# siyuanwu99/pred-occ-planner

Measured on AMD Instinct MI355X. Metric: replans/sec (SOGM update + QP: full replan = SOGM update + A* + corridors + QP + deconfliction), 128-agent batch per GPU, 200x200x200x20 voxel grid; aggregate over all agents, higher is better.
Workload: dtype f32 occupancy / f64 planning; 1 GPU; 128 agents/GPU x 1 GPU, 200x200x200x20 SOGM, sim_fkpcp-style moving cylinders, batched ADMM QP (BASELINE configs[2] per GPU); agents_total=128, cloud_points=622040, cylinders=555, map_input_staleness_ticks=0, parallelism=agents sharded x1, 1 all-gather/tick, exchange=local, sogm_grids_per_agent=3, sogm_reset=sparse (logged 32-byte sectors), sogm_cell_order=2x2x2 tiles, map_update=at the start of the tick

## Files before the change

### include/sogm_abi_debug.h

```cpp
#ifndef SOGM_ABI_DEBUG_H
#define SOGM_ABI_DEBUG_H
#include "sogm_abi.h"
#ifdef __cplusplus
extern "C" {
#endif

int sogm_sparse_reset_state(sogm_ctx *ctx, int32_t *out_host);

int         sogm_set_tuning(sogm_ctx *ctx, const char *key, double value);
int         sogm_get_tuning(const sogm_ctx *ctx, const char *key, double *out_value_host);
const char *sogm_tuning_key(int index);

int sogm_map_traffic(sogm_ctx *ctx, int64_t *out_host, int reset);

int sogm_grid_history(sogm_ctx *ctx, int32_t *out_host);

enum {
  SOGM_PROF_CLEAR = 0,
  SOGM_PROF_STAMP = 1,
  SOGM_PROF_SPLAT = 2,
  SOGM_PROF_ASTAR = 3,
  SOGM_PROF_CORRIDOR = 4,
  SOGM_PROF_QP = 5,
  SOGM_PROF_CLEAR_HEAD = 6,
  SOGM_PROF_EXCHANGE = 7,
  SOGM_PROF_N = 8
};
int sogm_set_profiling(sogm_ctx *ctx, int enable);
int sogm_set_profiling_slots(sogm_ctx *ctx, int slot_mask);
int sogm_profile_read(sogm_ctx *ctx, double *out_ms_host);
int sogm_profile_read_all(sogm_ctx *ctx, int slot, double *out_ms_host, int cap, int *out_n);

int sogm_device_clock(sogm_ctx *ctx, int64_t *out_ticks_host, void *stream);
int sogm_tick_clock(sogm_ctx *ctx, int64_t *out2_host);

int sogm_download_reference_layout(sogm_ctx *ctx, int agent, float *out_vt_host);

int sogm_dsp_download_state(sogm_dsp *d, int agent, float *store_host, float *objnum_host,
                            int32_t *counters_host);
int sogm_dsp_upload_state(sogm_dsp *d, int agent, const float *store_host, const float *last_pos3_host, double last_stamp,
                          const int32_t *cursors3_host);
int sogm_dsp_download_born(sogm_dsp *d, int agent, float *born_host, int cap, int32_t *n_born, int32_t *counters4);
int sogm_dsp_download_observations(sogm_dsp *d, int agent, int32_t *nobs_host, float *pc_host,
                                   float *maxlen_host);

int sogm_gridmap_download(sogm_gridmap *g, int agent, double *occupancy_host, int8_t *inflate_host,
                          int32_t *bounds_host, int32_t *counters_host);
int sogm_gridmap_force_frame(sogm_gridmap *g, int raycast_num);

int sogm_corridor_rules_batched(sogm_planner *counters_of, const SogmPlannerParams *pp_host, const double *start_pva,
                                const double *route, const int32_t *route_len, int route_cap, const double *polys,
                                const int32_t *nfaces, const int32_t *seg_state, int n, int max_faces, double *out_box,
                                double *out_shrunk, int32_t *out_seg_nfaces, int32_t *out_seg_state, double *out_polys,
                                int32_t *out_nfaces, int32_t *out_npoly, double *out_goal, void *stream);
#define SOGM_RULES_PARALLEL 1
int sogm_corridor_rules_batched_flags(sogm_planner *counters_of, const SogmPlannerParams *pp_host, const double *start_pva,
                                      const double *route, const int32_t *route_len, int route_cap, const double *polys,
                                      const int32_t *nfaces, const int32_t *seg_state, int n, int max_faces,
                                      double *out_box, double *out_shrunk, int32_t *out_seg_nfaces, int32_t *out_seg_state,
                                      double *out_polys, int32_t *out_nfaces, int32_t *out_npoly, double *out_goal,
                                      int flags, void *stream);

#define SOGM_FINISH_WAVE 1
int sogm_finish_batched(sogm_planner *counters_of, double corridor_tau, const int32_t *ret, const int32_t *npoly,
                        const int32_t *status, const double *cpts, const SogmTrajRecord *swarm, int n_swarm,
                        const int32_t *swarm_ego, const double *swarm_now, const double *t_start, const int32_t *drone_ids,
                        const int32_t *due, int n, SogmTrajRecord *out, int32_t *out_ok, int32_t *out_safe,
                        SogmTrajRecord *pub_own, SogmTrajRecord *pub_table, int flags, void *stream);

int sogm_debug_corridor_pairs(sogm_planner *p, unsigned long long *out4);

enum {
  SOGM_QP_STAT_TOTAL = 0,
  SOGM_QP_STAT_SETUP = 1,
  SOGM_QP_STAT_REFAC = 2,
  SOGM_QP_STAT_N_REFAC = 3,
  SOGM_QP_STAT_CHECK = 4,
  SOGM_QP_STAT_N_CHECK = 5,
  SOGM_QP_STAT_ITERS = 6,
  SOGM_QP_STAT_PATH = 7,
  SOGM_QP_STAT_FACTOR_ASM = 8,
  SOGM_QP_STAT_FACTOR_FWD = 9,
  SOGM_QP_STAT_FACTOR_BWD = 10,
  SOGM_QP_STAT_SHADER_CLOCKS = 11,
  SOGM_QP_STAT_CHECK_STAGE = 12,
  SOGM_QP_STAT_CHECK_RESID = 13,
  SOGM_QP_STAT_SETUP_SPLIT = 14,
  SOGM_QP_STAT_N = 16
};
int sogm_debug_qp_stats(sogm_planner *p, long long *out_host);
int sogm_debug_qp_layout(sogm_planner *p, int n_pieces, const int32_t *nfaces_host, long long *out8);

#ifdef __cplusplus
}
#endif
#endif
```

### pred-occ-planner_amd/_abi.py

```python
import ctypes as C
import os

_HERE = os.path.dirname(os.path.abspath(__file__))
LIB_PATH = os.environ.get("SOGM_LIB_PATH") or os.path.join(_HERE, "libsogm_hip.so")

SOGM_ABI_VERSION = 6
SOGM_MAX_PIECES = 16
SOGM_MAP_FAKE = 0
SOGM_MAP_RISKBASE = 1
SOGM_MAP_RISKVOXEL = 2
SOGM_STORE_F32, SOGM_STORE_F16 = 0, 1
SOGM_LAYOUT_TILED = 16
SOGM_DSP_MAX_T = 16

SOGM_OK = 0
SOGM_ERR_INVALID_ARG = -1
SOGM_ERR_NO_DEVICE = -2
SOGM_ERR_HIP = -3
SOGM_ERR_CAPACITY = -4
SOGM_ERR_STATE = -5
SOGM_ERR_COMM = -6
SOGM_COMM_ID_BYTES = 128
PROF_CLEAR, PROF_STAMP, PROF_SPLAT, PROF_ASTAR, PROF_CORRIDOR, PROF_QP, PROF_CLEAR_HEAD, PROF_EXCHANGE, PROF_N = range(9)

# ... 148 lines not shown
MAPAUDIT_ROW_FIELDS = ("n_region", "n_test", "n_truth", "n_both", "n_test_near", "n_truth_near", "truth_slice", "status")
MAPAUDIT_PARAMS_BYTES = C.sizeof(SogmMapAuditParams)

SOGM_VIEW_OUTSIDE, SOGM_VIEW_OFFIMAGE, SOGM_VIEW_FREE, SOGM_VIEW_SURFACE, SOGM_VIEW_HIDDEN = 0, 1, 2, 3, 4
SOGM_VIEWBIT_OUTSIDE, SOGM_VIEWBIT_OFFIMAGE, SOGM_VIEWBIT_FREE, SOGM_VIEWBIT_SURFACE, SOGM_VIEWBIT_HIDDEN = 1, 2, 4, 8, 16
SOGM_VIEWBIT_ALL = 31
VIEW_CLASS_NAMES = ("outside", "offimage", "free", "surface", "hidden")


class SogmViewParams(C.Structure):
    _fields_ = [("fx", C.c_double), ("fy", C.c_double), ("cx", C.c_double), ("cy", C.c_double), ("depth_scale", C.c_double),
                ("max_depth", C.c_double), ("near_z", C.c_double), ("far_z", C.c_double), ("tan_h", C.c_double),
                ("tan_v", C.c_double), ("band", C.c_double), ("rows", C.c_int32), ("cols", C.c_int32), ("classes", C.c_int32),
                ("reserved_", C.c_int32)]


VIEW_PARAMS_BYTES = C.sizeof(SogmViewParams)


class SogmFsmParams(C.Structure):
    _fields_ = [("replan_duration", C.c_double), ("replan_start_time", C.c_double), ("goal_tolerance", C.c_double),
                ("new_plan_interval", C.c_double), ("replan_max_failures", C.c_int32), ("reserved_", C.c_int32)]


class SogmFsmState(C.Structure):
    _fields_ = [("traj_start", C.c_double), ("status", C.c_int32), ("fail", C.c_int32), ("success", C.c_int32),
                ("reserved_", C.c_int32)]


class SogmFlightFsm(C.Structure):
    _fields_ = [("prm", SogmFsmParams), ("check_duration", C.c_double), ("state_inout", C.c_void_p),
                ("log_state", C.c_void_p), ("log_due", C.c_void_p), ("log_safe", C.c_void_p), ("log_reached", C.c_void_p),
                ("log_pub", C.c_void_p), ("log_hover_start", C.c_void_p), ("log_own", C.c_void_p)]


FSM_STATE_BYTES = C.sizeof(SogmFsmState)
FSM_PUB_NONE, FSM_PUB_NEW, FSM_PUB_HOVER = 0, 1, 2

SOGM_TRAJSRV_QUEUE = 256
SOGM_CMD_PUBLISHED, SOGM_CMD_HELD = 1, 2


class SogmTrajServerParams(C.Structure):
    _fields_ = [("replan_threshold", C.c_double), ("sample_dt", C.c_double), ("yaw_pi", C.c_double),
                ("yaw_dot_max", C.c_double), ("yaw_mode", C.c_int32), ("reserved_", C.c_int32)]


class SogmTrajPoint(C.Structure):
    _fields_ = [("t", C.c_double), ("pos", C.c_double * 3), ("vel", C.c_double * 3), ("acc", C.c_double * 3),
                ("yaw", C.c_double), ("yaw_dot", C.c_double)]


class SogmPositionCommand(C.Structure):
    _fields_ = [("t_pub", C.c_double), ("t_sample", C.c_double), ("pos", C.c_double * 3), ("vel", C.c_double * 3),
                ("acc", C.c_double * 3), ("yaw", C.c_double), ("yaw_dot", C.c_double), ("traj_id", C.c_int32),
                ("flags", C.c_int32)]


class SogmTrajServerCore(C.Structure):
    _fields_ = [("ts", C.c_double), ("te", C.c_double), ("duration", C.c_double), ("last_yaw", C.c_double),
                ("last_yawdot", C.c_double), ("init_pos", C.c_double * 3), ("head", C.c_int32), ("size", C.c_int32),
                ("traj_id", C.c_int32), ("received", C.c_int32), ("overflow", C.c_int32), ("reserved_", C.c_int32 * 3)]


FLIGHT_MAX_TICKS = 64
RULES_PARALLEL = 1
FINISH_WAVE = 1
FLIGHT_HDR_ERR, FLIGHT_HDR_FINISHED, FLIGHT_HDR_LATE_WGS = 4, 5, 15
FLIGHT_STAT_NAMES = ("gate_wait", "map", "search", "corridor", "qp", "finish", "chain", "ticks")
TRAJ_RECORD_BYTES = C.sizeof(SogmTrajRecord)
CYLINDER_BYTES = C.sizeof(SogmCylinder)
DEPTH_CAMERA_BYTES = C.sizeof(SogmDepthCamera)
DEPTH_BODIES_BYTES = C.sizeof(SogmDepthBodies)
SOGM_HIT_GROUND, SOGM_HIT_NONE = -1, -2
LABEL_SOURCES_BYTES = C.sizeof(SogmLabelSources)


class SogmTrajServerState(C.Structure):
    _fields_ = [("core", SogmTrajServerCore), ("traj", SogmTrajRecord)]


TRAJ_POINT_BYTES = C.sizeof(SogmTrajPoint)
POSITION_COMMAND_BYTES = C.sizeof(SogmPositionCommand)
TRAJSRV_STATE_BYTES = C.sizeof(SogmTrajServerState)

_vp = C.c_void_p
_i = C.c_int

QP_STAT_TOTAL, QP_STAT_SETUP, QP_STAT_REFAC, QP_STAT_N_REFAC, QP_STAT_CHECK, QP_STAT_N_CHECK, QP_STAT_ITERS, QP_STAT_PATH = range(8)
QP_STAT_FACTOR_ASM, QP_STAT_FACTOR_FWD, QP_STAT_FACTOR_BWD, QP_STAT_SHADER_CLOCKS = 8, 9, 10, 11
QP_STAT_CHECK_STAGE, QP_STAT_CHECK_RESID, QP_STAT_SETUP_SPLIT, QP_STAT_N = 12, 13, 14, 16

PROTOTYPES = {
    "sogm_abi_version": (_i, []),
    "sogm_last_error": (C.c_char_p, []),
    "sogm_device_count": (_i, []),
    "sogm_create": (_i, [C.POINTER(SogmSpec), _i, _i, C.POINTER(_vp)]),
    "sogm_destroy": (None, [_vp]),
    "sogm_grid_bytes": (C.c_int64, [_vp]),
    "sogm_grid_ptr": (_vp, [_vp]),
    "sogm_set_sparse_reset": (_i, [_vp, _i, _i]),
    "sogm_sparse_reset_state": (_i, [_vp, _vp]),
    "sogm_grid_history": (_i, [_vp, _vp]),
    "sogm_map_traffic": (_i, [_vp, _vp, _i]),
    "sogm_set_resample": (_i, [_vp, C.c_float, _i, _vp, _i]),
    "sogm_set_tuning": (_i, [_vp, C.c_char_p, C.c_double]),
    "sogm_get_tuning": (_i, [_vp, C.c_char_p, C.POINTER(C.c_double)]),
    "sogm_tuning_key": (C.c_char_p, [_i]),
    "sogm_set_body_particles": (_i, [_vp, C.POINTER(C.c_double), _i]),
    "sogm_set_overlap_clear": (_i, [_vp, _i]),
    "sogm_set_profiling": (_i, [_vp, _i]),
    "sogm_set_profiling_slots": (_i, [_vp, _i]),
    "sogm_profile_read": (_i, [_vp, C.POINTER(C.c_double)]),
    "sogm_profile_read_all": (_i, [_vp, _i, C.POINTER(C.c_double), _i, C.POINTER(_i)]),
    "sogm_update_gt": (_i, [_vp, _vp, _vp, _vp, _i, _vp, _vp, _vp]),
    "sogm_project_neighbours": (_i, [_vp, _vp, _i, _vp, _vp]),
    "sogm_update_gt_swarm": (_i, [_vp, _vp, _vp, _vp, _i, _vp, _vp, _vp, _i, _vp, _vp]),
    "sogm_device_clock": (_i, [_vp, C.POINTER(C.c_int64), _vp]),
    "sogm_tick_clock": (_i, [_vp, C.POINTER(C.c_int64)]),
    "sogm_cloud_block_bounds": (_i, [_vp, _i, _i, _vp, _vp]),
    "sogm_update_world": (_i, [_vp, C.POINTER(SogmWorld), _vp, _vp, _vp, _i, _vp, _vp]),
    "sogm_world_frames": (_i, [C.POINTER(SogmWorldTimeline), _i, _i, C.POINTER(SogmWorld), _vp]),
    "sogm_set_future_risk": (_i, [_vp, _vp, _vp, _vp, _vp]),
    "sogm_download_reference_layout": (_i, [_vp, _i, _vp]),
    "sogm_tick_inputs": (_i, [_vp, _i, C.c_double, C.c_double, _vp, _vp, _vp, _vp, _vp, _vp]),
    "sogm_merge_latest": (_i, [_vp, _vp, _vp, _vp, _i, _vp]),
    "sogm_fsm_init": (_i, [_vp, _i, C.c_double, _vp]),
    "sogm_fsm_inputs": (_i, [C.POINTER(SogmFsmParams), _vp, _vp, _vp, _i, C.c_double, _vp, _vp, _vp, _vp, _vp, _vp, _vp,
                             _vp, _vp]),
    "sogm_fsm_apply": (_i, [C.POINTER(SogmFsmParams), _vp, _vp, _vp, _vp, _vp, _vp, _vp, _vp, _vp, _vp, _vp, _i,
                            C.c_double, _vp]),
    "sogm_map_state": (_i, [_vp, _i, C.POINTER(C.c_double), C.POINTER(C.c_float), _vp]),
    "sogm_traj_eval": (_i, [_vp, _i, _vp, _vp, _vp, _vp]),
    "sogm_firi_batched": (_i, [_vp, _i, _vp, _vp, _vp, _vp, _vp, _i, C.c_double, _i, _i, _i, _vp, _vp, _vp, _vp]),
    "sogm_planner_select_agents": (_i, [_vp, _i, _i]),
    "sogm_planner_set_search_mode": (_i, [_vp, _i]),
    "sogm_query_clear": (_i, [_vp, _vp, _vp, _vp, _i, _i, _vp, _vp]),
    "sogm_obstacle_points": (_i, [_vp, _vp, _vp, _vp, _vp, _vp, _i, _vp, _vp, _i, _vp]),
    "sogm_planner_create": (_i, [_vp, C.POINTER(SogmAstarParams), C.POINTER(SogmPlannerParams),
                                 C.POINTER(SogmQpSettings), C.POINTER(_vp)]),
    "sogm_planner_destroy": (None, [_vp]),
    "sogm_astar_search": (_i, [_vp, _vp, _vp, _vp, _vp, _vp, _vp, _i, _vp, _vp, _i, _vp]),
    "sogm_corridor_generate": (_i, [_vp, _vp, _vp, _vp, _vp, _i, _vp, _vp, _vp, _vp, _vp]),
    "sogm_bezier_qp_solve": (_i, [_vp, _vp, _vp, _vp, _vp, _vp, _vp, _vp, _vp, _vp]),
    "sogm_bezier_qp_solve_timed": (_i, [_vp, _vp, _vp, _vp, C.c_double, C.c_double, _vp, _vp, _vp, _vp, _vp, _vp, _vp]),
    "sogm_linprog_batched": (_i, [_i, _vp, _vp, _vp, _vp, _i, _vp, _vp, _vp]),
    "sogm_corridor_rules_batched": (_i, [_vp, _vp, _vp, _vp, _vp, _i, _vp, _vp, _vp, _i, _i, _vp, _vp, _vp, _vp, _vp, _vp,
                                         _vp, _vp, _vp]),
    "sogm_corridor_rules_batched_flags": (_i, [_vp, _vp, _vp, _vp, _vp, _i, _vp, _vp, _vp, _i, _i, _vp, _vp, _vp, _vp, _vp,
                                               _vp, _vp, _vp, _i, _vp]),
    "sogm_finish_batched": (_i, [_vp, C.c_double, _vp, _vp, _vp, _vp, _vp, _i, _vp, _vp, _vp, _vp, _vp, _i, _vp, _vp, _vp,
                                 _vp, _vp, _i, _vp]),
    "sogm_debug_corridor_pairs": (_i, [_vp, _vp]),
    "sogm_debug_qp_stats": (_i, [_vp, _vp]),
    "sogm_debug_qp_layout": (_i, [_vp, _i, _vp, _vp]),
    "sogm_replan": (_i, [_vp, _vp, _vp, _vp, _vp, _vp, _vp, _vp]),
    "sogm_gridmap_create": (_i, [C.POINTER(SogmGridMapParams), _i, _i, C.POINTER(_vp)]),
    "sogm_gridmap_destroy": (None, [_vp]),
    "sogm_gridmap_update": (_i, [_vp, _vp, _vp, _vp, _vp, _vp]),
    "sogm_gridmap_query_inflate": (_i, [_vp, _vp, _vp, _i, _vp, _vp]),
    "sogm_render_depth": (_i, [C.POINTER(SogmWorld), C.POINTER(SogmDepthCamera), _i, _vp, _vp, _vp, _vp, _vp, _vp]),
    "sogm_render_depth_swarm": (_i, [C.POINTER(SogmWorld), C.POINTER(SogmDepthCamera), C.POINTER(SogmDepthBodies), _i, _vp,
                                     _vp, _vp, _vp, _vp, _vp, _vp]),
    "sogm_gridmap_download": (_i, [_vp, _i, _vp, _vp, _vp, _vp]),
    "sogm_gridmap_force_frame": (_i, [_vp, _i]),
    "sogm_traj_safe": (_i, [_vp, _vp, _vp, C.c_double, _vp, _vp]),
    "sogm_safe_after_opt": (_i, [_vp, _vp, _vp, _vp, _i, _vp, _vp, _vp, _vp]),
    "sogm_planner_flow_error": (_i, [_vp]),
    "sogm_planner_flow_failures": (_i, [_vp, _vp]),
    "sogm_planner_set_publish": (_i, [_vp, _vp, _vp]),
    "sogm_planner_set_prestamp": (_i, [_vp, _vp]),
    "sogm_prestamp_pending": (_i, [_vp]),
    "sogm_prestamp_join": (_i, [_vp, _vp]),
    "sogm_update_prestamped": (_i, [_vp, _vp, _i, _vp, _vp]),
    "sogm_planner_counters": (_i, [_vp, C.POINTER(C.c_int64), _i]),
    "sogm_flight_run": (_i, [_vp, C.POINTER(SogmFlight), _vp]),
    "sogm_flight_prepare": (_i, [_vp, _i]),
    "sogm_flight_stats": (_i, [_vp, _vp, _vp]),
    "sogm_planner_set_swarm": (_i, [_vp, _vp, _i, _vp, _vp]),
    "sogm_planner_set_due": (_i, [_vp, _vp]),
    "sogm_planner_set_flight_fsm": (_i, [_vp, C.POINTER(SogmFlightFsm)]),
    "sogm_audit_init_agents": (_i, [_vp, _i, _vp]),
    "sogm_swarm_audit": (_i, [C.POINTER(SogmAuditParams), _vp, _i, _i, _vp, C.c_double, _i, C.c_double, _i, _i, _vp, _vp,
                              _vp, _i, _vp, _vp, _vp, _vp]),
    "sogm_map_audit_default_params": (_i, [_i, _i, C.POINTER(SogmMapAuditParams)]),
    "sogm_map_audit": (_i, [_vp, _vp, C.POINTER(SogmMapAuditParams), _vp, _vp, _vp, _vp]),
    "sogm_view_default_params": (_i, [C.POINTER(SogmDepthCamera), C.POINTER(SogmViewParams)]),
    "sogm_view_mask": (_i, [_vp, C.POINTER(SogmViewParams), _vp, _vp, _vp, _vp, _vp, _vp]),
    "sogm_map_audit_masked": (_i, [_vp, _vp, C.POINTER(SogmMapAuditParams), _vp, _vp, _vp, _vp]),
    "sogm_traj_server_init": (_i, [_vp, _vp, _i, C.c_double, _vp, _vp, _vp]),
    "sogm_traj_server_run": (_i, [C.POINTER(SogmTrajServerParams), _vp, _vp, _vp, _vp, _vp, _i, _i, _i, _i, C.c_double, _i,
                                  C.c_double, C.c_double, _vp, _vp]),
    "sogm_camera_poses": (_i, [_vp, _i, _i, C.POINTER(C.c_double), C.POINTER(C.c_double), _vp, _vp, _vp]),
    "sogm_traj_allgather": (_i, [_vp, _vp, _vp, _i, _vp, _vp]),
    "sogm_exchange_wait": (_i, [_vp, _vp]),
    "sogm_comm_unique_id": (_i, [C.c_char_p]),
    "sogm_comm_create": (_i, [C.c_char_p, _i, _i, _i, C.POINTER(_vp)]),
    "sogm_comm_destroy": (None, [_vp]),
    "sogm_comm_handle": (_vp, [_vp]),
    "sogm_comm_info": (_i, [_vp, _vp]),
    "sogm_filter_point_cloud": (_i, [_vp, _vp, _vp, C.c_float, _i, _vp, _vp, _vp]),
    "sogm_filter_point_cloud_labelled": (_i, [_vp, _vp, _vp, _vp, C.c_float, _i, C.POINTER(SogmLabelSources), _vp, _vp, _vp,
                                              _vp, _vp]),
    "sogm_filter_reserve": (_i, [_vp, _i]),
    "sogm_dsp_create": (_i, [_vp, C.POINTER(SogmDspParams), _vp, _vp, _i, _vp, _i, _i, C.POINTER(_vp)]),
    "sogm_dsp_destroy": (None, [_vp]),
    "sogm_update_dsp": (_i, [_vp, _vp, _vp, _vp, _vp, _vp, _vp, _vp, _vp]),
    "sogm_dsp_publish": (_i, [_vp, _vp, _vp]),
    "sogm_dsp_download_state": (_i, [_vp, _i, _vp, _vp, _vp]),
    "sogm_dsp_upload_state": (_i, [_vp, _i, _vp, _vp, C.c_double, _vp]),
    "sogm_dsp_download_born": (_i, [_vp, _i, _vp, _i, _vp, _vp]),
    "sogm_dsp_download_observations": (_i, [_vp, _i, _vp, _vp, _vp]),
}


class SogmError(RuntimeError):
    pass


def load_library(path=LIB_PATH):
    if not os.path.exists(path):
        raise SogmError(
            f"HIP extension not built: {path} is missing. Run `python -c 'import __graft_entry__ as g; "
            "g.build()'` (hipcc --offload-arch=gfx950). There is no CPU fallback.")
    try:
        import torch
    except ImportError:
        pass
    lib = C.CDLL(path)
    for name, (res, args) in PROTOTYPES.items():
        fn = getattr(lib, name)
        fn.restype = res
        fn.argtypes = args
    got = lib.sogm_abi_version()
    if got != SOGM_ABI_VERSION:
        raise SogmError(f"{path} implements ABI version {got}, this binding was written against {SOGM_ABI_VERSION}: "
                        "rebuild the extension (python -c 'import __graft_entry__ as g; g.build()')")
    return lib


_lib = None


def lib():
    global _lib
    if _lib is None:
        _lib = load_library()
    return _lib


def check(rc, what):
    if rc != SOGM_OK:
        msg = lib().sogm_last_error()
        raise SogmError(f"{what} failed: status {rc} ({msg.decode() if msg else ''})")
```

### pred-occ-planner_amd/csrc/sogm_clear.hip

```cpp
#include <hip/hip_runtime.h>

#include <vector>

#include "sogm_device.hpp"

namespace sogm {

template <bool NT>
__device__ inline void clear_store(vfloat4 *p) {
  const vfloat4 z = {0.f, 0.f, 0.f, 0.f};
  if (NT)
    __builtin_nontemporal_store(z, p);
  else
    *p = z;
}
template <bool NT>
__global__ __launch_bounds__(256) void k_clear_slabs(vfloat4 *__restrict__ p, size_t n_vec4,
                                                     float *__restrict__ tail, int n_tail, int throttle) {
  const size_t stride = (size_t)gridDim.x * blockDim.x;
  size_t       i      = (size_t)blockIdx.x * blockDim.x + threadIdx.x;
  for (; i + 3 * stride < n_vec4; i += 4 * stride) {
    clear_store<NT>(p + i);
    clear_store<NT>(p + i + stride);
    clear_store<NT>(p + i + 2 * stride);
// ... 136 lines not shown
  MarkLog none{nullptr, nullptr, 0, nullptr};
  if (!c->sparse || slot < 0) return none;
  GridSlot &g = c->pool.slot[slot];
  if (!g.log) {
    Resources::Setup setup(c->res);
    if (c->res.device(&g.log, sizeof(unsigned) * (size_t)c->log_cap * c->n_agents) != hipSuccess ||
        c->res.device(&g.log_n, sizeof(unsigned) * (size_t)c->n_agents, true) != hipSuccess ||
        (!c->d_reset_stat && c->res.device(&c->d_reset_stat, 8 * sizeof(unsigned long long), true) != hipSuccess) ||
        hipStreamSynchronize(nullptr) != hipSuccess) {
      (void)hipGetLastError();
      c->sparse = 0;
      c->pool.untrack_all();
      return none;
    }
    setup.done();
    g.tracked = 0;
  }
  return MarkLog{g.log, g.log_n, c->log_cap, c->d_reset_stat ? c->d_reset_stat + 4 : nullptr};
}
static size_t agent_grid_bytes(const sogm_ctx *c) { return (size_t)c->spec.T * (size_t)c->geom.V * c->cell_bytes(); }

int reset_slot(sogm_ctx *c, hipStream_t st, int slot, float *grid, bool polite) {
  if (c->pool.loggable(slot)) {
    const MarkLog lg = mark_log(c, slot);
    const int wgs = c->tune_i(SOGM_TUNE_RESET_WGS) > 0 ? c->tune_i(SOGM_TUNE_RESET_WGS) : 32;
    const int lanes_env = c->tune_i(SOGM_TUNE_RESET_LANES), unroll_env = c->tune_i(SOGM_TUNE_RESET_UNROLL);
    const int lanes  = lanes_env == 2 || lanes_env == 4 ? lanes_env : polite ? 2 : 4;
    const int unroll = unroll_env == 1 || unroll_env == 8 ? unroll_env : polite ? 1 : 8;
    prof_begin(c, SOGM_PROF_CLEAR, st);
    auto *kern = lanes == 4 ? (unroll == 1 ? k_reset_sectors<4, 1> : k_reset_sectors<4, 8>)
                            : (unroll == 1 ? k_reset_sectors<2, 1> : k_reset_sectors<2, 8>);
    hipLaunchKernelGGL(kern, dim3(wgs, c->n_agents), dim3(256), 0, st, reinterpret_cast<char *>(grid),
                       agent_grid_bytes(c), lg.entries, lg.n, lg.cap, c->d_reset_stat);
    prof_end(c, SOGM_PROF_CLEAR, st);
    SOGM_HIP_CHECK(hipGetLastError());
    hipLaunchKernelGGL(k_zero_words, dim3((c->n_agents + 255) / 256), dim3(256), 0, st, lg.n, c->n_agents);
    SOGM_HIP_CHECK(hipGetLastError());
    c->pool.slot[slot].n_sparse++;
    return SOGM_OK;
  }
  return launch_clear(c, st, grid, polite);
}

int retire_wide_clear(sogm_ctx *c, hipStream_t st) {
  if (c->overlap >= 2 && c->clear_gate && c->wide_clear_pending) {
    hipLaunchKernelGGL(k_set_word, dim3(1), dim3(1), 0, st, c->clear_epoch_word, 0);
    SOGM_HIP_CHECK(hipGetLastError());
    c->wide_clear_pending = 0;
  }
  return SOGM_OK;
}

int adopt_preclear(sogm_ctx *c, hipStream_t st, bool join) {
  if (join)
    if (int rc = join_prestamp(c, st)) return rc;
  if (!c->pool.precleared()) return SOGM_OK;
  if (c->overlap >= 2) {
    const int nxt = c->pool.adopt_front();
    sync_grid(c);
    SOGM_HIP_CHECK(hipStreamWaitEvent(st, c->pool.slot[nxt].cleared, 0));
    const int early = c->tune_i(SOGM_TUNE_CLEAR_EARLY);
    if (join)
      if (int rc = retire_wide_clear(c, st)) return rc;
    if (c->clear_gate && early) {
      return queue_spare_clears_ahead(c, st);
    }
    return SOGM_OK;
  }
  SOGM_HIP_CHECK(hipStreamWaitEvent(st, c->ev_cleared, 0));
  c->pool.forget_preclear();
  return SOGM_OK;
}

int queue_spare_clears(sogm_ctx *c, hipEvent_t after) {
  if (c->overlap < 2 || c->pool.first_dirty() < 0) return SOGM_OK;
  SOGM_HIP_CHECK(hipStreamWaitEvent(c->side, after, 0));
  const double head_gb = c->tune[SOGM_TUNE_CLEAR_HEAD_GB] >= 0 ? c->tune[SOGM_TUNE_CLEAR_HEAD_GB] : 1.0e9;
  const size_t total = clear_vec4_total(c);
  size_t       head  = (size_t)(head_gb * 1e9 / 16.0);
  if (head > total) head = total;
  for (int g; (g = c->pool.first_dirty()) >= 0;) {
    float *grid = c->pool.slot[g].grid;
    int    rc   = SOGM_OK;
    if (c->pool.loggable(g)) {
      const int late = c->tune_i(SOGM_TUNE_RESET_LATE);
      if (late && c->clear_gate) {
        if (c->gate_frac_agents > 0 && c->gate_frac_agents < c->clear_gate_target && !c->gate_frac_valid) {
          hipLaunchKernelGGL(k_clear_gate, dim3(1), dim3(64), 0, c->side, c->clear_cursor, ~(size_t)0, c->clear_gate,
                             c->clear_gate_err, c->gate_frac_agents, c->clear_epoch_word, c->clear_epoch);
          SOGM_HIP_CHECK(hipGetLastError());
          SOGM_HIP_CHECK(hipEventRecord(c->ev_gate_frac, c->side));
          c->gate_frac_valid = 1;
        }
        hipLaunchKernelGGL(k_clear_gate, dim3(1), dim3(64), 0, c->side, c->clear_cursor, ~(size_t)0, c->clear_gate,
                           c->clear_gate_err, c->clear_gate_target, c->clear_epoch_word, c->clear_epoch);
        SOGM_HIP_CHECK(hipGetLastError());
        SOGM_HIP_CHECK(hipEventRecord(c->ev_gate_open, c->side));
        c->gate_open_valid = 1;
      }
      rc = reset_slot(c, c->side, g, grid, true);
    } else if (head == 0) {
      rc = launch_clear(c, c->side, grid, false);
    } else if (head >= total) {
      rc = launch_clear(c, c->side, grid, true);
    } else {
      rc = launch_clear(c, c->side, grid, true, 1, head);
      if (!rc) rc = launch_clear(c, c->side, grid, false, 2, head);
    }
    if (rc) return rc;
    SOGM_HIP_CHECK(hipEventRecord(c->pool.slot[g].cleared, c->side));
    c->pool.queue_ready(g);
  }
  return SOGM_OK;
}

int queue_spare_clears_ahead(sogm_ctx *c, hipStream_t st) {
  c->clear_epoch_ahead = 1;
  SOGM_HIP_CHECK(hipEventRecord(c->ev_grid_free, st));
  const int rc         = queue_spare_clears(c, c->ev_grid_free);
  c->clear_epoch_ahead = 0;
  return rc;
}
size_t clear_vec4_total(const sogm_ctx *c) {
  return (size_t)c->n_agents * c->spec.T * (size_t)c->geom.V * c->cell_bytes() / 4 / 4;
}
int launch_clear(sogm_ctx *c, hipStream_t st, float *grid, bool polite, int part, size_t split) {
  if (!grid) grid = c->d_grid;
  const int rc = launch_clear_impl(c, st, grid, polite, part, split);
  if (rc == SOGM_OK && part != 1) {
    const int     slot = c->pool.slot_of(grid);
    const MarkLog lg   = mark_log(c, slot);
    if (slot >= 0) c->pool.slot[slot].n_dense++;
    if (lg.entries) {
      hipLaunchKernelGGL(k_zero_words, dim3((c->n_agents + 255) / 256), dim3(256), 0, st, lg.n, c->n_agents);
      c->pool.slot[slot].tracked = hipGetLastError() == hipSuccess ? 1 : 0;
    }
  }
  return rc;
}
static int launch_clear_impl(sogm_ctx *c, hipStream_t st, float *grid, bool polite, int part, size_t split) {
  const size_t n     = ((size_t)c->n_agents * c->spec.T * (size_t)c->geom.V * c->cell_bytes() + 3) / 4;
  const size_t nall  = n / 4;
  const size_t first = part == 2 ? split : 0;
  const size_t nv4   = part == 1 ? split : nall - first;
  const int    tail  = part == 1 ? 0 : (int)(n - nall * 4);
  const int    slot  = part == 1 ? SOGM_PROF_CLEAR_HEAD : SOGM_PROF_CLEAR;
  size_t       want  = (nv4 + 255) / 256;
  const int env_wgs = c->tune_i(SOGM_TUNE_CLEAR_WGS) > 0 ? c->tune_i(SOGM_TUNE_CLEAR_WGS) : 0;
  const int env_throttle = c->tune_i(SOGM_TUNE_CLEAR_THROTTLE), nt = c->tune_i(SOGM_TUNE_CLEAR_NT) != 0;
  const size_t max_wgs  = env_wgs ? (size_t)env_wgs : (polite ? (c->clear_gate && part == 0 ? 80 : 64) : 2048);
  const int    throttle = env_wgs ? env_throttle : (polite ? 4 : 0);
  const int    nblk     = (int)(want < 1 ? 1 : (want > max_wgs ? max_wgs : want));
  const int wide_wgs = c->tune_i(SOGM_TUNE_CLEAR_WIDE_WGS), wide_bound = c->tune_i(SOGM_TUNE_CLEAR_WIDE_BOUND);
  if (polite && part == 0 && c->clear_gate && c->clear_cursor && c->side2 && wide_wgs > 0 && nt) {
    const size_t        nchunks = (nall + CLEAR_CHUNK_V4 - 1) / CLEAR_CHUNK_V4;
    unsigned long long *cur = c->clear_cursor + (c->clear_seq & 1), *nxt = c->clear_cursor + ((c->clear_seq + 1) & 1);
    ++c->clear_seq;
    SOGM_HIP_CHECK(hipEventRecord(c->ev_side2_go, st));
    SOGM_HIP_CHECK(hipStreamWaitEvent(c->side2, c->ev_side2_go, 0));
    prof_begin(c, slot, st);
    const int epoch = c->clear_epoch + c->clear_epoch_ahead;
    c->wide_clear_pending = 1;
    hipLaunchKernelGGL(k_clear_chunks<true>, dim3(nblk), dim3(256), 0, st, (vfloat4 *)grid, nall, grid + nall * 4,
                       tail, cur, nxt, c->clear_epoch_word, epoch, 0);
    hipLaunchKernelGGL(k_clear_gate, dim3(1), dim3(64), 0, c->side2, cur, nchunks, c->clear_gate,
                       c->clear_gate_err, c->clear_gate_target, c->clear_epoch_word, epoch);
    hipLaunchKernelGGL(k_clear_chunks<false>, dim3(wide_wgs), dim3(256), 0, c->side2, (vfloat4 *)grid, nall,
                       grid + nall * 4, 0, cur, nxt, c->clear_epoch_word, epoch, wide_bound);
    SOGM_HIP_CHECK(hipEventRecord(c->ev_side2_done, c->side2));
    SOGM_HIP_CHECK(hipStreamWaitEvent(st, c->ev_side2_done, 0));
    prof_end(c, slot, st);
    SOGM_HIP_CHECK(hipGetLastError());
    return SOGM_OK;
  }
  prof_begin(c, slot, st);
  if (nt)
    hipLaunchKernelGGL(k_clear_slabs<true>, dim3(nblk), dim3(256), 0, st, (vfloat4 *)grid + first, nv4,
                       grid + nall * 4, tail, throttle);
  else
    hipLaunchKernelGGL(k_clear_slabs<false>, dim3(nblk), dim3(256), 0, st, (vfloat4 *)grid + first, nv4,
                       grid + nall * 4, tail, throttle);
  prof_end(c, slot, st);
  SOGM_HIP_CHECK(hipGetLastError());
  return SOGM_OK;
}

int next_clear_epoch(sogm_ctx *c) {
  if (++c->clear_epoch <= 0) c->clear_epoch = 1;
  return c->clear_epoch;
}
int announce_clear_epoch(sogm_ctx *c, hipStream_t st) {
  next_clear_epoch(c);
  hipLaunchKernelGGL(k_set_word, dim3(1), dim3(1), 0, st, c->clear_epoch_word, c->clear_epoch);
  SOGM_HIP_CHECK(hipGetLastError());
  return SOGM_OK;
}

}

using namespace sogm;

__global__ __launch_bounds__(256) void k_log_distinct(sogm::MarkLog lg, int n_agents, unsigned *bitmap, size_t words_per_agent,
                                                      unsigned long long *out) {
  const int agent = blockIdx.y;
  if (agent >= n_agents) return;
  const unsigned  n = lg.n[agent] > (unsigned)lg.cap ? (unsigned)lg.cap : lg.n[agent];
  const unsigned *e = lg.entries + (size_t)agent * lg.cap;
  unsigned       *bm = bitmap + (size_t)agent * words_per_agent;
  unsigned long long ent = 0, dis = 0, near8 = 0, near63 = 0, near1k = 0;
  for (unsigned i = blockIdx.x * blockDim.x + threadIdx.x; i < n; i += gridDim.x * blockDim.x) {
    const unsigned sec = e[i];
    if (sec == 0xFFFFFFFFu || (size_t)(sec >> 5) >= words_per_agent) continue;
    ++ent;
    const unsigned bit = 1u << (sec & 31);
    if (!(atomicOr(bm + (sec >> 5), bit) & bit)) ++dis;
    bool d8 = false, d63 = false, d1k = false;
    for (unsigned b = 1; b <= 1023 && b <= i; ++b)
      if (e[i - b] == sec) {
        d1k = true;
        if (b <= 63) d63 = true;
        if (b <= 8) d8 = true;
        break;
      }
    near8 += d8, near63 += d63, near1k += d1k;
  }
  for (int d = 32; d >= 1; d >>= 1) {
    ent += __shfl_xor(ent, d, 64);
    dis += __shfl_xor(dis, d, 64);
    near8 += __shfl_xor(near8, d, 64);
    near63 += __shfl_xor(near63, d, 64);
    near1k += __shfl_xor(near1k, d, 64);
  }
  if ((threadIdx.x & 63) == 0 && ent) {
    atomicAdd(out, ent);
    atomicAdd(out + 1, dis);
    atomicAdd(out + 3, near8);
    atomicAdd(out + 4, near63);
    atomicAdd(out + 5, near1k);
  }
  if (blockIdx.x == 0 && threadIdx.x == 0 && lg.n[agent] > (unsigned)lg.cap) atomicAdd(out + 2, 1ull);
}

extern "C" {

int sogm_set_overlap_clear(sogm_ctx *c, int mode) {
  if (!c || mode < 0 || mode > 3) return SOGM_ERR_INVALID_ARG;
  SOGM_HIP_CHECK(hipSetDevice(c->device));
  if (c->update_pending) {
    (void)hipDeviceSynchronize();
    c->update_pending = 0;
  }
  if (c->pool.precleared() || c->pool.n_slots() > 1) {
    (void)hipDeviceSynchronize();
  }
  const sogm::GridPool::Change ch = c->pool.rebuild(mode >= 2 ? mode : 1);
  for (int i = ch.release_to; i-- > ch.release_from;) c->res.release(&c->pool.slot[i].grid);
  const size_t bytes = ((size_t)sogm_grid_bytes(c) + 15) & ~(size_t)15;
  {
    sogm::Resources::Setup setup(c->res);
    hipError_t e = hipSuccess;
    bool       grid = false;
    for (int i = ch.acquire_from; i < ch.acquire_to && e == hipSuccess; ++i)
      grid = (e = c->res.device(&c->pool.slot[i].grid, bytes)) != hipSuccess;
    for (int i = 0; i < ch.acquire_to && e == hipSuccess; ++i)
      if (!c->pool.slot[i].cleared) e = c->res.event(&c->pool.slot[i].cleared);
    if (e != hipSuccess) {
      (void)hipGetLastError();
      sogm::set_error(grid ? "sogm_set_overlap_clear: no room for the spare grid(s)" : "sogm_set_overlap_clear: event", e);
      return grid ? SOGM_ERR_CAPACITY : SOGM_ERR_HIP;
    }
    setup.done();
    c->pool.acquired(ch);
  }
  c->overlap = mode;
  return SOGM_OK;
}

int sogm_set_sparse_reset(sogm_ctx *c, int enable, int log_capacity) {
  if (!c || log_capacity < 0) return SOGM_ERR_INVALID_ARG;
  SOGM_HIP_CHECK(hipSetDevice(c->device));
  SOGM_HIP_CHECK(hipDeviceSynchronize());
  for (sogm::GridSlot &g : c->pool.slot) {
    c->res.release(&g.log);
    c->res.release(&g.log_n);
  }
  c->pool.untrack_all();
  c->sparse = enable ? 1 : 0;
  if (log_capacity > 0) c->log_cap = log_capacity;
  return SOGM_OK;
}

int sogm_sparse_reset_state(sogm_ctx *c, int32_t *out) {
  if (!c || !out) return SOGM_ERR_INVALID_ARG;
  SOGM_HIP_CHECK(hipSetDevice(c->device));
  SOGM_HIP_CHECK(hipDeviceSynchronize());
  const sogm::GridSlot &cur = c->pool.slot[c->pool.current()];
  auto clamp31 = [](unsigned long long v) { return (int32_t)(v > 0x7FFFFFFFull ? 0x7FFFFFFFull : v); };
  out[0] = c->sparse;
  out[1] = c->log_cap;
  out[2] = cur.tracked;
  out[3] = 0;
  out[4] = 0;
  if (c->sparse && cur.log_n) {
    std::vector<unsigned> n((size_t)c->n_agents);
    SOGM_HIP_CHECK(hipMemcpy(n.data(), cur.log_n, sizeof(unsigned) * n.size(), hipMemcpyDeviceToHost));
    unsigned           mx  = 0;
    unsigned long long tot = 0;
// ... 80 lines not shown
```

### pred-occ-planner_amd/csrc/sogm_context.hip

```cpp
#include <hip/hip_runtime.h>

#include <cmath>
#include <cstdio>
#include <cstdlib>
#include <cstring>
#include <new>

#include "sogm_device.hpp"

namespace sogm {

static thread_local char g_err[512] = {0};
void set_error(const char *what, hipError_t e) {
  std::snprintf(g_err, sizeof(g_err), "%s: %s", what, hipGetErrorString(e));
}
void set_error_text(const char *text) { std::snprintf(g_err, sizeof(g_err), "%s", text); }

}

using namespace sogm;

__global__ __launch_bounds__(256) void k_div_check(sogm::GridGeom g, unsigned bits_lo, unsigned bits_hi, unsigned long long *out) {
  const unsigned long long n    = (unsigned long long)(bits_hi - bits_lo);
  const unsigned long long step = (unsigned long long)gridDim.x * blockDim.x;
  unsigned                 bad = 0, first = 0xFFFFFFFFu;
  for (unsigned long long i = (unsigned long long)blockIdx.x * blockDim.x + threadIdx.x; i < n; i += step) {
    const unsigned b = bits_lo + (unsigned)i;
    const float    a = __uint_as_float(b);
    const float    q = g.div_res(a), t = a / g.res, qn = g.div_res(-a), tn = (-a) / g.res;
    if (__float_as_uint(q) != __float_as_uint(t) || __float_as_uint(qn) != __float_as_uint(tn)) {
      ++bad;
      if (b < first) first = b;
    }
  }
  if (bad) {
    atomicAdd(out, (unsigned long long)bad);
    atomicMin(out + 1, (unsigned long long)first);
  }
  if (blockIdx.x == 0 && threadIdx.x == 0) out[2] = (unsigned long long)g.fast_div;
}
__global__ void k_device_clock(long long *out) { *out = wall_clock64(); }

extern "C" {

int sogm_abi_version(void) { return SOGM_ABI_VERSION; }
const char *sogm_last_error(void) { return sogm::g_err; }

int sogm_device_count(void) {
  int n = 0;
  if (hipGetDeviceCount(&n) != hipSuccess) return 0;
  return n;
}

int sogm_create(const SogmSpec *spec, int n_agents, int device, sogm_ctx **out) {
  if (!spec || !out || n_agents <= 0) return SOGM_ERR_INVALID_ARG;
  if (spec->L <= 0 || spec->W <= 0 || spec->H <= 0 || spec->T <= 0 || spec->T > 32 ||
      !(spec->resolution > 0.f) || !(spec->time_resolution > 0.f))
    return SOGM_ERR_INVALID_ARG;
  if (spec->map_kind != SOGM_MAP_FAKE && spec->map_kind != SOGM_MAP_RISKBASE &&
      spec->map_kind != SOGM_MAP_RISKVOXEL)
    return SOGM_ERR_INVALID_ARG;
  if ((spec->storage & ~(1 | SOGM_LAYOUT_TILED)) != 0) return SOGM_ERR_INVALID_ARG;
  if ((spec->storage & SOGM_LAYOUT_TILED) && ((spec->L | spec->W | spec->H) & 1)) return SOGM_ERR_INVALID_ARG;
  if ((unsigned long long)spec->L * spec->W * spec->H >= (1ull << 30)) {
    sogm::set_error_text("sogm_create: L * W * H must stay below 2^30 cells per time slice");
    return SOGM_ERR_INVALID_ARG;
  }
  *out = nullptr;
  if (sogm_device_count() <= device || device < 0) {
    std::snprintf(sogm::g_err, sizeof(sogm::g_err), "no HIP device %d", device);
    return SOGM_ERR_NO_DEVICE;
  }
  if (hipSetDevice(device) != hipSuccess) return SOGM_ERR_NO_DEVICE;
  sogm_ctx *c = new (std::nothrow) sogm_ctx();
  if (!c) return SOGM_ERR_INVALID_ARG;
  c->spec          = *spec;
  c->geom          = make_geom(*spec);
  c->n_agents      = n_agents;
  c->device        = device;
  {
#define X(id, name, dflt, lo, hi) c->tune[SOGM_TUNE_##id] = (double)(dflt);
    SOGM_TUNING_TABLE(X)
#undef X
    const char *e = getenv("SOGM_SPARSE_RESET");
    c->sparse     = e ? atoi(e) != 0 : 1;
    const long long dflt = (long long)spec->L * spec->W * spec->H * spec->T / 80;
    c->log_cap    = (int)(dflt < (1 << 20) ? (1 << 20) : (dflt > (1 << 26) ? (1 << 26) : dflt));
  }
  const size_t n   = (size_t)n_agents * spec->T * (size_t)c->geom.V;
  hipError_t   e   = c->res.device(&c->pool.slot[0].grid, (n * c->cell_bytes() + 15) & ~(size_t)15);
  sogm::sync_grid(c);
  if (e == hipSuccess) e = c->res.device(&c->d_poses, sizeof(float) * 3 * n_agents, true);
  if (e == hipSuccess) e = c->res.device(&c->d_stamps, sizeof(double) * n_agents, true);
  if (e == hipSuccess) e = c->res.device(&c->d_scratch_vt, sizeof(float) * (size_t)c->geom.V * spec->T);
  if (e == hipSuccess) e = c->res.device(&c->clear_cursor, 2 * sizeof(unsigned long long), true);
  if (e == hipSuccess) e = c->res.stream(&c->side);
  if (e == hipSuccess) e = c->res.stream(&c->side2);
  if (e == hipSuccess) e = c->res.stream(&c->pstream);
  if (e == hipSuccess) e = c->res.event(&c->ev_side2_go);
  if (e == hipSuccess) e = c->res.event(&c->ev_side2_done);
  if (e == hipSuccess) e = c->res.event(&c->ev_grid_free);
  if (e == hipSuccess) e = c->res.event(&c->ev_cleared);
  if (e == hipSuccess) e = c->res.event(&c->ev_gate_open);
  if (e == hipSuccess) e = c->res.event(&c->ev_gate_frac);
  if (e == hipSuccess) e = hipStreamSynchronize(nullptr);
  if (e != hipSuccess) {
    sogm::set_error("sogm_create", e);
    sogm_destroy(c);
    return SOGM_ERR_HIP;
  }
  *out = c;
  return SOGM_OK;
}

void sogm_destroy(sogm_ctx *c) {
  if (!c) return;
  (void)hipSetDevice(c->device);
  c->res.release_all();
  delete c;
}

int64_t sogm_grid_bytes(const sogm_ctx *c) {
  return c ? (int64_t)c->n_agents * c->spec.T * (int64_t)c->geom.V * (int64_t)c->cell_bytes() : 0;
}
float *sogm_grid_ptr(sogm_ctx *c) {
  if (!c) return nullptr;
  if (c->update_pending) {
    (void)hipStreamSynchronize(c->ustream);
    c->update_pending = 0;
  }
  c->pool.dense_write_current();
  return c->d_grid;
}

static const char *const k_tune_names[SOGM_TUNE_N] = {
#define X(id, name, dflt, lo, hi) name,
    SOGM_TUNING_TABLE(X)
#undef X
};
static const double k_tune_range[SOGM_TUNE_N][2] = {
#define X(id, name, dflt, lo, hi) {(double)(lo), (double)(hi)},
    SOGM_TUNING_TABLE(X)
#undef X
};
static int tune_index(const char *key) {
  if (!key) return -1;
  for (int i = 0; i < SOGM_TUNE_N; ++i)
    if (std::strcmp(key, k_tune_names[i]) == 0) return i;
  return -1;
}
int sogm_set_tuning(sogm_ctx *c, const char *key, double value) {
  const int i = tune_index(key);
  if (!c) return SOGM_ERR_INVALID_ARG;
  if (i < 0) {
    char buf[160];
    std::snprintf(buf, sizeof(buf), "sogm_set_tuning: unknown key '%s'", key ? key : "(null)");
    sogm::set_error_text(buf);
    return SOGM_ERR_INVALID_ARG;
  }
  if (!(value >= k_tune_range[i][0] && value <= k_tune_range[i][1])) {
    char buf[200];
    std::snprintf(buf, sizeof(buf), "sogm_set_tuning: '%s' = %g is outside [%g, %g]", key, value, k_tune_range[i][0],
                  k_tune_range[i][1]);
    sogm::set_error_text(buf);
    return SOGM_ERR_INVALID_ARG;
  }
  c->tune[i] = value;
  return SOGM_OK;
}
int sogm_get_tuning(const sogm_ctx *c, const char *key, double *out) {
  const int i = tune_index(key);
  if (!c || !out || i < 0) return SOGM_ERR_INVALID_ARG;
  *out = c->tune[i];
  return SOGM_OK;
}
const char *sogm_tuning_key(int index) { return index >= 0 && index < SOGM_TUNE_N ? k_tune_names[index] : nullptr; }

int sogm_set_resample(sogm_ctx *c, float replan_risk_rate, int num_resample, const float *normal_table_dev, int n_table) {
  if (!c || !(replan_risk_rate >= 0.0f) || num_resample < 0 || n_table < 0) return SOGM_ERR_INVALID_ARG;
  const bool on = replan_risk_rate > 0.0f && num_resample > 0;
  if (on) {
    if (!normal_table_dev || c->n_body <= 0 || n_table < 3 * c->n_body * num_resample) {
      sogm::set_error_text("sogm_set_resample: the table must hold 3 * body particles * num_resample standard normals "
                           "(call sogm_set_body_particles first)");
      return SOGM_ERR_INVALID_ARG;
    }
    if (c->geom.half) {
      sogm::set_error_text("sogm_set_resample: fractional weights need SOGM_STORE_F32 cells");
      return SOGM_ERR_INVALID_ARG;
    }
  }
  c->geom.rs_rate = on ? replan_risk_rate : 0.0f;
  c->geom.rs_n    = on ? num_resample : 0;
  c->geom.rs_z    = on ? normal_table_dev : nullptr;
  c->geom.rs_nz   = on ? n_table : 0;
  return SOGM_OK;
}

int sogm_set_body_particles(sogm_ctx *c, const double *xyz, int n) {
  if (!c || !xyz || n <= 0) return SOGM_ERR_INVALID_ARG;
  SOGM_HIP_CHECK(hipSetDevice(c->device));
  c->res.release(&c->d_body);
  SOGM_HIP_CHECK(c->res.device(&c->d_body, sizeof(double) * 3 * n));
  SOGM_HIP_CHECK(hipMemcpy(c->d_body, xyz, sizeof(double) * 3 * n, hipMemcpyHostToDevice));
  c->n_body = n;
  for (int k = 0; k < 3; ++k) {
    double m = 0.0;
    for (int e = 0; e < n; ++e) m = std::fabs(xyz[e * 3 + k]) > m ? std::fabs(xyz[e * 3 + k]) : m;
    c->geom.body_ext[k] = (float)m;
  }
  return SOGM_OK;
}

int sogm_set_profiling(sogm_ctx *c, int enable) {
  return sogm_set_profiling_slots(c, enable ? (1 << SOGM_PROF_N) - 1 : 0);
}

int sogm_set_profiling_slots(sogm_ctx *c, int slot_mask) {
  if (!c || slot_mask < 0 || slot_mask >= (1 << SOGM_PROF_N)) return SOGM_ERR_INVALID_ARG;
  c->profiling = slot_mask;
  for (int k = 0; k < SOGM_PROF_N; ++k) c->ring_n[k] = 0;
  return SOGM_OK;
}

int sogm_profile_read(sogm_ctx *c, double *out_ms) {
  if (!c || !out_ms) return SOGM_ERR_INVALID_ARG;
  SOGM_HIP_CHECK(hipSetDevice(c->device));
  SOGM_HIP_CHECK(hipDeviceSynchronize());
  for (int k = 0; k < SOGM_PROF_N; ++k) {
    out_ms[k] = -1.0;
    if (c->ring_n[k] <= 0 || c->ring[k].empty()) continue;
    hipEvent_t *p  = c->ring[k].data() + 2 * ((c->ring_n[k] - 1) % SOGM_PROF_RING);
    float       ms = 0.f;
    if (hipEventElapsedTime(&ms, p[0], p[1]) == hipSuccess) out_ms[k] = (double)ms;
  }
  return SOGM_OK;
}

int sogm_profile_read_all(sogm_ctx *c, int slot, double *out_ms, int cap, int *out_n) {
  if (!c || !out_ms || !out_n || slot < 0 || slot >= SOGM_PROF_N || cap < 0) return SOGM_ERR_INVALID_ARG;
  SOGM_HIP_CHECK(hipSetDevice(c->device));
  SOGM_HIP_CHECK(hipDeviceSynchronize());
  long long n = c->ring_n[slot];
  if (n > SOGM_PROF_RING) n = SOGM_PROF_RING;
  if (n > cap) n = cap;
  *out_n = 0;
  if (c->ring[slot].empty()) return SOGM_OK;
  for (long long i = c->ring_n[slot] - n; i < c->ring_n[slot]; ++i) {
    hipEvent_t *p  = c->ring[slot].data() + 2 * (i % SOGM_PROF_RING);
    float       ms = 0.f;
    if (hipEventElapsedTime(&ms, p[0], p[1]) != hipSuccess) ms = -1.f;
// ... 56 lines not shown
```

### pred-occ-planner_amd/csrc/sogm_corridor.hip

```cpp
#include <hip/hip_runtime.h>

#include "sogm_corridor.hpp"

namespace sogm {

__global__ __launch_bounds__(256) void k_corridor_points(MapView m, SogmPlannerParams pp, CorridorWorkspace ws,
                                                        const double *__restrict__ start_pva,
                                                        const double *__restrict__ t_start,
                                                        const double *__restrict__ route,
                                                        const int32_t *__restrict__ route_len, int route_cap,
                                                        int agent0) {
  const CorridorIO io{.start_pva = start_pva, .t_start = t_start, .route = route, .route_len = route_len,
                      .route_cap = route_cap};
  corridor_points_body<4>(m, pp, ws, io, blockIdx.y + agent0, blockIdx.x);
}

__global__ __launch_bounds__(64) void k_corridor_segment(
    MapView m, SogmPlannerParams pp, CorridorWorkspace ws, const double *__restrict__ start_pva,
    const double *__restrict__ t_start, const double *__restrict__ route,
    const int32_t *__restrict__ route_len, int route_cap, int agent0) {
  extern __shared__ __attribute__((aligned(16))) char smem[];
  const CorridorIO io{.start_pva = start_pva, .t_start = t_start, .route = route, .route_len = route_len,
                      .route_cap = route_cap};
  corridor_segment_body<6, false>(m, pp, ws, io, blockIdx.y + agent0, blockIdx.x, smem, FiriDirect{});
}

__global__ __launch_bounds__(64) void k_firi_direct(MapView m, SogmPlannerParams pp, CorridorWorkspace ws,
                                                    FiriDirect fd) {
  extern __shared__ __attribute__((aligned(16))) char smem[];
  corridor_segment_body<FIRI_DIRECT_BD_MAX, true>(m, pp, ws, CorridorIO{}, blockIdx.x, 0, smem, fd);
}

__global__ __launch_bounds__(64) void k_corridor_finalize(
    SogmPlannerParams pp, CorridorWorkspace ws, const double *__restrict__ start_pva,
    const double *__restrict__ route, const int32_t *__restrict__ route_len, int route_cap,
    double *__restrict__ out_polys, int32_t *__restrict__ out_nfaces,
    int32_t *__restrict__ out_npoly, double *__restrict__ out_goal, int agent0) {
  const CorridorIO io{.start_pva = start_pva, .route = route, .route_len = route_len, .route_cap = route_cap,
                      .out_polys = out_polys, .out_nfaces = out_nfaces, .out_npoly = out_npoly, .out_goal = out_goal};
  extern __shared__ __attribute__((aligned(16))) char smem[];
  corridor_finalize_body(pp, ws, io, blockIdx.x + agent0, LpLds::carve(smem));
}

struct CorridorRules {
  const SogmPlannerParams *pp;
  const double            *polys_in;
  const int32_t           *nfaces_in;
  const int32_t           *state_in;
  double                  *out_box;
};
__device__ __forceinline__ void rules_segment(const CorridorRules &cr, const SogmPlannerParams &pp, const CorridorWorkspace &ws,
                                              const CorridorIO &io, int prob, int seg, char *smem) {
  double *base = (double *)smem, *s_poly = base + RulesLds::poly, *s_box = base + RulesLds::box, *s_w = base + RulesLds::w;
  const LpScratch sc{base + LpLds::work, base + LpLds::rows, (int *)(smem + RulesLds::perm)};
  const int lane = threadIdx.x, MF = pp.max_faces;
  const int slot = prob * SOGM_MAX_PIECES + seg;
  if (seg >= io.points(prob) - 1) {
    if (lane == 0) {
      ws.seg_state[slot]  = -2;
      ws.seg_nfaces[slot] = 0;
      for (int k = 0; k < 6; ++k) cr.out_box[slot * 6 + k] = 0.0;
    }
    return;
  }
  int nf = cr.nfaces_in[slot];
  nf     = nf < 0 ? 0 : (nf > MF ? MF : nf);
  if (lane == 0) segment_box(pp, io.start_pva + prob * 9, io.route + (size_t)prob * io.route_cap * 6, seg, s_box, s_w);
  for (int i = lane; i < nf * 4; i += 64) s_poly[i] = cr.polys_in[(size_t)slot * MF * 4 + i];
  wave_lds_sync();
  shrink_corridor(pp, s_w, s_poly, nf);
  wave_lds_sync();
  const bool valid = corridorValidW(s_poly, nf, nullptr, 0, sc);
  double    *out   = ws.polys + (size_t)slot * MF * 4;
  for (int i = lane; i < nf * 4; i += 64) out[i] = s_poly[i];
  if (lane == 0) {
    for (int k = 0; k < 6; ++k) cr.out_box[slot * 6 + k] = s_box[k];
    ws.seg_nfaces[slot] = nf;
    ws.seg_state[slot]  = cr.state_in && cr.state_in[slot] == -3 ? -3 : (valid ? 1 : 0);
  }
  wave_lds_sync();
}
__global__ __launch_bounds__(64) void k_corridor_rules(CorridorRules cr, CorridorWorkspace ws, CorridorIO io) {
  extern __shared__ __attribute__((aligned(16))) char smem[];
  double         *base = (double *)smem;
  const LpScratch sc{base + LpLds::work, base + LpLds::rows, (int *)(smem + RulesLds::perm)};
  const int               prob = blockIdx.x;
  const SogmPlannerParams pp   = cr.pp[prob];
  for (int seg = 0; seg < SOGM_MAX_PIECES; ++seg) rules_segment(cr, pp, ws, io, prob, seg, smem);
  __threadfence_block();
  __syncthreads();
  corridor_finalize_body(pp, ws, io, prob, sc);
}

__global__ __launch_bounds__(64) void k_corridor_rules_slots(CorridorRules cr, CorridorWorkspace ws, CorridorIO io, int *seg_done) {
  extern __shared__ __attribute__((aligned(16))) char smem[];
  const int               prob = blockIdx.x / SOGM_MAX_PIECES, seg = blockIdx.x % SOGM_MAX_PIECES;
  const SogmPlannerParams pp   = cr.pp[prob];
  rules_segment(cr, pp, ws, io, prob, seg, smem);
  __syncthreads();
  corridor_slot_done(pp, ws, io, prob, seg, seg < io.points(prob) - 1, smem, seg_done, false);
}
__global__ void k_pairs_residue(const unsigned *words, int n, unsigned long long *pair_cnt) {
  unsigned v = 0;
  for (int i = threadIdx.x; i < n; i += blockDim.x) v |= words[i];
  if (v) atomicOr(&pair_cnt[3], (unsigned long long)v);
}

__global__ __launch_bounds__(64) void k_corridor_flow(MapView m, SogmPlannerParams pp, CorridorWorkspace ws,
                                                      FlowCtl fc, CorridorIO io, int n_agents) {
  extern __shared__ __attribute__((aligned(16))) char smem[];
  const int lane  = threadIdx.x;
  const int total = n_agents * SOGM_MAX_PIECES;
  for (;;) {
    const int k = flow_ticket(&fc.hdr[FLOW_C_TICKET]);
    if (k >= total) break;
    const int agent = flow_wait_slot(fc.a_ready + k / SOGM_MAX_PIECES, &fc.hdr[FLOW_ERR]);
    if (agent < 0) break;
    __threadfence();
    const int seg = k % SOGM_MAX_PIECES;
    if (seg == 0 && lane == 0) fc.ts[agent * 8 + 2] = wall_clock64();
    if (corridor_slot(m, pp, ws, io, agent, seg, smem, fc.seg_done, false, nullptr)) {
      if (lane == 0) fc.ts[agent * 8 + 3] = wall_clock64();
      __threadfence();
      if (lane == 0) publish_next(fc.q_ready, &fc.hdr[FLOW_Q_READY_N], agent);
    }
    __syncthreads();
  }
}

hipError_t launch_corridor_flow(const MapView &m, const SogmPlannerParams &pp, const CorridorWorkspace &ws,
                                const FlowCtl &fc, int n_agents, int n_workgroups, const CorridorIO &io, hipStream_t st) {
  hipLaunchKernelGGL(k_corridor_flow, dim3(n_workgroups), dim3(64), SegmentLds<6>::bytes(pp.pc_capacity), st, m, pp,
                     ws, fc, io, n_agents);
  return hipGetLastError();
}

hipError_t launch_corridor(const MapView &m, const SogmPlannerParams &pp, const CorridorWorkspace &ws, int n_agents,
                           const CorridorIO &io, hipStream_t st, int agent0, hipEvent_t ev_map_read) {
  hipLaunchKernelGGL(k_corridor_points, dim3(SOGM_MAX_PIECES, n_agents), dim3(256), 0, st, m, pp, ws, io.start_pva,
                     io.t_start, io.route, io.route_len, io.route_cap, agent0);
  hipError_t e = hipGetLastError();
  if (e == hipSuccess && ev_map_read) e = hipEventRecord(ev_map_read, st);
  if (e != hipSuccess) return e;
  hipLaunchKernelGGL(k_corridor_segment, dim3(SOGM_MAX_PIECES, n_agents), dim3(64),
                     SegmentLds<6>::bytes(pp.pc_capacity), st, m, pp, ws, io.start_pva, io.t_start, io.route,
                     io.route_len, io.route_cap, agent0);
  if ((e = hipGetLastError()) != hipSuccess) return e;
  hipLaunchKernelGGL(k_corridor_finalize, dim3(n_agents), dim3(64), LpLds::bytes(), st, pp, ws, io.start_pva, io.route,
                     io.route_len, io.route_cap, io.out_polys, io.out_nfaces, io.out_npoly, io.out_goal, agent0);
  return hipGetLastError();
}

}

#include "sogm_flight_light.hpp"

extern "C" int sogm_firi_batched(const double *bd, int n_bd, const double *pc_xyz, const int32_t *pc_range,
                                 const double *a, const double *b, double *r, int iterations, double epsilon, int n,
                                 int max_points, int max_faces, double *out_hpoly, int32_t *out_nfaces,
                                 int32_t *out_status, void *stream) {
  if (n < 0 || n_bd < 1 || n_bd > FIRI_DIRECT_BD_MAX || iterations < 1 || max_points < 1 || max_points > 16384 ||
      max_faces < 1 || max_faces > FIRI_MAX_H ||
      (n > 0 && (!bd || !pc_range || !a || !b || !r || !out_hpoly || !out_nfaces || !out_status)))
    return SOGM_ERR_INVALID_ARG;
  if (n == 0) return SOGM_OK;
  hipStream_t st = (hipStream_t)stream;
  const size_t per = sizeof(double) * 8 * (size_t)max_points + sizeof(long long) * 16;
  char        *scratch = nullptr;
  SOGM_HIP_CHECK(hipMallocAsync((void **)&scratch, per * (size_t)n, st));
  sogm::CorridorWorkspace ws{};
  ws.fpc     = (double *)scratch;
  ws.tang    = ws.fpc + (size_t)n * max_points * 3;
  ws.distr   = ws.tang + (size_t)n * max_points * 4;
  ws.seg_dbg = (long long *)(ws.distr + (size_t)n * max_points);
  SogmPlannerParams pp{};
  pp.pc_capacity = max_points;
  sogm::FiriDirect fd{bd, n_bd, pc_xyz, pc_range, a, b, r, iterations, out_hpoly, out_nfaces, out_status,
                      max_faces, 0, epsilon};
  hipLaunchKernelGGL(sogm::k_firi_direct, dim3(n), dim3(64), sogm::SegmentLds<FIRI_DIRECT_BD_MAX>::bytes(max_points), st, sogm::MapView{},
                     pp, ws, fd);
  const hipError_t e = hipGetLastError();
  (void)hipFreeAsync(scratch, st);
  SOGM_HIP_CHECK(e);
  return SOGM_OK;
}

extern "C" int sogm_corridor_rules_batched(sogm_planner *counters_of, const SogmPlannerParams *pp_host,
                                           const double *start_pva, const double *route, const int32_t *route_len,
                                           int route_cap, const double *polys, const int32_t *nfaces,
                                           const int32_t *seg_state, int n, int max_faces, double *out_box,
                                           double *out_shrunk, int32_t *out_seg_nfaces, int32_t *out_seg_state,
                                           double *out_polys, int32_t *out_nfaces, int32_t *out_npoly,
                                           double *out_goal, void *stream) {
  return sogm_corridor_rules_batched_flags(counters_of, pp_host, start_pva, route, route_len, route_cap, polys, nfaces, seg_state,
                                           n, max_faces, out_box, out_shrunk, out_seg_nfaces, out_seg_state, out_polys,
                                           out_nfaces, out_npoly, out_goal, 0, stream);
}

extern "C" int sogm_corridor_rules_batched_flags(sogm_planner *counters_of, const SogmPlannerParams *pp_host,
                                                 const double *start_pva, const double *route, const int32_t *route_len,
                                                 int route_cap, const double *polys, const int32_t *nfaces,
                                                 const int32_t *seg_state, int n, int max_faces, double *out_box,
                                                 double *out_shrunk, int32_t *out_seg_nfaces, int32_t *out_seg_state,
                                                 double *out_polys, int32_t *out_nfaces, int32_t *out_npoly,
                                                 double *out_goal, int flags, void *stream) {
  if ((flags & ~SOGM_RULES_PARALLEL) || ((flags & SOGM_RULES_PARALLEL) && n > (1 << 20)) ||
      n < 0 || max_faces < 1 || max_faces > RULES_MAX_FACES || route_cap <= SOGM_MAX_PIECES ||
      (n > 0 && (!pp_host || !start_pva || !route || !route_len || !polys || !nfaces || !out_box || !out_shrunk ||
                 !out_seg_nfaces || !out_seg_state || !out_polys || !out_nfaces || !out_npoly || !out_goal)))
    return SOGM_ERR_INVALID_ARG;
  for (int i = 0; i < n; ++i)
    if (pp_host[i].max_faces != max_faces) return SOGM_ERR_INVALID_ARG;
  if (n == 0) return SOGM_OK;
  hipStream_t        st   = (hipStream_t)stream;
  SogmPlannerParams *d_pp = nullptr;
  SOGM_HIP_CHECK(hipMallocAsync((void **)&d_pp, sizeof(SogmPlannerParams) * (size_t)n, st));
  hipError_t e = hipMemcpyAsync(d_pp, pp_host, sizeof(SogmPlannerParams) * (size_t)n, hipMemcpyHostToDevice, st);
  if (e == hipSuccess) e = hipStreamSynchronize(st);
  int         *d_ctl = nullptr;
  const size_t n_ctl = (size_t)n + sogm::corridor_pair_words(n);
  if (e == hipSuccess && (flags & SOGM_RULES_PARALLEL)) {
    e = hipMallocAsync((void **)&d_ctl, sizeof(int) * n_ctl, st);
    if (e == hipSuccess) e = hipMemsetAsync(d_ctl, 0, sizeof(int) * n_ctl, st);
  }
  if (e == hipSuccess) {
    sogm::CorridorWorkspace ws{};
    ws.polys      = out_shrunk;
    ws.seg_nfaces = out_seg_nfaces;
    ws.seg_state  = out_seg_state;
    ws.counters   = counters_of ? counters_of->cw.counters : nullptr;
    const sogm::CorridorIO    io{.start_pva = start_pva, .route = route, .route_len = route_len, .route_cap = route_cap,
                                 .out_polys = out_polys, .out_nfaces = out_nfaces, .out_npoly = out_npoly,
                                 .out_goal = out_goal};
    const sogm::CorridorRules cr{d_pp, polys, nfaces, seg_state, out_box};
    if (flags & SOGM_RULES_PARALLEL) {
      ws.seg_ready = reinterpret_cast<unsigned *>(d_ctl + n);
      ws.pair_ok   = d_ctl + 2 * (size_t)n;
      ws.pair_cnt  = counters_of ? counters_of->cw.pair_cnt : nullptr;
      hipLaunchKernelGGL(sogm::k_corridor_rules_slots, dim3(n * SOGM_MAX_PIECES), dim3(64), sogm::RulesLds::bytes(), st, cr, ws,
                         io, d_ctl);
      if (ws.pair_cnt)
        hipLaunchKernelGGL(sogm::k_pairs_residue, dim3(1), dim3(256), 0, st, ws.seg_ready, (int)sogm::corridor_pair_words(n),
                           ws.pair_cnt);
    } else {
      hipLaunchKernelGGL(sogm::k_corridor_rules, dim3(n), dim3(64), sogm::RulesLds::bytes(), st, cr, ws, io);
    }
    e = hipGetLastError();
  }
  if (d_ctl) (void)hipFreeAsync(d_ctl, st);
  (void)hipFreeAsync(d_pp, st);
  SOGM_HIP_CHECK(e);
  return SOGM_OK;
}

extern "C" int sogm_debug_corridor_occupancy(int pc_capacity) {
  int n = 0;
  if (hipOccupancyMaxActiveBlocksPerMultiprocessor(&n, (const void *)sogm::k_corridor_segment, 64,
                                                   sogm::SegmentLds<6>::bytes(pc_capacity)) != hipSuccess)
    return -1;
  return n;
}

#ifdef SOGM_PROFILE_MVIE
extern "C" int sogm_debug_mvie_prof(unsigned long long *out2) {
  if (hipMemcpyFromSymbol(out2, HIP_SYMBOL(sogm::g_mvie_prof), 16) != hipSuccess) return -1;
  if (hipMemcpyFromSymbol(out2 + 2, HIP_SYMBOL(sogm::g_lbfgs_prof), 40) != hipSuccess) return -1;
  unsigned long long z[5] = {0, 0, 0, 0, 0};
  (void)hipMemcpyToSymbol(HIP_SYMBOL(sogm::g_mvie_prof), z, 16);
  (void)hipMemcpyToSymbol(HIP_SYMBOL(sogm::g_lbfgs_prof), z, 40);
  return 0;
}
#endif
```

### pred-occ-planner_amd/csrc/sogm_device.hpp

```cpp
#pragma once

#include <hip/hip_fp16.h>
#include <hip/hip_runtime.h>

#include <cstdlib>

#include <new>
#include <stdint.h>

#include "../../include/sogm_abi_debug.h"
#include "../../include/sogm_detmath.h"
#include "sogm_gridpool.hpp"
#include "sogm_resources.hpp"

namespace sogm {
typedef float vfloat4 __attribute__((ext_vector_type(4)));

struct GridGeom {
  int   L, W, H, T;
  int   V;
  float res;
  float rx, ry, rz;
  float dt;
  float risk_threshold;
// ... 271 lines not shown
  const void  *sl  = m.slab(agent, t);
  const int    s   = g.inf_step;
  const int    zs  = g.map_kind == SOGM_MAP_FAKE ? 0 : s;
  const float  thr = g.map_kind == SOGM_MAP_FAKE ? g.risk_threshold
                                                 : g.thr_region - (float)t * g.decay_region;
  float        sum = 0.0F;
  if (zs == 0 && s <= 3) {
    const char *base = reinterpret_cast<const char *>(sl);
    switch (s) {
      case 0: return window_sum_hits<0>(base, g, ix, iy, iz, thr);
      case 1: return window_sum_hits<1>(base, g, ix, iy, iz, thr);
      case 2: return window_sum_hits<2>(base, g, ix, iy, iz, thr);
      default: return window_sum_hits<3>(base, g, ix, iy, iz, thr);
    }
  }
  for (int x = -s; x <= s; ++x) {
    const int qx = ix + x;
    for (int y = -s; y <= s; ++y) {
      const int qy = iy + y;
      for (int z = -zs; z <= zs; ++z) {
        const int qz = iz + z;
        if (!g.in_range(qx, qy, qz)) continue;
        sum += cell_ld(sl, (size_t)g.phys(qx, qy, qz), g.half);
        if (sum > thr) return 1;
      }
    }
  }
  return 0;
}

__device__ inline int query_clear_time(const MapView &m, int agent, double px, double py,
                                       double pz, double dt) {
  int tf = (int)floor(dt / (double)m.g.dt);
  tf     = tf > (m.g.T - 1) ? m.g.T - 1 : tf;
  tf     = tf < 0 ? 0 : tf;
  return query_clear_idx(m, agent, px, py, pz, tf);
}

__device__ inline void bezier_pos(const SogmTrajRecord &r, double t, double out[3]) {
  int    piece = r.n_pieces - 1;
  double tt    = t;
  for (int i = 0; i < r.n_pieces; ++i) {
    tt -= r.duration[i];
    if (tt < 0) {
      piece = i;
      break;
    }
  }
  double t0 = 0;
  for (int k = 0; k < piece; ++k) t0 += r.duration[k];
  const double tf  = t0 + r.duration[piece];
  const double dur = tf - t0;
  const double s   = (t - t0) / dur;
  double       S[5];
  S[0] = 1.0;
  S[1] = s;
  S[2] = s * s;
  S[3] = s * s * s;
  S[4] = (s * s) * (s * s);
  const double A[5][5] = {{1, -4, 6, -4, 1},
                          {0, 4, -12, 12, -4},
                          {0, 0, 6, -12, 6},
                          {0, 0, 0, 4, -4},
                          {0, 0, 0, 0, 1}};
  const double *c = r.cpts + piece * 15;
  for (int d = 0; d < 3; ++d) {
    double acc = 0.0;
    for (int j = 0; j < 5; ++j) {
      double b = 0.0;
      for (int i = 0; i < 5; ++i) b += c[i * 3 + d] * A[i][j];
      acc += b * S[j];
    }
    out[d] = acc;
  }
}

__device__ inline int traj_safe_agent(const MapView &m, int a, const SogmTrajRecord &r, double t_now, double T, int first,
                                      int stride) {
  if (r.n_pieces <= 0) return 1;
  double t0 = t_now - r.time_start;
  if (t0 < 0) t0 = 0;
  if (t0 > T) return 1;
  double dur = 0;
  for (int k = 0; k < r.n_pieces; ++k) dur += r.duration[k];
  T = T > dur ? dur : T;
  int j = 0;
  for (double t = t0; t < T; t += 0.1, ++j) {
    if (j % stride != first) continue;
    double p[3];
    bezier_pos(r, t, p);
    const double dt = t + r.time_start - m.stamps[a];
    if (query_clear_time(m, a, p[0], p[1], p[2], dt) == 1) return 0;
  }
  return 1;
}

static_assert(sizeof(SogmTrajRecord) % 16 == 0, "a record is copied in 16-byte pieces");
__device__ __forceinline__ void copy_record(SogmTrajRecord *dst, const SogmTrajRecord *src, int lane, int stride = 64) {
  const uint4 *s = reinterpret_cast<const uint4 *>(src);
  uint4       *d = reinterpret_cast<uint4 *>(dst);
  for (int w = lane; w < (int)(sizeof(SogmTrajRecord) / 16); w += stride) d[w] = s[w];
}
__device__ inline bool traj_eval_relative(const SogmTrajRecord &r, double tt, double out[9]) {
  if (r.n_pieces <= 0) {
    for (int k = 0; k < 9; ++k) out[k] = 0.0;
    return false;
  }
  double total = 0;
  for (int k = 0; k < r.n_pieces; ++k) total += r.duration[k];
  tt = tt < 0 ? 0 : (tt > total ? total : tt);
  int    piece = r.n_pieces - 1;
  double rem   = tt;
  for (int k = 0; k < r.n_pieces; ++k) {
    rem -= r.duration[k];
    if (rem < 0) {
      piece = k;
      break;
    }
  }
  double t0 = 0;
  for (int k = 0; k < piece; ++k) t0 += r.duration[k];
  const double tf = t0 + r.duration[piece], dur = tf - t0, s = (tt - t0) / dur;
  const double A[5][5] = {{1, -4, 6, -4, 1}, {0, 4, -12, 12, -4}, {0, 0, 6, -12, 6},
                          {0, 0, 0, 4, -4},  {0, 0, 0, 0, 1}};
  const double S0[5] = {1, s, s * s, s * s * s, (s * s) * (s * s)};
  const double S1[5] = {0, 1, 2 * s, 3 * (s * s), 4 * (s * s * s)};
  const double S2[5] = {0, 0, 2, 6 * s, 12 * (s * s)};
  const double *c    = r.cpts + piece * 15;
  for (int d = 0; d < 3; ++d) {
    double p = 0, v = 0, a = 0;
    for (int j = 0; j < 5; ++j) {
      double b = 0;
      for (int q = 0; q < 5; ++q) b += c[q * 3 + d] * A[q][j];
      p += b * S0[j];
      v += b * S1[j];
      a += b * S2[j];
    }
    out[d]     = p;
    out[3 + d] = v / dur;
    out[6 + d] = a / (dur * dur);
  }
  return true;
}
__device__ inline bool traj_eval_record(const SogmTrajRecord &r, double t_abs, double out[9]) {
  return traj_eval_relative(r, t_abs - r.time_start, out);
}
}

#define SOGM_TUNING_TABLE(X)                                                                                             \
  X(GROUPS, "groups", 2, 1, 64)                     \
  X(SPEC_ASTAR, "spec_astar", 1, 0, 1)             \
  X(CLEAR_GATE_FRAC, "clear_gate_frac", 1, 0, 1)  \
  X(QP_WGS, "qp_wgs", 0, 0, 1024)                     \
  X(QP_ABLATE, "qp_ablate", 0, 0, 255)               \
  X(CLEAR_WGS, "clear_wgs", 0, 0, 65536)               \
  X(CLEAR_THROTTLE, "clear_throttle", 0, 0, 64)     \
  X(CLEAR_NT, "clear_nt", 1, 0, 1)                 \
  X(CLEAR_WIDE_WGS, "clear_wide_wgs", 256, 0, 65536)   \
  X(CLEAR_WIDE_BOUND, "clear_wide_bound", 0, 0, 64)  \
  X(CLEAR_HEAD_GB, "clear_head_gb", 1.0e9, 0, 1.0e12)   \
  X(CLEAR_EARLY, "clear_early", 0, 0, 1)           \
  X(CLEAR_RETIRE_AT_END, "clear_retire_at_end", 0, 0, 1)   \
  X(RESET_WGS, "reset_wgs", 32, 0, 4096)              \
  X(RESET_LANES, "reset_lanes", 0, 0, 4)           \
  X(RESET_UNROLL, "reset_unroll", 0, 0, 8)         \
  X(RESET_LATE, "reset_late", 1, 0, 1)             \
  X(STAMP_WGS, "stamp_wgs", 256, 0, 4096)             \
  X(STAMP_BITS_WGS, "stamp_bits_wgs", 0, 0, 4096)     \
  X(STAMP_LDS_LOG, "stamp_lds_log", 1, 0, 1)          \
  X(STAMP_CACHED, "stamp_cached", 0, 0, 1)            \
  X(STAMP_LDS_KB, "stamp_lds_kb", 0, 0, 64)                \
  X(SPLAT_WGS, "splat_wgs", 256, 0, 65536)             \
  X(SPLAT_OVERLAP, "splat_overlap", 1, 0, 1)       \
  X(PRESTAMP_BITS, "prestamp_bits", 32, 0, 1024)      \
  X(PRESTAMP_MARKS, "prestamp_marks", 64, 0, 1024)    \
  X(PRESTAMP_WGS, "prestamp_wgs", 0, 0, 65536)         \
  X(PRESTAMP_GATE_FRAC, "prestamp_gate_frac", 0.9, 0, 1)  \
  X(PRESTAMP_STREAM, "prestamp_stream", 1, 0, 1)  \
  X(PRESTAMP_LATE_AGENTS, "prestamp_late_agents", 8, 0, 65536)    \
  X(PRESTAMP_LATE_BITS, "prestamp_late_bits", 128, 0, 4096)      \
  X(PRESTAMP_LATE_MARKS, "prestamp_late_marks", 256, 0, 4096)    \
  X(FLIGHT_QP_UNITS, "flight_qp_units", 4, 1, 13)            \
  X(FLIGHT_SEARCH_UNITS, "flight_search_units", 2, 1, 13)    \
  X(FLIGHT_MAP_UNITS, "flight_map_units", 4, 1, 13)          \
  X(FLIGHT_MASKS, "flight_masks", 1, 0, 1)                   \
  X(FLIGHT_SPEC, "flight_spec", 1, 0, 1)                     \
  X(FLIGHT_RESET, "flight_reset", 8, 1, 256)                 \
  X(FLIGHT_BITS, "flight_bits", 16, 1, 256)                  \
  X(FLIGHT_MARKS, "flight_marks", 32, 1, 256)                \
  X(FLIGHT_SPLAT, "flight_splat", 4, 1, 64)                  \
  X(FLIGHT_ADMIT, "flight_admit", 48, 1, 65536)              \
  X(FLIGHT_PACE_US, "flight_pace_us", 20, 0, 100000)         \
  X(FLIGHT_HEADS, "flight_heads", 32, 1, 4096)               \
  X(FLIGHT_URGENT, "flight_urgent", 8, 0, 65536)            \
  X(FLIGHT_URGENT_WAVES, "flight_urgent_waves", 4096, 1, 4096)  \
  X(FLIGHT_URGENT_FINE, "flight_urgent_fine", 4, 1, 16)      \
  X(FLIGHT_GATE_PACE_US, "flight_gate_pace_us", 20, 0, 100000)   \
  X(FLIGHT_NEIGHBOUR_LAG, "flight_neighbour_lag", 2, 1, 2)  \
  X(FLIGHT_ENGINES, "flight_engines", 4, 1, 4)              \
  X(FLIGHT_ENGINE_FIRST, "flight_engine_first", 0, 0, 3)    \
  X(FLIGHT_EXCHANGE_UNITS, "flight_exchange_units", 0, 0, 4)  \
  X(FLIGHT_LIGHT_PER_CU, "flight_light_per_cu", 4, 1, 4)    \
  X(FLIGHT_MAP_PER_CU, "flight_map_per_cu", 8, 1, 8)        \
  X(UPDATE_FLOW, "update_flow", 0, 0, 1)                    \
  X(UPDATE_BITS, "update_bits", 16, 1, 256)                  \
  X(UPDATE_MARKS, "update_marks", 64, 1, 256)                \
  X(UPDATE_SPLAT, "update_splat", 40, 1, 64)                 \
  X(UPDATE_WGS, "update_wgs", 0, 0, 65536)                   \
  X(UPDATE_CHUNK, "update_chunk", 1, 1, 64)                  \
  X(UPDATE_CACHED, "update_cached", 0, 0, 1)                 \
  X(UPDATE_ORDER, "update_order", 1, 0, 1)
enum {
#define X(id, name, dflt, lo, hi) SOGM_TUNE_##id,
  SOGM_TUNING_TABLE(X)
#undef X
  SOGM_TUNE_N
};

struct sogm_ctx {
  sogm::Resources res;
  SogmSpec       spec;
  sogm::GridGeom geom;
  int            n_agents;
  int            device;
  float         *d_grid;
  size_t         cell_bytes() const { return geom.half ? 2 : 4; }
  float         *d_poses;
  double        *d_stamps;
  double        *d_body;
  int            n_body;
  int            updated;
  float         *d_scratch_vt;
  int            overlap;
  sogm::GridPool pool;
  hipStream_t    side;
  hipStream_t    pstream;
  hipEvent_t     ev_gate_frac;
  int            gate_frac_valid, gate_frac_agents;
  hipEvent_t     ev_gate_open;
  int            gate_open_valid;
  hipEvent_t     ev_grid_free, ev_cleared;
  const int          *clear_gate;
  const int          *clear_gate_err;
  int                 clear_gate_target;
  int                *clear_epoch_word;
  int                 clear_epoch, clear_epoch_ahead;
  int                 wide_clear_pending;
  unsigned long long *clear_cursor;
  unsigned            clear_seq;
  hipStream_t         side2;
  hipEvent_t          ev_side2_go, ev_side2_done;
  float         *d_filter_cells;
  void          *d_filter_box;
  int           *d_filter_blocks;
  int            filter_max_cells;
  unsigned long long *d_filter_keys;
  unsigned      *d_stamp_bits;
  float         *d_poses_next;
  double        *d_stamps_next;
  int            sparse;
  int            log_cap;
  unsigned long long *d_reset_stat;
  long long      n_stamps;
  long long     *h_tick_clock;
  void          *d_cand;
  int           *d_ncand;
  int           *d_blk_list;
  int           *d_blk_n;
  int            blk_cap;
  hipStream_t    xstream;
  hipEvent_t     ev_xin, ev_xdone;
  int            exchange_pending;
  hipEvent_t            ev_records_final;
  const SogmTrajRecord *records_final_ptr;
  int                   records_final_valid;
  hipEvent_t            ev_pdone;
  int                   pdone_pending;
  const int            *ps_stage;
  int                  *ps_err;
  volatile int         *ps_fail_host;
  int                   ps_fail_seen;
  hipStream_t    ustream;
  hipEvent_t     ev_uin, ev_udone;
  int            update_pending;
  int            map_epoch;
  int           *d_map_ready;
  int           *d_update_ctl;
  long long     *d_update_ts;
  int           *d_update_order;
  double         tune[SOGM_TUNE_N];
  int            tune_i(int k) const { return (int)tune[k]; }
  int            profiling;
  std::vector<hipEvent_t> ring[SOGM_PROF_N];
  long long      ring_n[SOGM_PROF_N];
};
#define SOGM_PROF_RING 1024

namespace sogm {
inline hipEvent_t *prof_pair(sogm_ctx *c, int slot, long long n) {
  if (c->ring[slot].empty()) c->ring[slot].resize(2 * SOGM_PROF_RING, nullptr);
  hipEvent_t *p = c->ring[slot].data() + 2 * (n % SOGM_PROF_RING);
  if (!p[0]) {
    Resources::Setup setup(c->res);
    if (c->res.event(&p[0], hipEventDefault) != hipSuccess || c->res.event(&p[1], hipEventDefault) != hipSuccess) return nullptr;
    setup.done();
  }
// ... 88 lines not shown
```

### pred-occ-planner_amd/csrc/sogm_finish.hip

```cpp
#include <hip/hip_runtime.h>

#include "sogm_finish.hpp"

namespace sogm {

__global__ __launch_bounds__(64) void k_safe_after_opt(const double *__restrict__ cpts,
                                                       const int32_t *__restrict__ npoly,
                                                       const SogmTrajRecord *__restrict__ rec, int n_rec,
                                                       const int32_t *__restrict__ ego_ids,
                                                       const double *__restrict__ t_now,
                                                       int32_t *__restrict__ out_safe, int agent0,
                                                       unsigned long long *counters) {
  extern __shared__ __attribute__((aligned(16))) double s_dyn[];
  const int a = blockIdx.y + agent0, i = blockIdx.x;
  if (deconflict_pair_unsafe(cpts + (size_t)a * SOGM_MAX_PIECES * 15, npoly[a], rec[i], ego_ids[a], t_now[a],
                             LpLds::carve(s_dyn), counters) &&
      threadIdx.x == 0)
    out_safe[a] = 0;
}

__global__ void k_fill_i32(int32_t *p, int n, int32_t v, int agent0) {
  const int i = blockIdx.x * blockDim.x + threadIdx.x;
  if (i < n) p[agent0 + i] = v;
}

__global__ __launch_bounds__(64) void k_finish_flow(FlowCtl fc, FinishArgs f, int n_agents) {
  extern __shared__ __attribute__((aligned(16))) double s_dyn[];
  const int lane = threadIdx.x;
  for (;;) {
    const int k = flow_ticket(&fc.hdr[FLOW_F_TICKET]);
    if (k >= n_agents) break;
    const int a = flow_wait_slot(fc.f_ready + k, &fc.hdr[FLOW_ERR]);
    if (a < 0) break;
    __threadfence();
    const int  code = finish_agent(f, a, LpLds::carve(s_dyn), lane);
    const bool safe = (code & 1) != 0;
    if (fc.p_ready) {
      __threadfence();
      if (lane == 0) publish_next(fc.p_ready, &fc.hdr[FLOW_P_READY_N], a);
    }
    if (lane == 0) {
      fc.ts[a * 8 + 6] = wall_clock64();
      finish_count(f, a, safe);
    }
  }
}

__global__ __launch_bounds__(64) void k_finish_wave(FinishArgs f) {
  extern __shared__ __attribute__((aligned(16))) double s_dyn[];
  const int a = blockIdx.x, lane = threadIdx.x;
  const int code = finish_agent(f, a, LpLds::carve(s_dyn), lane);
  if (lane == 0) finish_count(f, a, (code & 1) != 0);
}

__global__ void k_pack_records(int A, FinishArgs f, int agent0) {
  const int a = blockIdx.x * blockDim.x + threadIdx.x + agent0;
  if (a >= A) return;
  const int  npoly = f.npoly[a];
  const bool safe  = f.swarm ? f.out_safe[a] != 0 : true;
  const int  outcome = replan_outcome(f.ret[a], npoly, f.status[a], safe);
  const bool good    = outcome == SOGM_CNT_REPLAN_OK;
  if (f.counters && !(f.due && f.due[a] == 0)) atomicAdd(&f.counters[outcome], 1ull);
  SogmTrajRecord &r = f.out[a];
  r.drone_id        = f.drone_ids[a];
  r.time_start      = f.t_start[a];
  r.n_pieces        = good ? npoly : 0;
  for (int i = 0; i < SOGM_MAX_PIECES; ++i) r.duration[i] = (good && i < npoly) ? f.corridor_tau : 0.0;
  for (int i = 0; i < SOGM_MAX_PIECES * 15; ++i)
    r.cpts[i] = (good && i < npoly * 15) ? f.cpts[(size_t)a * SOGM_MAX_PIECES * 15 + i] : 0.0;
  f.out_ok[a] = good ? 1 : 0;
  if (f.pub_own) {
    if (good) f.pub_own[a] = r;
    if (f.pub_table) f.pub_table[a] = f.pub_own[a];
  }
}

hipError_t launch_deconflict(int n_agents, const double *cpts, const int32_t *npoly, const SogmTrajRecord *rec,
                             int n_rec, const int32_t *ego_ids, const double *t_now, int32_t *out_safe,
                             hipStream_t st, int agent0, unsigned long long *counters) {
  hipLaunchKernelGGL(k_fill_i32, dim3((n_agents + 63) / 64), dim3(64), 0, st, out_safe, n_agents, 1, agent0);
  if (n_rec > 0)
    hipLaunchKernelGGL(k_safe_after_opt, dim3(n_rec, n_agents), dim3(64), LpLds::bytes(), st, cpts, npoly, rec, n_rec,
                       ego_ids, t_now, out_safe, agent0, counters);
  return hipGetLastError();
}

hipError_t launch_finish_flow(const FlowCtl &fc, int n_agents, int n_workgroups, const FinishArgs &f, hipStream_t st) {
  hipLaunchKernelGGL(k_finish_flow, dim3(n_workgroups), dim3(64), LpLds::bytes(), st, fc, f, n_agents);
  return hipGetLastError();
}

hipError_t launch_pack_records(int n_agents, const FinishArgs &f, hipStream_t st, int agent0) {
  hipLaunchKernelGGL(k_pack_records, dim3((n_agents + 63) / 64), dim3(64), 0, st, agent0 + n_agents, f, agent0);
  return hipGetLastError();
}

}

extern "C" int sogm_finish_batched(sogm_planner *counters_of, double corridor_tau, const int32_t *ret, const int32_t *npoly,
                                   const int32_t *status, const double *cpts, const SogmTrajRecord *swarm, int n_swarm,
                                   const int32_t *swarm_ego, const double *swarm_now, const double *t_start,
                                   const int32_t *drone_ids, const int32_t *due, int n, SogmTrajRecord *out, int32_t *out_ok,
                                   int32_t *out_safe, SogmTrajRecord *pub_own, SogmTrajRecord *pub_table, int flags,
                                   void *stream) {
  if ((flags & ~SOGM_FINISH_WAVE) || n < 0 || n > (1 << 20) || n_swarm < 0 ||
      (n > 0 && (!ret || !npoly || !status || !cpts || !t_start || !drone_ids || !out || !out_ok || !out_safe)) ||
      (n > 0 && swarm && (!swarm_ego || !swarm_now)))
    return SOGM_ERR_INVALID_ARG;
  if (n == 0) return SOGM_OK;
  if (!swarm) n_swarm = 0;
  hipStream_t            st = (hipStream_t)stream;
  const sogm::FinishArgs f{.corridor_tau = corridor_tau, .ret = ret, .npoly = npoly, .status = status, .cpts = cpts,
                           .swarm = swarm, .n_swarm = n_swarm, .swarm_ego = swarm_ego, .swarm_now = swarm_now,
                           .t_start = t_start, .drone_ids = drone_ids, .out = out, .out_ok = out_ok, .out_safe = out_safe,
                           .counters = counters_of ? counters_of->cw.counters : nullptr, .pub_own = pub_own,
                           .pub_table = pub_table, .due = due};
  if (flags & SOGM_FINISH_WAVE) {
    hipLaunchKernelGGL(sogm::k_finish_wave, dim3(n), dim3(64), sogm::LpLds::bytes(), st, f);
    return launched("sogm_finish_batched k_finish_wave", hipGetLastError());
  }
  if (swarm)
    if (int rc = launched("sogm_finish_batched launch_deconflict",
                          sogm::launch_deconflict(n, cpts, npoly, swarm, n_swarm, swarm_ego, swarm_now, out_safe, st, 0,
                                                  f.counters)))
      return rc;
  return launched("sogm_finish_batched launch_pack_records", sogm::launch_pack_records(n, f, st, 0));
}
```

### pred-occ-planner_amd/csrc/sogm_planner.hip

```cpp
#include <hip/hip_runtime.h>

#include <cmath>
#include <cstdio>
#include <cstdlib>
#include <cstring>
#include <new>
#include <vector>

#include "sogm_planner.hpp"
#include "sogm_qp_layout.hpp"

using namespace sogm;

static void min_jerk_block(double *QM ) {
  auto diff = [](int rows, double scale, double *out, int cols) {
    for (int i = 0; i < rows * cols; ++i) out[i] = 0.0;
    for (int i = 0; i < rows / 3; ++i)
      for (int d = 0; d < 3; ++d) {
        out[(i * 3 + d) * cols + i * 3 + d]       = -scale;
        out[(i * 3 + d) * cols + (i + 1) * 3 + d] = scale;
      }
  };
  double p2v[12 * 15], v2a[9 * 12], a2j[6 * 9], p2a[9 * 15], p2j[6 * 15], W[6 * 6], T[6 * 15];
  diff(12, 4, p2v, 15);
  diff(9, 3, v2a, 12);
  diff(6, 2, a2j, 9);
  auto mul = [](const double *A, const double *B, double *C, int r, int k, int c) {
    for (int i = 0; i < r; ++i)
      for (int j = 0; j < c; ++j) {
        double s = 0;
        for (int q = 0; q < k; ++q) s += A[i * k + q] * B[q * c + j];
        C[i * c + j] = s;
      }
  };
  mul(v2a, p2v, p2a, 9, 12, 15);
  mul(a2j, p2a, p2j, 6, 9, 15);
  for (int i = 0; i < 36; ++i) W[i] = 0.0;
  for (int d = 0; d < 3; ++d) {
    W[d * 6 + d]           = 1.0 / 3;
    W[d * 6 + 3 + d]       = 1.0 / 6;
    W[(3 + d) * 6 + d]     = 1.0 / 6;
    W[(3 + d) * 6 + 3 + d] = 1.0 / 3;
  }
  mul(W, p2j, T, 6, 6, 15);
  for (int i = 0; i < 15; ++i)
    for (int j = 0; j < 15; ++j) {
      double s = 0;
      for (int q = 0; q < 6; ++q) s += p2j[q * 15 + i] * T[q * 15 + j];
      QM[i * 15 + j] = s;
    }
}

namespace sogm {
__global__ void k_flow_gate(FlowCtl fc, int expected) {
  if (threadIdx.x != 0) return;
  wait_at_least<WaitResidencyGate, false>(&fc.hdr[FLOW_ERR], &fc.hdr[FLOW_A_RESIDENT], expected);
}

hipError_t launch_flow_gate(const FlowCtl &fc, int expected, hipStream_t st) {
  hipLaunchKernelGGL(k_flow_gate, dim3(1), dim3(64), 0, st, fc, expected);
  return hipGetLastError();
}
}

__global__ void k_flow_report(const int *__restrict__ hdr, int *__restrict__ host_words, int *__restrict__ epoch_word,
                              long long *__restrict__ tick_clock) {
  if (tick_clock) tick_clock[1] = wall_clock64();
  if (epoch_word) *epoch_word = 0;
  const int e = hdr[FLOW_ERR];
  if (e != 0) {
    host_words[0] = e;
    host_words[1] = host_words[1] + 1;
  }
}

extern "C" {

static int planner_acquire(sogm_planner *p) {
  sogm_ctx                *map = p->map;
  const SogmPlannerParams *pp  = &p->pp;
  const int                A   = map->n_agents;
  sogm::Resources::Setup   setup(p->res);
  SOGM_HIP_CHECK(p->res.device(&p->aw.pool, p->aw.pool_stride * A * 2));
  SOGM_HIP_CHECK(p->res.device(&p->aw.hkeys, 8 * (size_t)p->aw.hash_cap * A * 2));
  SOGM_HIP_CHECK(p->res.device(&p->aw.verdict, sizeof(int) * A));
  SOGM_HIP_CHECK(p->res.device(&p->aw.dbg, sizeof(long long) * 8 * A, true));
  SOGM_HIP_CHECK(p->res.device(&p->d_ret, sizeof(int32_t) * A));
  SOGM_HIP_CHECK(p->res.device(&p->d_route_len, sizeof(int32_t) * A));
  SOGM_HIP_CHECK(p->res.device(&p->d_stats, sizeof(int32_t) * 4 * A));
  SOGM_HIP_CHECK(p->res.device(&p->d_route, sizeof(double) * 6 * p->route_cap * A));
  const size_t slots = (size_t)A * SOGM_MAX_PIECES, cap = (size_t)pp->pc_capacity;
  SOGM_HIP_CHECK(p->res.device(&p->cw.pc, sizeof(double) * slots * cap * 3));
  SOGM_HIP_CHECK(p->res.device(&p->cw.fpc, sizeof(double) * slots * cap * 3));
  SOGM_HIP_CHECK(p->res.device(&p->cw.tang, sizeof(double) * slots * cap * 4));
  SOGM_HIP_CHECK(p->res.device(&p->cw.distr, sizeof(double) * slots * cap));
  SOGM_HIP_CHECK(p->res.device(&p->cw.polys, sizeof(double) * slots * pp->max_faces * 4));
  SOGM_HIP_CHECK(p->res.device(&p->cw.seg_nfaces, sizeof(int32_t) * slots));
  SOGM_HIP_CHECK(p->res.device(&p->cw.seg_state, sizeof(int32_t) * slots));
  SOGM_HIP_CHECK(p->res.device(&p->cw.seg_npts, sizeof(int32_t) * slots));
  SOGM_HIP_CHECK(p->res.device(&p->cw.seg_dbg, sizeof(long long) * 16 * slots, true));
  SOGM_HIP_CHECK(p->res.device(&p->cw.counters, sizeof(unsigned long long) * SOGM_CNT_N, true));
  SOGM_HIP_CHECK(p->res.device(&p->cw.seg_ready, sizeof(int32_t) * sogm::corridor_pair_words(A), true));
  p->cw.pair_ok = reinterpret_cast<int32_t *>(p->cw.seg_ready) + A;
  SOGM_HIP_CHECK(p->res.device(&p->cw.pair_cnt, sizeof(unsigned long long) * 4, true));
  SOGM_HIP_CHECK(p->res.device(&p->cw.fin_dbg, sizeof(long long) * 4 * (size_t)A, true));
  p->qw.scratch_stride = qp_scratch_bytes_per_agent(pp->max_faces);
  p->qw.dyn_lds_bytes  = qp_kernel_setup();
  SOGM_HIP_CHECK(p->res.device(&p->qw.scratch, p->qw.scratch_stride * (size_t)A));
  SOGM_HIP_CHECK(p->res.device(&p->qw.k1_scratch, qp_k1_scratch_bytes_per_agent() * (size_t)A));
  SOGM_HIP_CHECK(p->res.device(&p->qw.dbg, sizeof(long long) * SOGM_QP_STAT_N * (size_t)A, true));
  SOGM_HIP_CHECK(p->res.device(&p->d_polys, sizeof(double) * slots * pp->max_faces * 4));
  SOGM_HIP_CHECK(p->res.device(&p->d_goal, sizeof(double) * 6 * A));
  SOGM_HIP_CHECK(p->res.device(&p->d_cpts, sizeof(double) * slots * 15));
  SOGM_HIP_CHECK(p->res.device(&p->d_nfaces, sizeof(int32_t) * slots));
  SOGM_HIP_CHECK(p->res.device(&p->d_npoly, sizeof(int32_t) * A));
  SOGM_HIP_CHECK(p->res.device(&p->d_status, sizeof(int32_t) * A));
  SOGM_HIP_CHECK(p->res.device(&p->d_iters, sizeof(int32_t) * A));
  SOGM_HIP_CHECK(p->res.device(&p->d_safe, sizeof(int32_t) * A));
  for (int g = 0; g < p->n_groups; ++g) {
    SOGM_HIP_CHECK(p->res.event(&p->ev_corr[g]));
    SOGM_HIP_CHECK(p->res.event(&p->ev_pts[g]));
    SOGM_HIP_CHECK(p->res.event(&p->ev_done[g]));
  }
  SOGM_HIP_CHECK(p->res.event(&p->ev_in));
  SOGM_HIP_CHECK(p->res.device(&p->d_flow, sizeof(int) * FlowBlock::words(A), true));
  FlowBlock::carve(p->d_flow, A, &p->fc);
  SOGM_HIP_CHECK(p->res.event(&p->ev_pdone));
  SOGM_HIP_CHECK(p->res.device(&p->d_flow_ts, sizeof(long long) * 12 * (size_t)A, true));
  p->fc.ts = p->d_flow_ts;
  for (int k = 0; k < 4; ++k) {
    SOGM_HIP_CHECK(p->res.stream(&p->fstream[k]));
    SOGM_HIP_CHECK(p->res.event(&p->ev_fdone[k]));
  }
  SOGM_HIP_CHECK(p->res.event(&p->ev_gate));
  SOGM_HIP_CHECK(p->res.device(&p->d_epoch, sizeof(int), true));
  SOGM_HIP_CHECK(p->res.pinned(&p->h_flow_fail, sizeof(int) * 2, hipHostMallocMapped));
  p->h_flow_fail[0] = p->h_flow_fail[1] = 0;
  SOGM_HIP_CHECK(hipStreamSynchronize(nullptr));
  return setup.done();
}

int sogm_planner_create(sogm_ctx *map, const SogmAstarParams *astar, const SogmPlannerParams *pp,
                        const SogmQpSettings *qp, sogm_planner **out) {
  if (!map || !astar || !pp || !qp || !out) return SOGM_ERR_INVALID_ARG;
  if (!(pp->opt_max_vel > 0 && pp->opt_max_vel < 1e20) || !(pp->opt_max_acc > 0 && pp->opt_max_acc < 1e20))
    return SOGM_ERR_INVALID_ARG;
  if (astar->allocate_num < 2 || astar->allocate_num > astar_pool_max() || astar->check_num < 1 || !(astar->resolution > 0) ||
      !(astar->time_resolution > 0))
    return SOGM_ERR_INVALID_ARG;
  if (pp->max_faces < 6 || pp->max_faces > 64 || pp->pc_capacity < 1 || pp->pc_capacity > 16384 || pp->firi_iterations < 1)
    return SOGM_ERR_INVALID_ARG;
  SOGM_HIP_CHECK(hipSetDevice(map->device));
  sogm_planner *p = new (std::nothrow) sogm_planner();
  if (!p) return SOGM_ERR_INVALID_ARG;
  p->map = map;
  p->ap  = *astar;
  p->pp  = *pp;
  p->ap.shot_ignores_time = pp->fake_planner ? 0 : 1;
  p->qs  = *qp;
  const int A = map->n_agents;
  int       hc = 1;
  while (hc < 2 * astar->allocate_num) hc <<= 1;
  p->aw.hash_cap    = hc;
  p->aw.pool_stride = astar_node_bytes() * (size_t)astar->allocate_num;
  p->route_cap      = 64;
  min_jerk_block(p->qc.QM);
  {
    int ng = map->tune_i(SOGM_TUNE_GROUPS);
    if (ng < 1) ng = 1;
    if (ng > SOGM_MAX_GROUPS) ng = SOGM_MAX_GROUPS;
    p->n_groups = A < ng ? A : ng;
  }
  p->sel_first   = 0;
  p->sel_count   = A;
  p->search_mode = 0;
  {
    p->spec_astar = map->tune_i(SOGM_TUNE_SPEC_ASTAR) != 0;
    if (p->spec_astar && 2 * A > sogm::astar_resident_workgroups(map->device)) p->spec_astar = 0;
  }
  {
    const char *ef = getenv("SOGM_FLOW");
    p->flow        = ef ? atoi(ef) != 0 : 1;
  }
  if (int rc = planner_acquire(p)) {
    delete p;
    return rc;
  }
  if (p->flow) {
    map->clear_gate        = p->fc.hdr + FLOW_Q_READY_N;
    map->clear_gate_err    = p->fc.hdr + FLOW_ERR;
    map->clear_gate_target = A;
    {
      const double f = map->tune[SOGM_TUNE_CLEAR_GATE_FRAC];
      if (f > 0.0 && f < 1.0) map->clear_gate_target = (int)(f * A + 0.5) < 1 ? 1 : (int)(f * A + 0.5);
    }
    map->clear_epoch_word  = p->d_epoch;
  }
  *out = p;
  return SOGM_OK;
}
void sogm_planner_destroy(sogm_planner *p) {
  if (!p) return;
  if (p->map) (void)hipSetDevice(p->map->device);
  if (p->map && p->map->ps_fail_host == p->h_flow_fail) p->map->ps_fail_host = nullptr;
  if (p->map && p->map->pdone_pending && p->map->ev_pdone == p->ev_pdone) {
    (void)hipDeviceSynchronize();
    p->map->pdone_pending = 0;
    p->map->ps_stage = p->map->ps_err = nullptr;
  }
  if (p->map && p->d_epoch && p->map->clear_epoch_word == p->d_epoch) {
    (void)hipDeviceSynchronize();
    p->map->clear_gate = p->map->clear_gate_err = p->map->clear_epoch_word = nullptr;
  }
  p->res.release_all();
  delete p;
}

int sogm_astar_search(sogm_planner *p, const double *start_pva, const double *goal,
                      const double *t_start, int32_t *out_ret, double *out_route,
                      int32_t *out_route_len, int route_cap, int32_t *out_stats,
                      int32_t *out_trace, int trace_cap, void *stream) {
  if (!p || !start_pva || !goal || !t_start || !out_ret || !out_route || !out_route_len ||
      !out_stats || route_cap < 2)
    return SOGM_ERR_INVALID_ARG;
  if (!p->map->updated) return SOGM_ERR_STATE;
  SOGM_HIP_CHECK(hipSetDevice(p->map->device));
  hipStream_t st = (hipStream_t)stream;
  if (int rc0 = sogm::join_update(p->map, st)) return rc0;
  const sogm::SearchIO io{.start_pva = start_pva, .goal = goal, .t_start = t_start, .out_ret = out_ret,
                          .out_route = out_route, .out_route_len = out_route_len, .route_cap = route_cap,
                          .out_stats = out_stats};
  prof_begin(p->map, SOGM_PROF_ASTAR, st);
  const hipError_t e = launch_astar(view_of(p->map), p->ap, p->pp.corridor_tau, astar_ws(p), p->sel_count, io, out_trace,
                                    out_trace ? trace_cap : 0, st, p->sel_first, nullptr, p->search_mode);
  prof_end(p->map, SOGM_PROF_ASTAR, st);
  return launched("k_astar", e);
}
int sogm_corridor_generate(sogm_planner *p, const double *start_pva, const double *t_start,
                           const double *route, const int32_t *route_len, int route_cap,
                           double *out_polys, int32_t *out_nfaces, int32_t *out_npoly,
                           double *out_goal, void *stream) {
  if (!p || !start_pva || !t_start || !route || !route_len || !out_polys || !out_nfaces ||
      !out_npoly || !out_goal || route_cap < 2)
    return SOGM_ERR_INVALID_ARG;
  if (!p->map->updated) return SOGM_ERR_STATE;
  SOGM_HIP_CHECK(hipSetDevice(p->map->device));
  hipStream_t st = (hipStream_t)stream;
  if (int rc0 = sogm::join_update(p->map, st)) return rc0;
  const sogm::CorridorIO io{.start_pva = start_pva, .t_start = t_start, .route = route, .route_len = route_len,
                            .route_cap = route_cap, .out_polys = out_polys, .out_nfaces = out_nfaces,
                            .out_npoly = out_npoly, .out_goal = out_goal};
  prof_begin(p->map, SOGM_PROF_CORRIDOR, st);
  const hipError_t e = launch_corridor(view_of(p->map), p->pp, p->cw, p->sel_count, io, st, p->sel_first);
  prof_end(p->map, SOGM_PROF_CORRIDOR, st);
  return launched("k_corridor", e);
}
int sogm_debug_astar_stats(sogm_planner *p, long long *out_host) {
  if (!p || !out_host) return SOGM_ERR_INVALID_ARG;
  SOGM_HIP_CHECK(hipDeviceSynchronize());
  SOGM_HIP_CHECK(hipMemcpy(out_host, p->aw.dbg, sizeof(long long) * 8 * (size_t)p->map->n_agents,
                           hipMemcpyDeviceToHost));
  return SOGM_OK;
}

int sogm_debug_astar_nodes(sogm_planner *p, int agent, void *out_host, int n) {
  if (!p || !out_host || agent < 0 || agent >= p->map->n_agents || n < 0) return SOGM_ERR_INVALID_ARG;
  SOGM_HIP_CHECK(hipDeviceSynchronize());
  SOGM_HIP_CHECK(hipMemcpy(out_host, p->aw.pool + (size_t)agent * p->aw.pool_stride, (size_t)n * sogm::astar_node_bytes(),
                           hipMemcpyDeviceToHost));
  return SOGM_OK;
}

int sogm_debug_qp_stats(sogm_planner *p, long long *out_host) {
  if (!p || !out_host) return SOGM_ERR_INVALID_ARG;
  SOGM_HIP_CHECK(hipDeviceSynchronize());
  SOGM_HIP_CHECK(hipMemcpy(out_host, p->qw.dbg, sizeof(long long) * SOGM_QP_STAT_N * (size_t)p->map->n_agents,
                           hipMemcpyDeviceToHost));
  return SOGM_OK;
}
int sogm_debug_qp_layout(sogm_planner *p, int n_pieces, const int32_t *nfaces_host, long long *out8) {
  if (!p || !nfaces_host || !out8 || n_pieces < 1 || n_pieces > SOGM_MAX_PIECES) return SOGM_ERR_INVALID_ARG;
  int faces = 0;
  for (int i = 0; i < n_pieces; ++i) {
    if (nfaces_host[i] < 0 || nfaces_host[i] > p->pp.max_faces) return SOGM_ERR_INVALID_ARG;
    faces += nfaces_host[i];
  }
  const sogm::QpLayout L(sogm::QpShape(n_pieces, faces), (size_t)p->qw.dyn_lds_bytes);
  const long long      out[8] = {L.fast, L.rows_in_lds, p->qw.dyn_lds_bytes, (long long)L.lds_bytes(), (long long)L.scratch_bytes(),
                                 L.fast && L.rows_in_lds, L.sh.G, L.sh.S};
  std::memcpy(out8, out, sizeof(out));
  return SOGM_OK;
}

int sogm_debug_corridor_stats(sogm_planner *p, long long *out_host) {
  if (!p || !out_host) return SOGM_ERR_INVALID_ARG;
  SOGM_HIP_CHECK(hipDeviceSynchronize());
  SOGM_HIP_CHECK(hipMemcpy(out_host, p->cw.seg_dbg,
                           sizeof(long long) * 16 * (size_t)p->map->n_agents * SOGM_MAX_PIECES,
                           hipMemcpyDeviceToHost));
  return SOGM_OK;
}

int sogm_debug_corridor_pairs(sogm_planner *p, unsigned long long *out4) {
  if (!p || !out4) return SOGM_ERR_INVALID_ARG;
  SOGM_HIP_CHECK(hipDeviceSynchronize());
  SOGM_HIP_CHECK(hipMemcpy(out4, p->cw.pair_cnt, sizeof(unsigned long long) * 4, hipMemcpyDeviceToHost));
  SOGM_HIP_CHECK(hipMemset(p->cw.pair_cnt, 0, sizeof(unsigned long long) * 4));
  std::vector<uint32_t> words(sogm::corridor_pair_words(p->map->n_agents));
  SOGM_HIP_CHECK(hipMemcpy(words.data(), p->cw.seg_ready, sizeof(uint32_t) * words.size(), hipMemcpyDeviceToHost));
  for (const uint32_t w : words) out4[3] |= w;
  return SOGM_OK;
}
int sogm_debug_corridor_finalize_times(sogm_planner *p, long long *out_host) {
  if (!p || !out_host) return SOGM_ERR_INVALID_ARG;
  SOGM_HIP_CHECK(hipDeviceSynchronize());
  SOGM_HIP_CHECK(hipMemcpy(out_host, p->cw.fin_dbg, sizeof(long long) * 4 * (size_t)p->map->n_agents, hipMemcpyDeviceToHost));
  return SOGM_OK;
}

int sogm_bezier_qp_solve(sogm_planner *p, const double *start_pva, const double *goal_pv,
                         const double *polys, const int32_t *nfaces, const int32_t *npoly,
                         double *out_cpts, int32_t *out_status, int32_t *out_iters, void *stream) {
  if (!p || !start_pva || !goal_pv || !polys || !nfaces || !npoly || !out_cpts || !out_status ||
      !out_iters)
    return SOGM_ERR_INVALID_ARG;
  SOGM_HIP_CHECK(hipSetDevice(p->map->device));
  hipStream_t st = (hipStream_t)stream;
  const sogm::QpIO io{.start_pva = start_pva, .goal_pv = goal_pv, .polys = polys, .nfaces = nfaces, .npoly = npoly,
                      .out_cpts = out_cpts, .out_status = out_status, .out_iters = out_iters};
  prof_begin(p->map, SOGM_PROF_QP, st);
  sogm::QpWorkspace qw0 = p->qw;
  qw0.ablate            = p->map->tune_i(SOGM_TUNE_QP_ABLATE);
  const hipError_t e    = launch_qp(p->pp, p->qs, qw0, p->qc, p->sel_count, io, st, p->sel_first);
  prof_end(p->map, SOGM_PROF_QP, st);
  return launched("k_qp", e);
}
int sogm_bezier_qp_solve_timed(sogm_planner *p, const double *start_pva, const double *end_pva,
                               const double *time_alloc, double max_vel, double max_acc, const double *polys,
                               const int32_t *nfaces, const int32_t *npoly, double *out_cpts, int32_t *out_status,
                               int32_t *out_iters, void *stream) {
  if (!p || !start_pva || !end_pva || !time_alloc || !polys || !nfaces || !npoly || !out_cpts || !out_status ||
      !out_iters || !(max_vel > 0 && max_vel < 1e20) || !(max_acc > 0 && max_acc < 1e20))
    return SOGM_ERR_INVALID_ARG;
  SOGM_HIP_CHECK(hipSetDevice(p->map->device));
  hipStream_t       st = (hipStream_t)stream;
  SogmPlannerParams pp = p->pp;
  pp.opt_max_vel       = max_vel;
  pp.opt_max_acc       = max_acc;
  sogm::QpWorkspace qw = p->qw;
  qw.t_alloc           = time_alloc;
  qw.goal_stride       = 9;
  const sogm::QpIO io{.start_pva = start_pva, .goal_pv = end_pva, .polys = polys, .nfaces = nfaces, .npoly = npoly,
                      .out_cpts = out_cpts, .out_status = out_status, .out_iters = out_iters};
  prof_begin(p->map, SOGM_PROF_QP, st);
  const hipError_t e = launch_qp(pp, p->qs, qw, p->qc, p->sel_count, io, st, p->sel_first);
  prof_end(p->map, SOGM_PROF_QP, st);
  return launched("k_qp", e);
}
int sogm_safe_after_opt(sogm_planner *p, const double *cpts, const int32_t *npoly,
                        const SogmTrajRecord *records, int n_records, const int32_t *ego_ids,
                        const double *t_now, int32_t *out_safe, void *stream) {
  if (!p || !cpts || !npoly || !ego_ids || !t_now || !out_safe || n_records < 0 || (n_records > 0 && !records))
    return SOGM_ERR_INVALID_ARG;
  SOGM_HIP_CHECK(hipSetDevice(p->map->device));
  if (int rc = sogm::join_exchange(p->map, (hipStream_t)stream)) return rc;
  return launched("sogm_safe_after_opt", sogm::launch_deconflict(p->sel_count, cpts, npoly, records, n_records, ego_ids,
                                                                t_now, out_safe, (hipStream_t)stream, p->sel_first));
}

int sogm_planner_select_agents(sogm_planner *p, int first, int count) {
  if (!p || first < 0 || count < 1 || first + count > p->map->n_agents) return SOGM_ERR_INVALID_ARG;
  p->sel_first = first;
  p->sel_count = count;
  return SOGM_OK;
}
int sogm_planner_set_search_mode(sogm_planner *p, int mode) {
  if (!p || mode < 0 || (mode & ~(3 | 4 | 16)) != 0 || (mode & 3) == 3) return SOGM_ERR_INVALID_ARG;
  p->search_mode = mode;
  return SOGM_OK;
}

int sogm_debug_flow_peek(sogm_planner *p, int *out_host, int n) {
  if (!p || !out_host || n < 0) return SOGM_ERR_INVALID_ARG;
  if (!p->peek) SOGM_HIP_CHECK(p->res.stream(&p->peek));
  hipStream_t peek = p->peek;
  const int nf = FlowBlock(p->map->n_agents).gen;
  SOGM_HIP_CHECK(hipMemcpyAsync(out_host, p->d_flow, sizeof(int) * (size_t)(n < nf ? n : nf), hipMemcpyDeviceToHost, peek));
  if (n > nf)
    SOGM_HIP_CHECK(hipMemcpyAsync(out_host + nf, p->d_safe, sizeof(int) * (size_t)(n - nf), hipMemcpyDeviceToHost, peek));
  SOGM_HIP_CHECK(hipStreamSynchronize(peek));
  return SOGM_OK;
}

int sogm_debug_flow_times(sogm_planner *p, long long *out_host) {
  if (!p || !out_host) return SOGM_ERR_INVALID_ARG;
  SOGM_HIP_CHECK(hipDeviceSynchronize());
  SOGM_HIP_CHECK(hipMemcpy(out_host, p->d_flow_ts, sizeof(long long) * 8 * (size_t)p->map->n_agents, hipMemcpyDeviceToHost));
  return SOGM_OK;
}

int sogm_debug_planner_buffer(sogm_planner *p, int which, void *out_host, size_t bytes) {
  if (!p || !out_host) return SOGM_ERR_INVALID_ARG;
  const size_t A = (size_t)p->map->n_agents, slots = A * SOGM_MAX_PIECES;
  const void  *src[11] = {p->d_polys, p->d_nfaces, p->d_npoly, p->d_goal, p->d_route, p->d_route_len, p->d_cpts, p->d_iters,
                          p->d_status, p->d_ret, p->d_stats};
  const size_t len[11] = {sizeof(double) * slots * p->pp.max_faces * 4, sizeof(int32_t) * slots, sizeof(int32_t) * A,
                          sizeof(double) * 6 * A, sizeof(double) * 6 * p->route_cap * A, sizeof(int32_t) * A,
                          sizeof(double) * slots * 15, sizeof(int32_t) * A, sizeof(int32_t) * A, sizeof(int32_t) * A,
                          sizeof(int32_t) * 4 * A};
  if (which < 0 || which > 10 || bytes > len[which]) return SOGM_ERR_INVALID_ARG;
  SOGM_HIP_CHECK(hipDeviceSynchronize());
  SOGM_HIP_CHECK(hipMemcpy(out_host, src[which], bytes, hipMemcpyDeviceToHost));
  return SOGM_OK;
}

int sogm_debug_prestamp_times(sogm_planner *p, long long *out_host) {
  if (!p || !out_host) return SOGM_ERR_INVALID_ARG;
  SOGM_HIP_CHECK(hipDeviceSynchronize());
  SOGM_HIP_CHECK(hipMemcpy(out_host, p->d_flow_ts + 8 * (size_t)p->map->n_agents, sizeof(long long) * 4 * (size_t)p->map->n_agents,
                           hipMemcpyDeviceToHost));
  return SOGM_OK;
}

int sogm_planner_flow_error(sogm_planner *p) {
  if (!p) return SOGM_ERR_INVALID_ARG;
  int hdr[FLOW_HDR];
  SOGM_HIP_CHECK(hipSetDevice(p->map->device));
  SOGM_HIP_CHECK(hipDeviceSynchronize());
  SOGM_HIP_CHECK(hipMemcpy(hdr, p->d_flow, sizeof(hdr), hipMemcpyDeviceToHost));
  return hdr[FLOW_ERR];
}

int sogm_planner_flow_failures(sogm_planner *p, int32_t out[2]) {
  if (!p || !out) return SOGM_ERR_INVALID_ARG;
  volatile int *h = p->h_flow_fail;
  out[0]          = h ? h[0] : 0;
  out[1]          = h ? h[1] : 0;
  return SOGM_OK;
}

int sogm_planner_counters(sogm_planner *p, int64_t *out_host, int reset) {
  if (!p || !out_host) return SOGM_ERR_INVALID_ARG;
  SOGM_HIP_CHECK(hipSetDevice(p->map->device));
  SOGM_HIP_CHECK(hipDeviceSynchronize());
  SOGM_HIP_CHECK(hipMemcpy(out_host, p->cw.counters, sizeof(int64_t) * SOGM_CNT_N, hipMemcpyDeviceToHost));
  if (reset) SOGM_HIP_CHECK(hipMemset(p->cw.counters, 0, sizeof(int64_t) * SOGM_CNT_N));
  return SOGM_OK;
}

int sogm_planner_set_publish(sogm_planner *p, SogmTrajRecord *own_records, SogmTrajRecord *next_table) {
  if (!p || (next_table && !own_records)) return SOGM_ERR_INVALID_ARG;
  p->pub_own   = own_records;
  p->pub_table = next_table;
  return SOGM_OK;
}

int sogm_planner_set_prestamp(sogm_planner *p, const SogmPrestamp *ps) {
  if (!p) return SOGM_ERR_INVALID_ARG;
  if (!ps) {
    p->ps_on = 0;
    return SOGM_OK;
  }
  if (!ps->hover_inout || !ps->out_now || !ps->out_t_start || !ps->out_pva) return SOGM_ERR_INVALID_ARG;
  const SogmWorld *w = ps->world;
  if (w) {
    if (!w->cloud_xyz || !w->block_bounds || w->n_points < 0 || w->block_points < 64 || w->block_points > 4096 ||
        w->n_blocks != (w->n_points + w->block_points - 1) / w->block_points || w->n_cyl < 0 || (w->n_cyl > 0 && !w->cylinders))
      return SOGM_ERR_INVALID_ARG;
  } else if (!ps->cloud_xyz || !ps->cloud_range || ps->n_cyl < 0 || (ps->n_cyl > 0 && !ps->cylinders)) {
    return SOGM_ERR_INVALID_ARG;
  }
  p->ps = sogm::PrestampDev{
      .frame      = {.cloud       = w ? w->cloud_xyz : ps->cloud_xyz,
                     .cloud_range = w ? nullptr : ps->cloud_range,
                     .cb          = {},
                     .cyl         = w ? w->cylinders : ps->cylinders,
                     .n_cyl       = w ? w->n_cyl : ps->n_cyl},
      .tick       = {.own = nullptr, .hover = ps->hover_inout, .now = ps->out_now, .t_start = ps->out_t_start,
                     .pva = ps->out_pva, .start_offset = ps->replan_start_offset},
      .stamp      = ps->next_stamp,
      .poses_host = ps->out_poses};
  p->ps_world_on = w ? 1 : 0;
  if (w) {
    p->ps_world = *w;
    sogm::CloudBlocks sized{};
    if (int rc = sogm::world_blocks(p->map, w, &sized)) return rc;
  }
  p->ps_on = 1;
  return SOGM_OK;
}

int sogm_planner_set_due(sogm_planner *p, const int32_t *due_dev_or_null) {
  if (!p) return SOGM_ERR_INVALID_ARG;
  p->due = due_dev_or_null;
  return SOGM_OK;
}

int sogm_planner_set_flight_fsm(sogm_planner *p, const SogmFlightFsm *fsm) {
  if (!p) return SOGM_ERR_INVALID_ARG;
  if (!fsm) {
    p->fl_fsm_on = 0;
    p->fl_fsm    = SogmFlightFsm{};
    return SOGM_OK;
  }
  if (!fsm->state_inout) {
    sogm::set_error_text("sogm_planner_set_flight_fsm: state_inout is NULL");
    return SOGM_ERR_INVALID_ARG;
  }
  const double v[5] = {fsm->prm.replan_duration, fsm->prm.replan_start_time, fsm->prm.goal_tolerance,
                       fsm->prm.new_plan_interval, fsm->check_duration};
  for (double x : v)
    if (!std::isfinite(x) || x < 0.0) {
      sogm::set_error_text("sogm_planner_set_flight_fsm: the parameters must be finite and not negative");
      return SOGM_ERR_INVALID_ARG;
    }
  if (fsm->prm.replan_max_failures < 0) {
    sogm::set_error_text("sogm_planner_set_flight_fsm: replan_max_failures must not be negative");
    return SOGM_ERR_INVALID_ARG;
  }
  p->fl_fsm    = *fsm;
  p->fl_fsm_on = 1;
  return SOGM_OK;
}

int sogm_planner_set_swarm(sogm_planner *p, const SogmTrajRecord *records, int n_records,
                           const int32_t *ego_ids, const double *t_now) {
  if (!p || n_records < 0 || (records && (!ego_ids || !t_now))) return SOGM_ERR_INVALID_ARG;
  p->swarm     = records;
  p->n_swarm   = records ? n_records : 0;
  p->swarm_ego = ego_ids;
  p->swarm_now = t_now;
  return SOGM_OK;
}

__global__ __launch_bounds__(1024) void k_flow_reset(int *hdr, int n_hdr, int *ready, int n_ready, int *verdict,
                                                     int n_verdict, unsigned *pairs, int n_pairs, int *epoch_word, int epoch,
                                                     int *gen_word, int gen) {
  const int i0 = (int)threadIdx.x, step = (int)blockDim.x;
  for (int i = i0; i < n_hdr; i += step) hdr[i] = 0;
  for (int i = i0; i < n_ready; i += step) ready[i] = -1;
  for (int i = i0; i < n_pairs; i += step) pairs[i] = 0u;
  if (verdict)
    for (int i = i0; i < n_verdict; i += step) verdict[i] = 0;
  __threadfence();
  __syncthreads();
  if (threadIdx.x == 0) {
    if (epoch_word) __hip_atomic_store(epoch_word, epoch, __ATOMIC_RELEASE, __HIP_MEMORY_SCOPE_AGENT);
    __hip_atomic_store(gen_word, gen, __ATOMIC_RELEASE, __HIP_MEMORY_SCOPE_AGENT);
  }
}

__global__ void k_update_rank(const long long *__restrict__ ts, int *__restrict__ order, int n, int by) {
  for (int a = threadIdx.x; a < n; a += blockDim.x) {
    if (!by) {
      order[a] = a;
      continue;
    }
    const long long da = ts[a * 8 + 6] - ts[a * 8 + 0];
    int             r  = 0;
    for (int b = 0; b < n; ++b) {
      const long long db = ts[b * 8 + 6] - ts[b * 8 + 0];
      r += (db > da || (db == da && b < a)) ? 1 : 0;
    }
    order[r] = a;
  }
}

struct FlowCall {
  const double   *start_pva, *goal, *t_start;
  const int32_t  *drone_ids;
  SogmTrajRecord *out_records;
  int32_t        *out_ok;
  hipStream_t     main;
  bool            spec;
  int            *gen_word;
  int             n_cu, wg_q, wg_f;
  bool            prestamp;
  hipStream_t     pst;
};

static int flow_reset(sogm_planner *p, FlowCall &call) {
  sogm_ctx         *c    = p->map;
  const hipStream_t main = call.main, sC = p->fstream[1];
  const int         A    = c->n_agents;
  const bool        spec = call.spec;
  SOGM_HIP_CHECK(hipStreamWaitEvent(sC, p->ev_pdone, 0));
  if (c->pool.current_prestamped()) {
    SOGM_HIP_CHECK(hipEventRecord(p->ev_gate, main));
    SOGM_HIP_CHECK(hipStreamWaitEvent(sC, p->ev_gate, 0));
  }
  const FlowBlock fb(A);
  int *gen_word = p->d_flow + fb.gen;
  ++p->reset_epoch;
  hipLaunchKernelGGL(k_flow_reset, dim3(1), dim3(1024), 0, sC, p->d_flow, fb.zero_words(), p->d_flow + fb.fill_first(),
                     fb.fill_words(), spec ? p->aw.verdict : nullptr, A, p->cw.seg_ready, (int)sogm::corridor_pair_words(A),
                     c->overlap >= 2 && c->clear_gate ? c->clear_epoch_word : nullptr,
                     c->overlap >= 2 && c->clear_gate ? sogm::next_clear_epoch(c) : 0, gen_word, p->reset_epoch);
  SOGM_HIP_CHECK(hipGetLastError());
  call.gen_word = gen_word;
  return SOGM_OK;
}
static int flow_launch_chain(sogm_planner *p, FlowCall &call) {
  sogm_ctx         *c    = p->map;
  const hipStream_t main = call.main, sA = main, sC = p->fstream[1], sQ = p->fstream[2], sF = p->fstream[3];
  const int         A    = c->n_agents;
  const MapView     mv   = view_of(c);
  const bool        spec = call.spec;
  int              *gen_word = call.gen_word;
  const double     *start_pva = call.start_pva, *goal = call.goal, *t_start = call.t_start;
  SogmTrajRecord   *out_records = call.out_records;
  int32_t          *out_ok      = call.out_ok;
  if (c->exchange_pending)
    for (int k = 1; k < 4; ++k) SOGM_HIP_CHECK(hipStreamWaitEvent(p->fstream[k], c->ev_xdone, 0));
  prof_begin(c, SOGM_PROF_ASTAR, sA);
  sogm::FlowCtl fca = p->fc;
  fca.map_ready = c->update_pending ? c->d_map_ready : nullptr;
  fca.map_epoch = c->map_epoch;
  fca.reset_gen   = gen_word;
  fca.reset_epoch = p->reset_epoch;
  fca.out_ok      = out_ok;
  fca.out_records = reinterpret_cast<int *>(out_records);
  fca.rec_words   = (int)(sizeof(SogmTrajRecord) / sizeof(int));
  if (int rc = launched("sogm_replan: k_astar",
                        launch_astar(mv, p->ap, p->pp.corridor_tau, astar_ws(p), A, search_io(p, start_pva, goal, t_start),
                                     nullptr, 0, sA, 0, &fca, spec ? 8 : 0)))
    return rc;
  prof_end(c, SOGM_PROF_ASTAR, sA);
  SOGM_HIP_CHECK(hipEventRecord(p->ev_in, main));
  if (int rc = launched("sogm_replan: k_flow_gate", sogm::launch_flow_gate(p->fc, spec ? 2 * A : A, sC))) return rc;
  SOGM_HIP_CHECK(hipEventRecord(p->ev_gate, sC));
  SOGM_HIP_CHECK(hipStreamWaitEvent(sQ, p->ev_gate, 0));
  SOGM_HIP_CHECK(hipStreamWaitEvent(sF, p->ev_gate, 0));
  int n_cu = 256;
  (void)hipDeviceGetAttribute(&n_cu, hipDeviceAttributeMultiprocessorCount, c->device);
  int wg_c = 4 * n_cu;
  if (wg_c > A * SOGM_MAX_PIECES) wg_c = A * SOGM_MAX_PIECES;
  int wg_q = n_cu / 2;
  if (c->tune_i(SOGM_TUNE_QP_WGS) > 0) wg_q = c->tune_i(SOGM_TUNE_QP_WGS);
  if (wg_q > A) wg_q = A;
  if (wg_q < 1) wg_q = 1;
  int wg_f = A < 64 ? A : 64;
  call.n_cu = n_cu, call.wg_q = wg_q, call.wg_f = wg_f;
  prof_begin(c, SOGM_PROF_CORRIDOR, sC);
  if (int rc = launched("sogm_replan: k_corridor_flow",
                        sogm::launch_corridor_flow(mv, p->pp, p->cw, p->fc, A, wg_c, corridor_io(p, start_pva, t_start), sC)))
    return rc;
  prof_end(c, SOGM_PROF_CORRIDOR, sC);
  if (c->update_pending) SOGM_HIP_CHECK(hipStreamWaitEvent(sQ, c->ev_udone, 0));
  prof_begin(c, SOGM_PROF_QP, sQ);
  if (int rc = launched("sogm_replan: k_qp_flow",
                        sogm::launch_qp_flow(p->pp, p->qs, p->qw, p->qc, p->fc, A, wg_q, qp_io(p, start_pva), sQ)))
    return rc;
  prof_end(c, SOGM_PROF_QP, sQ);
  c->gate_open_valid = 0;
  c->gate_frac_valid = 0;
  {
    const double f      = c->tune[SOGM_TUNE_PRESTAMP_GATE_FRAC];
    c->gate_frac_agents = f > 0.0 && f < 1.0 ? ((int)(f * A + 0.5) < 1 ? 1 : (int)(f * A + 0.5)) : 0;
  }
  if (c->overlap >= 2) {
    int rc = sogm::queue_spare_clears(c, p->ev_in);
    if (rc) return rc;
  }
  return SOGM_OK;
}
static int flow_finish(sogm_planner *p, FlowCall &call) {
  sogm_ctx         *c  = p->map;
  const hipStream_t sF = p->fstream[3];
  const int         A  = c->n_agents;
  sogm::FlowCtl fcf = p->fc;
  const bool prestamp = p->ps_on && c->sparse && c->overlap >= 2 && c->pool.front_ready() >= 0 && p->pub_own && c->clear_gate;
  if (!prestamp) fcf.p_ready = nullptr;
  call.prestamp = prestamp;
  return launched("sogm_replan: k_finish_flow",
                  sogm::launch_finish_flow(fcf, A, call.wg_f, finish_args(p, call.t_start, call.drone_ids, call.out_records, call.out_ok), sF));
}
static sogm::PrestampDev prestamp_args(const sogm_planner *p) {
  const sogm_ctx   *c = p->map;
  const int         A = c->n_agents;
  sogm::PrestampDev d = p->ps;
  d.tick.own = p->pub_own;
  d.n_agents = A;
  {
    const double f = c->tune[SOGM_TUNE_PRESTAMP_GATE_FRAC];
    d.gate_agents  = f >= 1.0 ? A : f <= 0.0 ? 0 : (int)(f * A + 0.5);
  }
  const int nb = c->tune_i(SOGM_TUNE_PRESTAMP_BITS) > 0 ? c->tune_i(SOGM_TUNE_PRESTAMP_BITS) : 32;
  const int nm = c->tune_i(SOGM_TUNE_PRESTAMP_MARKS) > 0 ? c->tune_i(SOGM_TUNE_PRESTAMP_MARKS) : 64;
  d.n_bits       = nb;
  d.n_marks      = nm;
  d.n_late       = c->tune_i(SOGM_TUNE_PRESTAMP_LATE_AGENTS) < 0 ? 0 : c->tune_i(SOGM_TUNE_PRESTAMP_LATE_AGENTS);
  d.n_bits_late  = c->tune_i(SOGM_TUNE_PRESTAMP_LATE_BITS) > 0 ? c->tune_i(SOGM_TUNE_PRESTAMP_LATE_BITS) : nb;
  d.n_marks_late = c->tune_i(SOGM_TUNE_PRESTAMP_LATE_MARKS) > 0 ? c->tune_i(SOGM_TUNE_PRESTAMP_LATE_MARKS) : nm;
  return d;
}
static int flow_prestamp(sogm_planner *p, FlowCall &call) {
  sogm_ctx *c = p->map;
  const int A = c->n_agents;
  c->pool.clear_prestamp_target();
  const bool        own_stream = c->tune_i(SOGM_TUNE_PRESTAMP_STREAM) != 0 && c->pstream != nullptr;
  const hipStream_t pst        = own_stream ? c->pstream : c->side;
  call.pst = pst;
  if (call.prestamp) {
    const int nxt = c->pool.front_ready();
    sogm::PrestampDev d = prestamp_args(p);
    if (int rc = sogm::map_target(c, nxt, true, nullptr, &d.tgt)) return rc;
    if (p->ps_world_on)
      if (int rc = sogm::world_blocks(c, &p->ps_world, &d.frame.cb)) return rc;
    SOGM_HIP_CHECK(hipStreamWaitEvent(pst, p->ev_in, 0));
    if (own_stream) {
      SOGM_HIP_CHECK(hipStreamWaitEvent(pst, c->pool.cleared_event(nxt), 0));
      if (c->gate_frac_valid && d.gate_agents < A)
        SOGM_HIP_CHECK(hipStreamWaitEvent(pst, c->ev_gate_frac, 0));
      else if (c->gate_open_valid && d.gate_agents >= A)
        SOGM_HIP_CHECK(hipStreamWaitEvent(pst, c->ev_gate_open, 0));
    }
    int wg_p = 8 * call.n_cu;
    if (c->tune_i(SOGM_TUNE_PRESTAMP_WGS) > 0) wg_p = c->tune_i(SOGM_TUNE_PRESTAMP_WGS);
    if (int rc = launched("sogm_replan: k_prestamp_flow",
                          sogm::launch_prestamp_flow(c->geom, p->fc, d, wg_p, call.wg_q, call.wg_f < A ? call.wg_f : A, pst)))
      return rc;
    c->pool.set_prestamp_target(nxt);
    c->n_stamps++;
    c->ps_fail_host = p->h_flow_fail;
    c->ps_fail_seen = p->h_flow_fail ? p->h_flow_fail[1] : 0;
  }
  return SOGM_OK;
}
static int flow_fan_in(sogm_planner *p, const FlowCall &call) {
  sogm_ctx         *c    = p->map;
  const hipStream_t main = call.main, sC = p->fstream[1], pst = call.pst;
  const int         A    = c->n_agents;
  const int         retire     = c->tune_i(SOGM_TUNE_CLEAR_RETIRE_AT_END);
  auto report = [&](hipStream_t st) {
    hipLaunchKernelGGL(k_flow_report, dim3(1), dim3(1), 0, st, (const int *)p->d_flow, p->h_flow_fail,
                       retire ? p->d_epoch : (int *)nullptr, c->h_tick_clock);
    return hipGetLastError();
  };
  const bool report_on_sc = !c->pool.prestamp_pending();
  for (int k = 0; k < 4; ++k)
    if (k != 1) SOGM_HIP_CHECK(hipEventRecord(p->ev_fdone[k], p->fstream[k]));
  if (report_on_sc) {
    SOGM_HIP_CHECK(hipStreamWaitEvent(sC, p->ev_fdone[2], 0));
    SOGM_HIP_CHECK(hipStreamWaitEvent(sC, p->ev_fdone[3], 0));
    SOGM_HIP_CHECK(report(sC));
  }
  SOGM_HIP_CHECK(hipEventRecord(p->ev_fdone[1], sC));
  for (int k = 0; k < 4; ++k) SOGM_HIP_CHECK(hipStreamWaitEvent(main, p->ev_fdone[k], 0));
  if (int rc = sogm::join_update(c, main)) return rc;
  if (c->d_update_order && c->tune_i(SOGM_TUNE_UPDATE_FLOW) != 0) {
    hipLaunchKernelGGL(k_update_rank, dim3(1), dim3(256), 0, main, (const long long *)p->fc.ts, c->d_update_order, A,
                       c->tune_i(SOGM_TUNE_UPDATE_ORDER));
    SOGM_HIP_CHECK(hipGetLastError());
  }
  bool reported = report_on_sc;
  if (c->pool.prestamp_pending()) {
    for (int k = 1; k < 4; ++k) SOGM_HIP_CHECK(hipStreamWaitEvent(pst, p->ev_fdone[k], 0));
    SOGM_HIP_CHECK(report(pst));
    SOGM_HIP_CHECK(hipEventRecord(p->ev_pdone, pst));
    const int defer = c->tune_i(SOGM_TUNE_SPLAT_OVERLAP) != 0;
    if (defer) {
      c->ev_pdone      = p->ev_pdone;
      c->pdone_pending = 1;
      c->ps_stage      = p->fc.stage;
      c->ps_err        = &p->fc.hdr[FLOW_ERR];
    } else {
      SOGM_HIP_CHECK(hipStreamWaitEvent(main, p->ev_pdone, 0));
    }
    reported = true;
  }
  c->records_final_valid = 0;
  if (p->pub_own) {
    c->ev_records_final    = p->ev_fdone[3];
    c->records_final_ptr   = p->pub_own;
    c->records_final_valid = 1;
  }
  if (!reported) SOGM_HIP_CHECK(report(main));
  return SOGM_OK;
}

static int replan_flow(sogm_planner *p, const double *start_pva, const double *goal, const double *t_start,
                       const int32_t *drone_ids, SogmTrajRecord *out_records, int32_t *out_ok, void *stream) {
  FlowCall call{.start_pva = start_pva, .goal = goal, .t_start = t_start, .drone_ids = drone_ids, .out_records = out_records,
                .out_ok = out_ok, .main = (hipStream_t)stream, .spec = p->spec_astar != 0};
  if (p->swarm)
    if (int rc = sogm::join_exchange(p->map, call.main)) return rc;
  if (int rc = flow_reset(p, call)) return rc;
  if (int rc = flow_launch_chain(p, call)) return rc;
  if (int rc = flow_finish(p, call)) return rc;
  if (int rc = flow_prestamp(p, call)) return rc;
  return flow_fan_in(p, call);
}

static int replan_impl(sogm_planner *p, const double *start_pva, const double *goal,
                       const double *t_start, const int32_t *drone_ids, SogmTrajRecord *out_records,
                       int32_t *out_ok, void *stream) {
  sogm_ctx   *c    = p->map;
  hipStream_t main = (hipStream_t)stream;
  const int   A = c->n_agents, G = p->n_groups;
  const MapView mv = view_of(c);
  if (int rc = sogm::join_update(c, main)) return rc;
  for (int g = 0; g < G; ++g)
    if (!p->gstream[g]) SOGM_HIP_CHECK(p->res.stream(&p->gstream[g]));
  if (p->swarm)
    if (int rc = sogm::join_exchange(c, main)) return rc;
  SOGM_HIP_CHECK(hipEventRecord(p->ev_in, main));
  if (c->overlap >= 2) {
    int rc = sogm::queue_spare_clears(c, p->ev_in);
    if (rc) return rc;
  }
  for (int g = 0; g < G; ++g) {
    const int a0 = (int)((long long)A * g / G), a1 = (int)((long long)A * (g + 1) / G), n = a1 - a0;
    if (n <= 0) continue;
    hipStream_t st = p->gstream[g];
    SOGM_HIP_CHECK(hipStreamWaitEvent(st, p->ev_in, 0));
    hipError_t e = launch_astar(mv, p->ap, p->pp.corridor_tau, astar_ws(p), n, search_io(p, start_pva, goal, t_start),
                                nullptr, 0, st, a0);
    if (e == hipSuccess) e = launch_corridor(mv, p->pp, p->cw, n, corridor_io(p, start_pva, t_start), st, a0, p->ev_pts[g]);
    if (int rc = launched("sogm_replan launch", e)) return rc;
    SOGM_HIP_CHECK(hipEventRecord(p->ev_corr[g], st));
  }
  if (c->overlap == 1) {
    const size_t total = sogm::clear_vec4_total(c);
    size_t       head  = (size_t)28e9 / 16;
    if (head > total / 2) head = total / 2;
    for (int g = 0; g < G; ++g) SOGM_HIP_CHECK(hipStreamWaitEvent(c->side, p->ev_pts[g], 0));
    const int slot = c->pool.current();
    if (c->pool.loggable(slot)) {
      int rc = sogm::reset_slot(c, c->side, slot, c->d_grid, true);
      if (rc) return rc;
    } else {
      int rc = sogm::launch_clear(c, c->side, c->d_grid, true, 1, head);
      if (rc) return rc;
      for (int g = 0; g < G; ++g) SOGM_HIP_CHECK(hipStreamWaitEvent(c->side, p->ev_corr[g], 0));
      rc = sogm::launch_clear(c, c->side, c->d_grid, false, 2, head);
      if (rc) return rc;
    }
    SOGM_HIP_CHECK(hipEventRecord(c->ev_cleared, c->side));
    c->pool.cleared_in_place();
    c->updated = 0;
  }
  for (int g = 0; g < G; ++g) {
    const int a0 = (int)((long long)A * g / G), a1 = (int)((long long)A * (g + 1) / G), n = a1 - a0;
    if (n <= 0) continue;
    hipStream_t st = p->gstream[g];
    if (int rc = launched("sogm_replan launch_qp", launch_qp(p->pp, p->qs, p->qw, p->qc, n, qp_io(p, start_pva), st, a0)))
      return rc;
    if (p->swarm)
      if (int rc = launched("sogm_replan launch_deconflict",
                            sogm::launch_deconflict(n, p->d_cpts, p->d_npoly, p->swarm, p->n_swarm, p->swarm_ego,
                                                    p->swarm_now, p->d_safe, st, a0, p->cw.counters)))
        return rc;
    SOGM_HIP_CHECK(sogm::launch_pack_records(n, finish_args(p, t_start, drone_ids, out_records, out_ok), st, a0));
    SOGM_HIP_CHECK(hipEventRecord(p->ev_done[g], st));
    SOGM_HIP_CHECK(hipStreamWaitEvent(main, p->ev_done[g], 0));
  }
  return SOGM_OK;
}


int sogm_replan(sogm_planner *p, const double *start_pva, const double *goal,
                const double *t_start, const int32_t *drone_ids, SogmTrajRecord *out_records,
                int32_t *out_ok, void *stream) {
  if (!p || !start_pva || !goal || !t_start || !drone_ids || !out_records || !out_ok)
    return SOGM_ERR_INVALID_ARG;
  if (!p->map->updated) return SOGM_ERR_STATE;
  sogm_ctx *c = p->map;
  if (p->pub_table && p->swarm) {
    const char *a0 = (const char *)p->pub_table, *a1 = a0 + sizeof(SogmTrajRecord) * (size_t)c->n_agents;
    const char *b0 = (const char *)p->swarm, *b1 = b0 + sizeof(SogmTrajRecord) * (size_t)p->n_swarm;
    if (a0 < b1 && b0 < a1) {
      sogm::set_error_text("sogm_replan: sogm_planner_set_publish's next_table overlaps the table given to sogm_planner_set_swarm");
      return SOGM_ERR_INVALID_ARG;
    }
  }
  if (p->pub_own) {
    const char *a0 = (const char *)p->pub_own, *a1 = a0 + sizeof(SogmTrajRecord) * (size_t)c->n_agents;
    const char *b0 = (const char *)out_records, *b1 = b0 + sizeof(SogmTrajRecord) * (size_t)c->n_agents;
    if (a0 < b1 && b0 < a1) {
      sogm::set_error_text("sogm_replan: out_records overlaps sogm_planner_set_publish's own_records");
      return SOGM_ERR_INVALID_ARG;
    }
  }
  SOGM_HIP_CHECK(hipSetDevice(c->device));
  const bool use_flow = p->flow && c->overlap != 1;
  if (int jr = sogm::join_prestamp(c, (hipStream_t)stream)) return jr;
  const int  rc = use_flow ? replan_flow(p, start_pva, goal, t_start, drone_ids, out_records, out_ok, stream)
                           : replan_impl(p, start_pva, goal, t_start, drone_ids, out_records, out_ok, stream);
  if (rc != SOGM_OK) {
    (void)hipDeviceSynchronize();
    if (c->pool.precleared() && c->overlap == 1) c->updated = 0;
    if (c->overlap < 2) c->pool.forget_preclear();
  }
  return rc;
}
}
```

### pred-occ-planner_amd/csrc/sogm_planner.hpp

```cpp
#pragma once

#include "sogm_device.hpp"
#include "sogm_handover.hpp"

namespace sogm {

struct AstarWorkspace {
  char  *pool;
  size_t pool_stride;
  void  *hkeys;
  int    hash_cap;
  long long *dbg;
  int *verdict;
};
int astar_pool_max();

struct CorridorWorkspace {
  double  *pc;
  double  *fpc;
  double  *tang;
  double  *distr;
  double  *polys;
  int32_t *seg_nfaces;
  int32_t *seg_state;
// ... 42 lines not shown
  void     *cand;
  int      *n_cand;
  MarkLog   lg;
  float    *poses;
  double   *stamps;
};
struct MapFrame {
  const float        *cloud;
  const int32_t      *cloud_range;
  CloudBlocks         cb;
  const SogmCylinder *cyl;
  int                 n_cyl;
};
struct OverlayIO {
  const SogmTrajRecord *rec;
  int                   n_rec;
  const int32_t        *ego_ids;
  const double         *body;
  int                   n_body;
};
struct TickInputsIO {
  const SogmTrajRecord *own;
  double               *hover, *now, *t_start, *pva;
  double                start_offset;
};
__device__ inline void tick_inputs_agent(const SogmTrajRecord &rec, const double *hov, int i, double stamp,
                                         const TickInputsIO &io, float *__restrict__ poses) {
  const double ts = stamp + io.start_offset;
  double       o[9];
  if (!traj_eval_record(rec, ts, o))
    for (int k = 0; k < 9; ++k) o[k] = hov[k];
  for (int k = 0; k < 9; ++k) io.pva[i * 9 + k] = o[k];
  for (int k = 0; k < 3; ++k) {
    io.hover[i * 9 + k]     = o[k];
    io.hover[i * 9 + 3 + k] = 0.0;
    io.hover[i * 9 + 6 + k] = 0.0;
    poses[i * 3 + k]        = (float)o[k];
  }
  io.now[i]     = stamp;
  io.t_start[i] = ts;
}
__device__ __forceinline__ void stage_record_hover(SogmTrajRecord *s_rec, double *s_hov, const SogmTrajRecord *own,
                                                   const double *hover, int agent, int lane) {
  copy_record(s_rec, own + agent, lane);
  if (lane < 9) s_hov[lane] = hover[agent * 9 + lane];
  __syncthreads();
}
struct FlightMapDev {
  MapTarget             tgt;
  const FlightWorld    *worlds;
  CloudBlocks           cb;
  OverlayIO             ov;
  const SogmTrajRecord *tables;
  int                   n_total;
  TickInputsIO          tick;
  double                t0, period;
  int                   n_reset, n_bits, n_marks, n_splat;
  int                   un_reset, un_bits, un_marks, un_splat;
  int                   n_head_wgs;
  int                   n_uhead_wgs;
  int                   n_uwork_wgs;
  int                   n_admit;
  int                   pace_ticks;
  size_t                agent_bytes;
  unsigned long long   *reset_stat;
  FlightFsmDev          fsm;
};
hipError_t launch_flight_map(const GridGeom &g, const FlightCtl &fl, const FlightMapDev &d, int n_workgroups, hipStream_t st);

struct SearchIO {
  const double *start_pva, *goal, *t_start;
  int32_t      *out_ret;
  double       *out_route;
  int32_t      *out_route_len;
  int           route_cap;
  int32_t      *out_stats;
  const int32_t *due;
};
struct CorridorIO {
  const double  *start_pva, *t_start, *route;
  const int32_t *route_len;
  int            route_cap;
  double        *out_polys;
  int32_t       *out_nfaces, *out_npoly;
  double        *out_goal;
  __device__ __forceinline__ int points(int agent) const {
    const int n = route_len[agent];
    return n < route_cap ? n : route_cap;
  }
};
struct QpIO {
  const double  *start_pva, *goal_pv, *polys;
  const int32_t *nfaces, *npoly;
  double        *out_cpts;
  int32_t       *out_status, *out_iters;
};
struct FinishArgs {
  double                corridor_tau;
  const int32_t        *ret, *npoly, *status;
  const double         *cpts;
  const SogmTrajRecord *swarm;
  int                   n_swarm;
  const int32_t        *swarm_ego;
  const double         *swarm_now, *t_start;
  const int32_t        *drone_ids;
  SogmTrajRecord       *out;
  int32_t              *out_ok, *out_safe;
  unsigned long long   *counters;
  SogmTrajRecord       *pub_own, *pub_table;
  const int32_t        *due;
};
struct FlightLightDev {
  CorridorIO      cor;
  FinishArgs      fin;
  SogmTrajRecord *tables;
  int             n_total, agent0;
  SogmTrajRecord *log_records;
  int32_t        *log_ok;
  FlightFsmDev    fsm;
};
struct CorridorWorkspace;
hipError_t launch_flight_light(const MapView &m, const SogmPlannerParams &pp, const CorridorWorkspace &ws, const FlightCtl &fl,
                               const FlightLightDev &d, int n_workgroups, hipStream_t st);
struct AstarWorkspace;
hipError_t launch_flight_search(const MapView &m, const SogmAstarParams &ap, double corridor_tau, const AstarWorkspace &wsp,
                                const FlightCtl &fl, int n_workgroups, const SearchIO &io, int spec, hipStream_t st);
struct QpWorkspace;
struct QpConst;
hipError_t launch_flight_qp(const SogmPlannerParams &pp, const SogmQpSettings &qs, const QpWorkspace &ws, const QpConst &qc,
                            const FlightCtl &fl, int n_workgroups, const QpIO &io, hipStream_t st);

struct PrestampDev {
  MapTarget    tgt;
  MapFrame     frame;
  TickInputsIO tick;
  double       stamp;
  float       *poses_host;
  int          n_agents;
  int          n_bits, n_marks;
  int          n_late, n_bits_late, n_marks_late;
  int          gate_agents;
};
hipError_t launch_prestamp_flow(const GridGeom &g, const FlowCtl &fc, const PrestampDev &ps, int n_workgroups, int n_qp,
                                int n_finish, hipStream_t st);

hipError_t launch_deconflict(int n_agents, const double *cpts, const int32_t *npoly, const SogmTrajRecord *rec,
                             int n_rec, const int32_t *ego_ids, const double *t_now, int32_t *out_safe,
                             hipStream_t st, int agent0, unsigned long long *counters = nullptr);
hipError_t launch_pack_records(int n_agents, const FinishArgs &f, hipStream_t st, int agent0);
hipError_t launch_corridor(const MapView &m, const SogmPlannerParams &pp, const CorridorWorkspace &ws, int n_agents,
                           const CorridorIO &io, hipStream_t st, int agent0 = 0, hipEvent_t ev_map_read = nullptr);

hipError_t launch_flow_gate(const FlowCtl &fc, int expected, hipStream_t st);
hipError_t launch_corridor_flow(const MapView &m, const SogmPlannerParams &pp, const CorridorWorkspace &ws,
                                const FlowCtl &fc, int n_agents, int n_workgroups, const CorridorIO &io, hipStream_t st);
hipError_t launch_finish_flow(const FlowCtl &fc, int n_agents, int n_workgroups, const FinishArgs &f, hipStream_t st);

struct QpWorkspace {
  char  *scratch;
  size_t scratch_stride;
  int    dyn_lds_bytes;
  double *k1_scratch;
  const double *t_alloc;
  int           goal_stride;
  long long    *dbg;
  int           ablate;
};
int    qp_kernel_setup();
struct QpConst {
  double QM[225];
};
int astar_resident_workgroups(int device);
hipError_t launch_qp(const SogmPlannerParams &pp, const SogmQpSettings &qs, const QpWorkspace &ws, const QpConst &qc,
                     int n_agents, const QpIO &io, hipStream_t st, int agent0 = 0);
hipError_t launch_qp_flow(const SogmPlannerParams &pp, const SogmQpSettings &qs, const QpWorkspace &ws, const QpConst &qc,
                          const FlowCtl &fc, int n_agents, int n_workgroups, const QpIO &io, hipStream_t st);

size_t astar_node_bytes();
hipError_t launch_astar(const MapView &m, const SogmAstarParams &ap, double corridor_tau, const AstarWorkspace &wsp,
                        int n_agents, const SearchIO &io, int32_t *out_trace, int trace_cap, hipStream_t st,
                        int agent0 = 0, const FlowCtl *fc = nullptr, int search_mode = 0);

}

#define SOGM_MAX_GROUPS 64

struct sogm_planner {
  sogm::Resources      res;
  sogm_ctx            *map;
  SogmAstarParams      ap;
  SogmPlannerParams    pp;
  SogmQpSettings       qs;
  sogm::AstarWorkspace aw;
  sogm::CorridorWorkspace cw;
  sogm::QpWorkspace qw;
  sogm::QpConst qc;
  int32_t *d_ret, *d_route_len, *d_stats;
  double  *d_route;
  int      route_cap;
  double  *d_polys, *d_goal, *d_cpts;
  int32_t *d_nfaces, *d_npoly, *d_status, *d_iters;
  int32_t              *d_safe;
  const SogmTrajRecord *swarm;
  int                   n_swarm;
  const int32_t        *swarm_ego;
  const double         *swarm_now;
  SogmTrajRecord       *pub_own, *pub_table;
  const int32_t        *due;
  int         n_groups;
  hipStream_t gstream[SOGM_MAX_GROUPS];
  hipEvent_t  ev_in, ev_corr[SOGM_MAX_GROUPS], ev_done[SOGM_MAX_GROUPS];
  hipEvent_t  ev_pts[SOGM_MAX_GROUPS];
  int            flow;
  int           *d_flow;
  long long     *d_flow_ts;
  sogm::FlowCtl  fc;
  hipStream_t    fstream[4];
  hipEvent_t     ev_pdone;
  sogm::PrestampDev ps;
  int            ps_on;
  int            ps_world_on;
  SogmWorld      ps_world;
  hipEvent_t     ev_gate, ev_fdone[4];
  int           *d_epoch;
  int            reset_epoch;
  int           *h_flow_fail;
  int sel_first, sel_count;
  int search_mode;
  int spec_astar;
  hipStream_t peek;
  sogm::FlightCtl     fl;
  int                *d_fl;
  sogm::FlightWorld  *d_fl_worlds, *h_fl_worlds;
  double             *d_fl_pva, *d_fl_tstart, *d_fl_now;
  hipStream_t         fl_stream[4];
  hipEvent_t          fl_ev_in, fl_ev_done[4];
  int                 fl_cus[4];
  int                 fl_wgs[4];
  int                 fl_epoch = 0;
  int                *fl_xready = nullptr;
  int                 fl_fsm_on = 0;
  SogmFlightFsm       fl_fsm{};
  int32_t            *d_fl_due = nullptr, *d_fl_reached = nullptr;
  double             *d_fl_posnow = nullptr;
};

inline sogm::AstarWorkspace astar_ws(const sogm_planner *p) {
  sogm::AstarWorkspace w = p->aw;
  if (!((p->map->profiling >> SOGM_PROF_ASTAR) & 1)) w.dbg = nullptr;
  return w;
}

inline int launched(const char *what, hipError_t e) {
  if (e == hipSuccess) return SOGM_OK;
  sogm::set_error(what, e);
  return SOGM_ERR_HIP;
}

inline sogm::SearchIO search_io(const sogm_planner *p, const double *start_pva, const double *goal, const double *t_start) {
  return sogm::SearchIO{.start_pva = start_pva, .goal = goal, .t_start = t_start, .out_ret = p->d_ret,
                        .out_route = p->d_route, .out_route_len = p->d_route_len, .route_cap = p->route_cap,
                        .out_stats = p->d_stats, .due = p->due};
}
inline sogm::CorridorIO corridor_io(const sogm_planner *p, const double *start_pva, const double *t_start) {
  return sogm::CorridorIO{.start_pva = start_pva, .t_start = t_start, .route = p->d_route,
                          .route_len = p->d_route_len, .route_cap = p->route_cap, .out_polys = p->d_polys,
                          .out_nfaces = p->d_nfaces, .out_npoly = p->d_npoly, .out_goal = p->d_goal};
}
inline sogm::QpIO qp_io(const sogm_planner *p, const double *start_pva) {
  return sogm::QpIO{.start_pva = start_pva, .goal_pv = p->d_goal, .polys = p->d_polys, .nfaces = p->d_nfaces,
                    .npoly = p->d_npoly, .out_cpts = p->d_cpts, .out_status = p->d_status, .out_iters = p->d_iters};
}
inline sogm::FinishArgs finish_args(const sogm_planner *p, const double *t_start, const int32_t *drone_ids,
                                    SogmTrajRecord *out, int32_t *out_ok) {
  return sogm::FinishArgs{.corridor_tau = p->pp.corridor_tau, .ret = p->d_ret, .npoly = p->d_npoly,
                          .status = p->d_status, .cpts = p->d_cpts, .swarm = p->swarm, .n_swarm = p->n_swarm,
                          .swarm_ego = p->swarm_ego, .swarm_now = p->swarm_now, .t_start = t_start,
                          .drone_ids = drone_ids, .out = out, .out_ok = out_ok, .out_safe = p->d_safe,
                          .counters = p->cw.counters, .pub_own = p->pub_own, .pub_table = p->pub_table,
                          .due = p->due};
}
```

### pred-occ-planner_amd/csrc/sogm_resources.hpp

```cpp
#pragma once
#include <hip/hip_runtime.h>

#include <cstddef>
#include <cstdint>
#include <vector>

namespace sogm {
class Resources {
 public:
  Resources() = default;
  Resources(const Resources &)            = delete;
  Resources &operator=(const Resources &) = delete;

  template <class T>
  hipError_t device(T **out, size_t bytes, bool zero = false) {
    void      *p = nullptr;
    hipError_t e = hipMalloc(&p, bytes);
    if (e == hipSuccess && zero && p) e = hipMemset(p, 0, bytes);
    return hold(DEVICE, p, (void **)out, e);
  }
  template <class T>
  hipError_t array(T **out, size_t n) {
    return device(out, n ? n * sizeof(T) : 16);
  }
  template <class T>
  hipError_t pinned(T **out, size_t bytes, unsigned flags) {
    void      *p = nullptr;
    hipError_t e = hipHostMalloc(&p, bytes, flags);
    return hold(PINNED, p, (void **)out, e);
  }
  hipError_t stream(hipStream_t *out) {
    hipStream_t s = nullptr;
    hipError_t  e = hipStreamCreateWithFlags(&s, hipStreamNonBlocking);
    return hold(STREAM, s, (void **)out, e);
  }
  hipError_t stream_masked(hipStream_t *out, uint32_t mask_words, const uint32_t *mask) {
    hipStream_t s = nullptr;
    hipError_t  e = hipExtStreamCreateWithCUMask(&s, mask_words, mask);
    return hold(STREAM, s, (void **)out, e);
  }
  hipError_t event(hipEvent_t *out, unsigned flags = hipEventDisableTiming) {
    hipEvent_t v = nullptr;
    hipError_t e = hipEventCreateWithFlags(&v, flags);
    return hold(EVENT, v, (void **)out, e);
  }

  template <class H>
  void release(H *field) {
    for (size_t i = held_.size(); i-- > 0;)
      if (held_[i].handle == (void *)*field && *field) {
        free_handle(held_[i]);
        held_.erase(held_.begin() + (std::ptrdiff_t)i);
        break;
      }
    *field = nullptr;
  }

  size_t mark() const { return held_.size(); }
  void rollback(size_t mark) {
    for (int pass = 0; pass < 3; ++pass)
      for (size_t i = held_.size(); i-- > mark;) {
        const Held &h = held_[i];
        if ((h.kind == STREAM ? 0 : h.kind == EVENT ? 1 : 2) != pass) continue;
        free_handle(h);
        if (*h.field == h.handle) *h.field = nullptr;
      }
    held_.resize(mark);
  }
  void release_all() { rollback(0); }

  class Setup {
   public:
    explicit Setup(Resources &r) : r_(r), mark_(r.mark()) {}
    ~Setup() {
      if (!done_) r_.rollback(mark_);
    }
    Setup(const Setup &)            = delete;
    Setup &operator=(const Setup &) = delete;
    int done() {
      done_ = true;
      return 0;
    }

   private:
    Resources &r_;
    size_t     mark_;
    bool       done_ = false;
  };

 private:
  enum Kind : unsigned char { STREAM, EVENT, DEVICE, PINNED };
  struct Held {
    Kind   kind;
    void  *handle;
    void **field;
  };
  std::vector<Held> held_;

  static void free_handle(const Held &h) {
    switch (h.kind) {
      case STREAM:
        (void)hipStreamSynchronize((hipStream_t)h.handle);
        (void)hipStreamDestroy((hipStream_t)h.handle);
        break;
      case EVENT: (void)hipEventDestroy((hipEvent_t)h.handle); break;
      case DEVICE: (void)hipFree(h.handle); break;
      case PINNED: (void)hipHostFree(h.handle); break;
    }
  }
  hipError_t hold(Kind kind, void *handle, void **field, hipError_t e) {
    const Held h{kind, handle, field};
    if (e == hipSuccess && handle) {
      try {
        held_.push_back(h);
      } catch (...) {
        e = hipErrorOutOfMemory;
      }
    }
    if (e != hipSuccess) {
      if (handle) free_handle(h);
      return e;
    }
    *field = handle;
    return hipSuccess;
  }
};
}
```

### pred-occ-planner_amd/planner.py

```python
import ctypes as C

import numpy as np
import torch

from . import _abi
from ._abi import SOGM_MAX_PIECES, check, lib
from .sogm import _dev, _stream


def linprog_batched(c, A_rows, b_rows, row_range):
    n, d = c.shape
    x = torch.zeros((n, d), dtype=torch.float64, device=c.device)
    v = torch.zeros((n,), dtype=torch.float64, device=c.device)
    check(lib().sogm_linprog_batched(d, c.data_ptr(), A_rows.data_ptr(), b_rows.data_ptr(), row_range.data_ptr(),
                                     n, x.data_ptr(), v.data_ptr(), _stream()), "sogm_linprog_batched")
    return x, v


def firi_batched(bd, pc, pc_range, a, b, r=None, iterations=2, epsilon=1.0e-6, max_points=4096, max_faces=64):
    n, n_bd = int(bd.shape[0]), int(bd.shape[1])
    dev = bd.device
    if r is None:
        r = torch.ones((n, 3), dtype=torch.float64, device=dev)
    hp = torch.zeros((n, max_faces, 4), dtype=torch.float64, device=dev)
    nf = torch.zeros((n,), dtype=torch.int32, device=dev)
    st = torch.zeros((n,), dtype=torch.int32, device=dev)
    check(lib().sogm_firi_batched(bd.data_ptr(), n_bd, pc.data_ptr(), pc_range.data_ptr(), a.data_ptr(), b.data_ptr(),
                                  r.data_ptr(), iterations, epsilon, n, max_points, max_faces, hp.data_ptr(),
                                  nf.data_ptr(), st.data_ptr(), _stream()), "sogm_firi_batched")
    return hp, nf, st, r


def corridor_rules_batched(pps, start_pva, route, route_len, polys, nfaces, seg_state=None, planner=None, parallel=False):
    n, P, MF = int(polys.shape[0]), SOGM_MAX_PIECES, int(polys.shape[2])
    dev = polys.device
    pp = (_abi.SogmPlannerParams * max(n, 1))(*pps)
    f64 = lambda *shape: torch.zeros(shape, dtype=torch.float64, device=dev)
    i32 = lambda *shape: torch.zeros(shape, dtype=torch.int32, device=dev)
    out = {"box": f64(n, P, 6), "shrunk": f64(n, P, MF, 4), "seg_nfaces": i32(n, P), "seg_state": i32(n, P),
           "polys": f64(n, P, MF, 4), "nfaces": i32(n, P), "npoly": i32(n), "goal": f64(n, 6)}
    check(lib().sogm_corridor_rules_batched_flags(
        planner._p if planner is not None else None, pp, start_pva.data_ptr(), route.data_ptr(), route_len.data_ptr(),
        int(route.shape[1]), polys.data_ptr(), nfaces.data_ptr(), seg_state.data_ptr() if seg_state is not None else None,
        n, MF, out["box"].data_ptr(), out["shrunk"].data_ptr(), out["seg_nfaces"].data_ptr(), out["seg_state"].data_ptr(),
        out["polys"].data_ptr(), out["nfaces"].data_ptr(), out["npoly"].data_ptr(), out["goal"].data_ptr(),
        _abi.RULES_PARALLEL if parallel else 0, _stream()), "sogm_corridor_rules_batched_flags")
    return out


def finish_batched(corridor_tau, ret, npoly, status, cpts, t_start, drone_ids, out, out_ok, out_safe, swarm=None, n_swarm=0,
                   swarm_ego=None, swarm_now=None, due=None, pub_own=None, pub_table=None, planner=None, wave=False):
    ptr = lambda t: t.data_ptr() if t is not None else None
    check(lib().sogm_finish_batched(
        planner._p if planner is not None else None, float(corridor_tau), ptr(ret), ptr(npoly), ptr(status), ptr(cpts),
        ptr(swarm), int(n_swarm), ptr(swarm_ego), ptr(swarm_now), ptr(t_start), ptr(drone_ids), ptr(due), int(ret.numel()),
        ptr(out), ptr(out_ok), ptr(out_safe), ptr(pub_own), ptr(pub_table), _abi.FINISH_WAVE if wave else 0, _stream()),
        "sogm_finish_batched")


class SogmPlanner:
    def __init__(self, sogm_map, astar_params, planner_params, qp_settings):
        self.map = sogm_map
        self.ap, self.pp, self.qs = astar_params, planner_params, qp_settings
        self.A = sogm_map.n_agents
        self._p = C.c_void_p()
        check(lib().sogm_planner_create(sogm_map.ctx, C.byref(astar_params), C.byref(planner_params),
                                        C.byref(qp_settings), C.byref(self._p)), "sogm_planner_create")

    def close(self):
        if self._p:
            torch.cuda.synchronize()
            lib().sogm_planner_destroy(self._p)
            self._p = C.c_void_p()

    def __del__(self):
        try:
            self.close()
        except Exception:
            pass

    def select_agents(self, first=0, count=None):
        check(lib().sogm_planner_select_agents(self._p, first, self.A if count is None else count),
              "sogm_planner_select_agents")

    def set_search_mode(self, mode):
        check(lib().sogm_planner_set_search_mode(self._p, mode), "sogm_planner_set_search_mode")

    def flow_error(self):
        return int(lib().sogm_planner_flow_error(self._p))

    def flow_failures(self):
        out = (C.c_int32 * 2)()
        check(lib().sogm_planner_flow_failures(self._p, out), "sogm_planner_flow_failures")
        return int(out[0]), int(out[1])

    def counters(self, reset=False):
        out = (C.c_int64 * len(_abi.COUNTER_NAMES))()
        check(lib().sogm_planner_counters(self._p, out, 1 if reset else 0), "sogm_planner_counters")
        return dict(zip(_abi.COUNTER_NAMES, [int(v) for v in out]))

    def corridor_pairs(self):
        out = (C.c_uint64 * 4)()
        check(lib().sogm_debug_corridor_pairs(self._p, out), "sogm_debug_corridor_pairs")
        return dict(zip(("eager", "late", "consumed", "residue"), [int(v) for v in out]))

    def qp_stats(self):
        out = np.zeros((self.A, _abi.QP_STAT_N), np.int64)
        check(lib().sogm_debug_qp_stats(self._p, out.ctypes.data_as(C.c_void_p)), "sogm_debug_qp_stats")
        return out

    def qp_layout(self, nfaces):
        nf = np.ascontiguousarray(nfaces, dtype=np.int32)
        out = (C.c_longlong * 8)()
        check(lib().sogm_debug_qp_layout(self._p, len(nf), nf.ctypes.data_as(C.c_void_p), out), "sogm_debug_qp_layout")
        keys = ("fast", "rows_in_lds", "dyn_lds_bytes", "lds_bytes", "scratch_bytes", "k1_in_lds", "G", "S")
        return dict(zip(keys, [int(v) for v in out]))

    def search(self, start_pva, goal, t_start, route_cap=64, trace_cap=0):
        A, dev = self.A, start_pva.device
        out = {
            "ret": torch.zeros((A,), dtype=torch.int32, device=dev),
            "route": torch.zeros((A, route_cap, 6), dtype=torch.float64, device=dev),
            "route_len": torch.zeros((A,), dtype=torch.int32, device=dev),
            "stats": torch.zeros((A, 4), dtype=torch.int32, device=dev),
            "trace": torch.full((A, max(trace_cap, 1)), -1, dtype=torch.int32, device=dev),
        }
        check(lib().sogm_astar_search(self._p, start_pva.data_ptr(), goal.data_ptr(), t_start.data_ptr(),
                                      out["ret"].data_ptr(), out["route"].data_ptr(),
                                      out["route_len"].data_ptr(), route_cap, out["stats"].data_ptr(),
                                      out["trace"].data_ptr() if trace_cap else None, trace_cap, _stream()),
              "sogm_astar_search")
        return out

    def generateCorridors(self, start_pva, t_start, route, route_len):
        A, dev = self.A, start_pva.device
        mf = self.pp.max_faces
        out = {
            "polys": torch.zeros((A, SOGM_MAX_PIECES, mf, 4), dtype=torch.float64, device=dev),
            "nfaces": torch.zeros((A, SOGM_MAX_PIECES), dtype=torch.int32, device=dev),
            "npoly": torch.zeros((A,), dtype=torch.int32, device=dev),
            "goal": torch.zeros((A, 6), dtype=torch.float64, device=dev),
        }
        check(lib().sogm_corridor_generate(self._p, start_pva.data_ptr(), t_start.data_ptr(),
                                           route.data_ptr(), route_len.data_ptr(), int(route.shape[1]),
                                           out["polys"].data_ptr(), out["nfaces"].data_ptr(),
                                           out["npoly"].data_ptr(), out["goal"].data_ptr(), _stream()),
              "sogm_corridor_generate")
        return out

    def optimize(self, start_pva, goal_pv, polys, nfaces, npoly):
        A, dev = self.A, start_pva.device
        out = {
            "cpts": torch.zeros((A, SOGM_MAX_PIECES * 15), dtype=torch.float64, device=dev),
            "status": torch.zeros((A,), dtype=torch.int32, device=dev),
            "iters": torch.zeros((A,), dtype=torch.int32, device=dev),
        }
        check(lib().sogm_bezier_qp_solve(self._p, start_pva.data_ptr(), goal_pv.data_ptr(),
                                         polys.data_ptr(), nfaces.data_ptr(), npoly.data_ptr(),
                                         out["cpts"].data_ptr(), out["status"].data_ptr(),
                                         out["iters"].data_ptr(), _stream()), "sogm_bezier_qp_solve")
        return out

    def optimize_timed(self, start_pva, end_pva, time_alloc, polys, nfaces, npoly, max_vel, max_acc):
        A, dev = self.A, start_pva.device
        out = {
            "cpts": torch.zeros((A, SOGM_MAX_PIECES * 15), dtype=torch.float64, device=dev),
            "status": torch.zeros((A,), dtype=torch.int32, device=dev),
            "iters": torch.zeros((A,), dtype=torch.int32, device=dev),
        }
        check(lib().sogm_bezier_qp_solve_timed(self._p, start_pva.data_ptr(), end_pva.data_ptr(), time_alloc.data_ptr(),
                                               float(max_vel), float(max_acc), polys.data_ptr(), nfaces.data_ptr(),
                                               npoly.data_ptr(), out["cpts"].data_ptr(), out["status"].data_ptr(),
                                               out["iters"].data_ptr(), _stream()), "sogm_bezier_qp_solve_timed")
        return out

    def isSafeAfterOpt(self, cpts, npoly, records, n_records, ego_ids, t_now):
        safe = torch.empty((self.A,), dtype=torch.int32, device=cpts.device)
        check(lib().sogm_safe_after_opt(self._p, cpts.data_ptr(), npoly.data_ptr(), records.data_ptr(), n_records,
                                        ego_ids.data_ptr(), t_now.data_ptr(), safe.data_ptr(), _stream()),
              "sogm_safe_after_opt")
        return safe

    def setSwarm(self, records, n_records, ego_ids, t_now):
        self._swarm = (records, ego_ids, t_now)
        if records is None:
            check(lib().sogm_planner_set_swarm(self._p, None, 0, None, None), "sogm_planner_set_swarm")
        else:
            check(lib().sogm_planner_set_swarm(self._p, records.data_ptr(), n_records, ego_ids.data_ptr(),
                                               t_now.data_ptr()), "sogm_planner_set_swarm")

    def set_due(self, due=None):
        self._due = due
        check(lib().sogm_planner_set_due(self._p, due.data_ptr() if due is not None else None), "sogm_planner_set_due")

    def set_flight_fsm(self, prm=None, check_duration=0.2, state=None, logs=None):
        if prm is None:
            self._flight_fsm = None
            check(lib().sogm_planner_set_flight_fsm(self._p, None), "sogm_planner_set_flight_fsm")
            return
        logs = dict(logs or {})
        ptr = lambda t: t.data_ptr() if t is not None else None
        f = _abi.SogmFlightFsm(prm, float(check_duration), ptr(state), ptr(logs.get("state")), ptr(logs.get("due")),
                               ptr(logs.get("safe")), ptr(logs.get("reached")), ptr(logs.get("pub")),
                               ptr(logs.get("hover_start")), ptr(logs.get("own")))
        self._flight_fsm = (state, logs)
        check(lib().sogm_planner_set_flight_fsm(self._p, C.byref(f)), "sogm_planner_set_flight_fsm")

    def setPublish(self, own_records, next_table=None):
        self._publish = (own_records, next_table)
        check(lib().sogm_planner_set_publish(self._p, own_records.data_ptr() if own_records is not None else None,
                                             next_table.data_ptr() if next_table is not None else None),
              "sogm_planner_set_publish")

    def setPrestamp(self, cloud, cloud_range, cylinders, n_cyl, next_stamp, start_offset, hover, now, t_start, pva,
                    poses=None, world=None):
        if cloud is None and world is None:
            self._prestamp = None
            check(lib().sogm_planner_set_prestamp(self._p, None), "sogm_planner_set_prestamp")
            return
        ptr = lambda t: t.data_ptr() if t is not None else None
        ps = _abi.SogmPrestamp(ptr(cloud), ptr(cloud_range), ptr(cylinders), int(n_cyl or 0), 0,
                               float(next_stamp), float(start_offset), hover.data_ptr(), now.data_ptr(),
                               t_start.data_ptr(), pva.data_ptr(), ptr(poses),
                               C.pointer(world.c) if world is not None else None)
        self._prestamp = (cloud, cloud_range, cylinders, hover, now, t_start, pva, poses, world)
        check(lib().sogm_planner_set_prestamp(self._p, C.byref(ps)), "sogm_planner_set_prestamp")

    def flight(self, worlds, first_tick, t0, period, start_offset, goals, drone_ids, hover, own, tables, log_records,
               log_ok, n_total=None, agent0=0, comm=None):
        n = len(worlds)
        arr = (_abi.SogmWorld * n)(*[w.c for w in worlds])
        f = _abi.SogmFlight(n, int(first_tick), float(t0), float(period), float(start_offset), arr, goals.data_ptr(),
                            drone_ids.data_ptr(), hover.data_ptr(), own.data_ptr(), tables.data_ptr(),
                            self.A if n_total is None else int(n_total), int(agent0),
                            log_records.data_ptr(), log_ok.data_ptr(), comm)
        self._flight_keep = (worlds, arr, goals, drone_ids, hover, own, tables, log_records, log_ok)
        check(lib().sogm_flight_run(self._p, C.byref(f), _stream()), "sogm_flight_run")

    def flight_prepare(self, max_cloud_points=0):
        check(lib().sogm_flight_prepare(self._p, int(max_cloud_points)), "sogm_flight_prepare")

    def flight_stats(self):
        ms = np.zeros((self.A, 8), np.float64)
        hdr = np.zeros((32,), np.int32)
        check(lib().sogm_flight_stats(self._p, ms.ctypes.data_as(C.c_void_p), hdr.ctypes.data_as(C.c_void_p)),
              "sogm_flight_stats")
        return ms, hdr

    def replan(self, start_pva, goal, t_start, drone_ids, out_records=None, out_ok=None):
        A, dev = self.A, start_pva.device
        if out_records is None:
            out_records = torch.zeros((A, _abi.TRAJ_RECORD_BYTES), dtype=torch.uint8, device=dev)
# ... 45 lines not shown
```

Before: 12930 replans/s.

## Merge finish workers into corridor flow kernel and trim planner streams

Finish work moves out of its own kernel on a separate stream. The first wg_f workgroups of a new combined k_worker_flow kernel now run it, while the remaining workgroups run corridor tickets. Planner streams drop from four to two (worker and QP), and the side2 and pstream streams are now created only when first needed. This removes one kernel launch, one stream and several event waits and records per replan, in exchange for the finish and corridor workloads sharing one grid and its LDS sizing. It also adds tuning knobs for the finish and corridor workgroup counts and a debug query for how many streams are held.

```diff
diff --git a/include/sogm_abi_debug.h b/include/sogm_abi_debug.h
--- a/include/sogm_abi_debug.h
+++ b/include/sogm_abi_debug.h
@@ -70,6 +70,8 @@
 
 int sogm_debug_corridor_pairs(sogm_planner *p, unsigned long long *out4);
 
+int sogm_debug_streams_held(sogm_planner *p);
+
 enum {
   SOGM_QP_STAT_TOTAL = 0,
   SOGM_QP_STAT_SETUP = 1,
diff --git a/pred-occ-planner_amd/_abi.py b/pred-occ-planner_amd/_abi.py
--- a/pred-occ-planner_amd/_abi.py
+++ b/pred-occ-planner_amd/_abi.py
@@ -324,6 +324,7 @@
     "sogm_finish_batched": (_i, [_vp, C.c_double, _vp, _vp, _vp, _vp, _vp, _i, _vp, _vp, _vp, _vp, _vp, _i, _vp, _vp, _vp,
                                  _vp, _vp, _i, _vp]),
     "sogm_debug_corridor_pairs": (_i, [_vp, _vp]),
+    "sogm_debug_streams_held": (_i, [_vp]),
     "sogm_debug_qp_stats": (_i, [_vp, _vp]),
     "sogm_debug_qp_layout": (_i, [_vp, _i, _vp, _vp]),
     "sogm_replan": (_i, [_vp, _vp, _vp, _vp, _vp, _vp, _vp, _vp]),
diff --git a/pred-occ-planner_amd/csrc/sogm_clear.hip b/pred-occ-planner_amd/csrc/sogm_clear.hip
--- a/pred-occ-planner_amd/csrc/sogm_clear.hip
+++ b/pred-occ-planner_amd/csrc/sogm_clear.hip
@@ -312,7 +312,12 @@
   const int    throttle = env_wgs ? env_throttle : (polite ? 4 : 0);
   const int    nblk     = (int)(want < 1 ? 1 : (want > max_wgs ? max_wgs : want));
   const int wide_wgs = c->tune_i(SOGM_TUNE_CLEAR_WIDE_WGS), wide_bound = c->tune_i(SOGM_TUNE_CLEAR_WIDE_BOUND);
-  if (polite && part == 0 && c->clear_gate && c->clear_cursor && c->side2 && wide_wgs > 0 && nt) {
+  if (polite && part == 0 && c->clear_gate && c->clear_cursor && !c->sparse && wide_wgs > 0 && nt) {
+    if (!c->side2) {
+      Resources::Setup setup(c->res);
+      SOGM_HIP_CHECK(c->res.stream(&c->side2));
+      setup.done();
+    }
     const size_t        nchunks = (nall + CLEAR_CHUNK_V4 - 1) / CLEAR_CHUNK_V4;
     unsigned long long *cur = c->clear_cursor + (c->clear_seq & 1), *nxt = c->clear_cursor + ((c->clear_seq + 1) & 1);
     ++c->clear_seq;
diff --git a/pred-occ-planner_amd/csrc/sogm_context.hip b/pred-occ-planner_amd/csrc/sogm_context.hip
--- a/pred-occ-planner_amd/csrc/sogm_context.hip
+++ b/pred-occ-planner_amd/csrc/sogm_context.hip
@@ -95,8 +95,6 @@
   if (e == hipSuccess) e = c->res.device(&c->d_scratch_vt, sizeof(float) * (size_t)c->geom.V * spec->T);
   if (e == hipSuccess) e = c->res.device(&c->clear_cursor, 2 * sizeof(unsigned long long), true);
   if (e == hipSuccess) e = c->res.stream(&c->side);
-  if (e == hipSuccess) e = c->res.stream(&c->side2);
-  if (e == hipSuccess) e = c->res.stream(&c->pstream);
   if (e == hipSuccess) e = c->res.event(&c->ev_side2_go);
   if (e == hipSuccess) e = c->res.event(&c->ev_side2_done);
   if (e == hipSuccess) e = c->res.event(&c->ev_grid_free);
diff --git a/pred-occ-planner_amd/csrc/sogm_corridor.hip b/pred-occ-planner_amd/csrc/sogm_corridor.hip
--- a/pred-occ-planner_amd/csrc/sogm_corridor.hip
+++ b/pred-occ-planner_amd/csrc/sogm_corridor.hip
@@ -1,6 +1,7 @@
 #include <hip/hip_runtime.h>
 
 #include "sogm_corridor.hpp"
+#include "sogm_finish.hpp"
 
 namespace sogm {
 
@@ -106,10 +107,30 @@
   if (v) atomicOr(&pair_cnt[3], (unsigned long long)v);
 }
 
-__global__ __launch_bounds__(64) void k_corridor_flow(MapView m, SogmPlannerParams pp, CorridorWorkspace ws,
-                                                      FlowCtl fc, CorridorIO io, int n_agents) {
-  extern __shared__ __attribute__((aligned(16))) char smem[];
-  const int lane  = threadIdx.x;
+__global__ __launch_bounds__(64) void k_worker_flow(MapView m, SogmPlannerParams pp, CorridorWorkspace ws, FlowCtl fc,
+                                                    CorridorIO io, FinishArgs f, int n_agents, int wg_f) {
+  extern __shared__ __attribute__((aligned(16))) char smem[];
+  const int lane = threadIdx.x;
+  if ((int)blockIdx.x < wg_f) {
+    for (;;) {
+      const int k = flow_ticket(&fc.hdr[FLOW_F_TICKET]);
+      if (k >= n_agents) break;
+      const int a = flow_wait_slot(fc.f_ready + k, &fc.hdr[FLOW_ERR]);
+      if (a < 0) break;
+      __threadfence();
+      const int  code = finish_agent(f, a, LpLds::carve(smem), lane);
+      const bool safe = (code & 1) != 0;
+      if (fc.p_ready) {
+        __threadfence();
+        if (lane == 0) publish_next(fc.p_ready, &fc.hdr[FLOW_P_READY_N], a);
+      }
+      if (lane == 0) {
+        fc.ts[a * 8 + 6] = wall_clock64();
+        finish_count(f, a, safe);
+      }
+    }
+    return;
+  }
   const int total = n_agents * SOGM_MAX_PIECES;
   for (;;) {
     const int k = flow_ticket(&fc.hdr[FLOW_C_TICKET]);
@@ -128,10 +149,11 @@
   }
 }
 
-hipError_t launch_corridor_flow(const MapView &m, const SogmPlannerParams &pp, const CorridorWorkspace &ws,
-                                const FlowCtl &fc, int n_agents, int n_workgroups, const CorridorIO &io, hipStream_t st) {
-  hipLaunchKernelGGL(k_corridor_flow, dim3(n_workgroups), dim3(64), SegmentLds<6>::bytes(pp.pc_capacity), st, m, pp,
-                     ws, fc, io, n_agents);
+hipError_t launch_worker_flow(const MapView &m, const SogmPlannerParams &pp, const CorridorWorkspace &ws, const FlowCtl &fc,
+                              int n_agents, int n_finish, int n_corridor, const CorridorIO &io, const FinishArgs &f,
+                              hipStream_t st) {
+  hipLaunchKernelGGL(k_worker_flow, dim3(n_finish + n_corridor), dim3(64), SegmentLds<6>::bytes(pp.pc_capacity), st, m, pp,
+                     ws, fc, io, f, n_agents, n_finish);
   return hipGetLastError();
 }
 
diff --git a/pred-occ-planner_amd/csrc/sogm_device.hpp b/pred-occ-planner_amd/csrc/sogm_device.hpp
--- a/pred-occ-planner_amd/csrc/sogm_device.hpp
+++ b/pred-occ-planner_amd/csrc/sogm_device.hpp
@@ -447,6 +447,8 @@
   X(SPEC_ASTAR, "spec_astar", 1, 0, 1)             \
   X(CLEAR_GATE_FRAC, "clear_gate_frac", 1, 0, 1)  \
   X(QP_WGS, "qp_wgs", 0, 0, 1024)                     \
+  X(FINISH_WGS, "finish_wgs", 0, 0, 64)             \
+  X(CORRIDOR_WGS, "corridor_wgs", 0, 0, 65536)      \
   X(QP_ABLATE, "qp_ablate", 0, 0, 255)               \
   X(CLEAR_WGS, "clear_wgs", 0, 0, 65536)               \
   X(CLEAR_THROTTLE, "clear_throttle", 0, 0, 64)     \
diff --git a/pred-occ-planner_amd/csrc/sogm_finish.hip b/pred-occ-planner_amd/csrc/sogm_finish.hip
--- a/pred-occ-planner_amd/csrc/sogm_finish.hip
+++ b/pred-occ-planner_amd/csrc/sogm_finish.hip
@@ -22,28 +22,6 @@
 __global__ void k_fill_i32(int32_t *p, int n, int32_t v, int agent0) {
   const int i = blockIdx.x * blockDim.x + threadIdx.x;
   if (i < n) p[agent0 + i] = v;
-}
-
-__global__ __launch_bounds__(64) void k_finish_flow(FlowCtl fc, FinishArgs f, int n_agents) {
-  extern __shared__ __attribute__((aligned(16))) double s_dyn[];
-  const int lane = threadIdx.x;
-  for (;;) {
-    const int k = flow_ticket(&fc.hdr[FLOW_F_TICKET]);
-    if (k >= n_agents) break;
-    const int a = flow_wait_slot(fc.f_ready + k, &fc.hdr[FLOW_ERR]);
-    if (a < 0) break;
-    __threadfence();
-    const int  code = finish_agent(f, a, LpLds::carve(s_dyn), lane);
-    const bool safe = (code & 1) != 0;
-    if (fc.p_ready) {
-      __threadfence();
-      if (lane == 0) publish_next(fc.p_ready, &fc.hdr[FLOW_P_READY_N], a);
-    }
-    if (lane == 0) {
-      fc.ts[a * 8 + 6] = wall_clock64();
-      finish_count(f, a, safe);
-    }
-  }
 }
 
 __global__ __launch_bounds__(64) void k_finish_wave(FinishArgs f) {
@@ -85,11 +63,6 @@
   return hipGetLastError();
 }
 
-hipError_t launch_finish_flow(const FlowCtl &fc, int n_agents, int n_workgroups, const FinishArgs &f, hipStream_t st) {
-  hipLaunchKernelGGL(k_finish_flow, dim3(n_workgroups), dim3(64), LpLds::bytes(), st, fc, f, n_agents);
-  return hipGetLastError();
-}
-
 hipError_t launch_pack_records(int n_agents, const FinishArgs &f, hipStream_t st, int agent0) {
   hipLaunchKernelGGL(k_pack_records, dim3((n_agents + 63) / 64), dim3(64), 0, st, agent0 + n_agents, f, agent0);
   return hipGetLastError();
diff --git a/pred-occ-planner_amd/csrc/sogm_planner.hip b/pred-occ-planner_amd/csrc/sogm_planner.hip
--- a/pred-occ-planner_amd/csrc/sogm_planner.hip
+++ b/pred-occ-planner_amd/csrc/sogm_planner.hip
@@ -128,10 +128,9 @@
   SOGM_HIP_CHECK(p->res.event(&p->ev_pdone));
   SOGM_HIP_CHECK(p->res.device(&p->d_flow_ts, sizeof(long long) * 12 * (size_t)A, true));
   p->fc.ts = p->d_flow_ts;
-  for (int k = 0; k < 4; ++k) {
-    SOGM_HIP_CHECK(p->res.stream(&p->fstream[k]));
-    SOGM_HIP_CHECK(p->res.event(&p->ev_fdone[k]));
-  }
+  SOGM_HIP_CHECK(p->res.event(&p->ev_records));
+  SOGM_HIP_CHECK(p->res.event(&p->ev_wdone));
+  SOGM_HIP_CHECK(p->res.event(&p->ev_qdone));
   SOGM_HIP_CHECK(p->res.event(&p->ev_gate));
   SOGM_HIP_CHECK(p->res.device(&p->d_epoch, sizeof(int), true));
   SOGM_HIP_CHECK(p->res.pinned(&p->h_flow_fail, sizeof(int) * 2, hipHostMallocMapped));
@@ -392,6 +391,11 @@
   return SOGM_OK;
 }
 
+int sogm_debug_streams_held(sogm_planner *p) {
+  if (!p || !p->map) return SOGM_ERR_INVALID_ARG;
+  return p->map->res.streams_held() + p->res.streams_held();
+}
+
 int sogm_debug_flow_times(sogm_planner *p, long long *out_host) {
   if (!p || !out_host) return SOGM_ERR_INVALID_ARG;
   SOGM_HIP_CHECK(hipDeviceSynchronize());
@@ -579,9 +583,16 @@
   hipStream_t     pst;
 };
 
+static int flow_streams(sogm_planner *p) {
+  if (p->wstream && p->qstream) return SOGM_OK;
+  sogm::Resources::Setup setup(p->res);
+  SOGM_HIP_CHECK(p->res.stream(&p->wstream));
+  SOGM_HIP_CHECK(p->res.stream(&p->qstream));
+  return setup.done();
+}
 static int flow_reset(sogm_planner *p, FlowCall &call) {
   sogm_ctx         *c    = p->map;
-  const hipStream_t main = call.main, sC = p->fstream[1];
+  const hipStream_t main = call.main, sC = p->wstream;
   const int         A    = c->n_agents;
   const bool        spec = call.spec;
   SOGM_HIP_CHECK(hipStreamWaitEvent(sC, p->ev_pdone, 0));
@@ -600,9 +611,14 @@
   call.gen_word = gen_word;
   return SOGM_OK;
 }
+static bool flow_prestamps(const sogm_planner *p) {
+  const sogm_ctx *c = p->map;
+  return p->ps_on && c->sparse && c->overlap >= 2 && (c->pool.front_ready() >= 0 || c->pool.first_dirty() >= 0) && p->pub_own &&
+         c->clear_gate;
+}
 static int flow_launch_chain(sogm_planner *p, FlowCall &call) {
   sogm_ctx         *c    = p->map;
-  const hipStream_t main = call.main, sA = main, sC = p->fstream[1], sQ = p->fstream[2], sF = p->fstream[3];
+  const hipStream_t main = call.main, sA = main, sC = p->wstream, sQ = p->qstream;
   const int         A    = c->n_agents;
   const MapView     mv   = view_of(c);
   const bool        spec = call.spec;
@@ -610,8 +626,10 @@
   const double     *start_pva = call.start_pva, *goal = call.goal, *t_start = call.t_start;
   SogmTrajRecord   *out_records = call.out_records;
   int32_t          *out_ok      = call.out_ok;
-  if (c->exchange_pending)
-    for (int k = 1; k < 4; ++k) SOGM_HIP_CHECK(hipStreamWaitEvent(p->fstream[k], c->ev_xdone, 0));
+  if (c->exchange_pending) {
+    SOGM_HIP_CHECK(hipStreamWaitEvent(sC, c->ev_xdone, 0));
+    SOGM_HIP_CHECK(hipStreamWaitEvent(sQ, c->ev_xdone, 0));
+  }
   prof_begin(c, SOGM_PROF_ASTAR, sA);
   sogm::FlowCtl fca = p->fc;
   fca.map_ready = c->update_pending ? c->d_map_ready : nullptr;
@@ -630,22 +648,29 @@
   if (int rc = launched("sogm_replan: k_flow_gate", sogm::launch_flow_gate(p->fc, spec ? 2 * A : A, sC))) return rc;
   SOGM_HIP_CHECK(hipEventRecord(p->ev_gate, sC));
   SOGM_HIP_CHECK(hipStreamWaitEvent(sQ, p->ev_gate, 0));
-  SOGM_HIP_CHECK(hipStreamWaitEvent(sF, p->ev_gate, 0));
   int n_cu = 256;
   (void)hipDeviceGetAttribute(&n_cu, hipDeviceAttributeMultiprocessorCount, c->device);
   int wg_c = 4 * n_cu;
+  if (c->tune_i(SOGM_TUNE_CORRIDOR_WGS) > 0) wg_c = c->tune_i(SOGM_TUNE_CORRIDOR_WGS);
   if (wg_c > A * SOGM_MAX_PIECES) wg_c = A * SOGM_MAX_PIECES;
   int wg_q = n_cu / 2;
   if (c->tune_i(SOGM_TUNE_QP_WGS) > 0) wg_q = c->tune_i(SOGM_TUNE_QP_WGS);
   if (wg_q > A) wg_q = A;
   if (wg_q < 1) wg_q = 1;
-  int wg_f = A < 64 ? A : 64;
+  int wg_f = 64;
+  if (c->tune_i(SOGM_TUNE_FINISH_WGS) > 0) wg_f = c->tune_i(SOGM_TUNE_FINISH_WGS);
+  if (wg_f > A) wg_f = A;
   call.n_cu = n_cu, call.wg_q = wg_q, call.wg_f = wg_f;
+  call.prestamp     = flow_prestamps(p);
+  sogm::FlowCtl fcw = p->fc;
+  if (!call.prestamp) fcw.p_ready = nullptr;
   prof_begin(c, SOGM_PROF_CORRIDOR, sC);
-  if (int rc = launched("sogm_replan: k_corridor_flow",
-                        sogm::launch_corridor_flow(mv, p->pp, p->cw, p->fc, A, wg_c, corridor_io(p, start_pva, t_start), sC)))
+  if (int rc = launched("sogm_replan: k_worker_flow",
+                        sogm::launch_worker_flow(mv, p->pp, p->cw, fcw, A, wg_f, wg_c, corridor_io(p, start_pva, t_start),
+                                                 finish_args(p, t_start, call.drone_ids, out_records, out_ok), sC)))
     return rc;
   prof_end(c, SOGM_PROF_CORRIDOR, sC);
+  SOGM_HIP_CHECK(hipEventRecord(p->ev_records, sC));
   if (c->update_pending) SOGM_HIP_CHECK(hipStreamWaitEvent(sQ, c->ev_udone, 0));
   prof_begin(c, SOGM_PROF_QP, sQ);
   if (int rc = launched("sogm_replan: k_qp_flow",
@@ -664,17 +689,6 @@
   }
   return SOGM_OK;
 }
-static int flow_finish(sogm_planner *p, FlowCall &call) {
-  sogm_ctx         *c  = p->map;
-  const hipStream_t sF = p->fstream[3];
-  const int         A  = c->n_agents;
-  sogm::FlowCtl fcf = p->fc;
-  const bool prestamp = p->ps_on && c->sparse && c->overlap >= 2 && c->pool.front_ready() >= 0 && p->pub_own && c->clear_gate;
-  if (!prestamp) fcf.p_ready = nullptr;
-  call.prestamp = prestamp;
-  return launched("sogm_replan: k_finish_flow",
-                  sogm::launch_finish_flow(fcf, A, call.wg_f, finish_args(p, call.t_start, call.drone_ids, call.out_records, call.out_ok), sF));
-}
 static sogm::PrestampDev prestamp_args(const sogm_planner *p) {
   const sogm_ctx   *c = p->map;
   const int         A = c->n_agents;
@@ -698,8 +712,13 @@
   sogm_ctx *c = p->map;
   const int A = c->n_agents;
   c->pool.clear_prestamp_target();
-  const bool        own_stream = c->tune_i(SOGM_TUNE_PRESTAMP_STREAM) != 0 && c->pstream != nullptr;
-  const hipStream_t pst        = own_stream ? c->pstream : c->side;
+  const bool own_stream = c->tune_i(SOGM_TUNE_PRESTAMP_STREAM) != 0 && call.prestamp;
+  if (own_stream && !c->pstream) {
+    sogm::Resources::Setup setup(c->res);
+    SOGM_HIP_CHECK(c->res.stream(&c->pstream));
+    setup.done();
+  }
+  const hipStream_t pst = own_stream ? c->pstream : c->side;
   call.pst = pst;
   if (call.prestamp) {
     const int nxt = c->pool.front_ready();
@@ -729,7 +748,7 @@
 }
 static int flow_fan_in(sogm_planner *p, const FlowCall &call) {
   sogm_ctx         *c    = p->map;
-  const hipStream_t main = call.main, sC = p->fstream[1], pst = call.pst;
+  const hipStream_t main = call.main, sC = p->wstream, sQ = p->qstream, pst = call.pst;
   const int         A    = c->n_agents;
   const int         retire     = c->tune_i(SOGM_TUNE_CLEAR_RETIRE_AT_END);
   auto report = [&](hipStream_t st) {
@@ -738,15 +757,14 @@
     return hipGetLastError();
   };
   const bool report_on_sc = !c->pool.prestamp_pending();
-  for (int k = 0; k < 4; ++k)
-    if (k != 1) SOGM_HIP_CHECK(hipEventRecord(p->ev_fdone[k], p->fstream[k]));
+  SOGM_HIP_CHECK(hipEventRecord(p->ev_qdone, sQ));
   if (report_on_sc) {
-    SOGM_HIP_CHECK(hipStreamWaitEvent(sC, p->ev_fdone[2], 0));
-    SOGM_HIP_CHECK(hipStreamWaitEvent(sC, p->ev_fdone[3], 0));
+    SOGM_HIP_CHECK(hipStreamWaitEvent(sC, p->ev_qdone, 0));
     SOGM_HIP_CHECK(report(sC));
   }
-  SOGM_HIP_CHECK(hipEventRecord(p->ev_fdone[1], sC));
-  for (int k = 0; k < 4; ++k) SOGM_HIP_CHECK(hipStreamWaitEvent(main, p->ev_fdone[k], 0));
+  SOGM_HIP_CHECK(hipEventRecord(p->ev_wdone, sC));
+  SOGM_HIP_CHECK(hipStreamWaitEvent(main, p->ev_wdone, 0));
+  SOGM_HIP_CHECK(hipStreamWaitEvent(main, p->ev_qdone, 0));
   if (int rc = sogm::join_update(c, main)) return rc;
   if (c->d_update_order && c->tune_i(SOGM_TUNE_UPDATE_FLOW) != 0) {
     hipLaunchKernelGGL(k_update_rank, dim3(1), dim3(256), 0, main, (const long long *)p->fc.ts, c->d_update_order, A,
@@ -755,7 +773,8 @@
   }
   bool reported = report_on_sc;
   if (c->pool.prestamp_pending()) {
-    for (int k = 1; k < 4; ++k) SOGM_HIP_CHECK(hipStreamWaitEvent(pst, p->ev_fdone[k], 0));
+    SOGM_HIP_CHECK(hipStreamWaitEvent(pst, p->ev_wdone, 0));
+    SOGM_HIP_CHECK(hipStreamWaitEvent(pst, p->ev_qdone, 0));
     SOGM_HIP_CHECK(report(pst));
     SOGM_HIP_CHECK(hipEventRecord(p->ev_pdone, pst));
     const int defer = c->tune_i(SOGM_TUNE_SPLAT_OVERLAP) != 0;
@@ -771,7 +790,7 @@
   }
   c->records_final_valid = 0;
   if (p->pub_own) {
-    c->ev_records_final    = p->ev_fdone[3];
+    c->ev_records_final    = p->ev_records;
     c->records_final_ptr   = p->pub_own;
     c->records_final_valid = 1;
   }
@@ -785,9 +804,9 @@
                 .out_ok = out_ok, .main = (hipStream_t)stream, .spec = p->spec_astar != 0};
   if (p->swarm)
     if (int rc = sogm::join_exchange(p->map, call.main)) return rc;
+  if (int rc = flow_streams(p)) return rc;
   if (int rc = flow_reset(p, call)) return rc;
   if (int rc = flow_launch_chain(p, call)) return rc;
-  if (int rc = flow_finish(p, call)) return rc;
   if (int rc = flow_prestamp(p, call)) return rc;
   return flow_fan_in(p, call);
 }
diff --git a/pred-occ-planner_amd/csrc/sogm_planner.hpp b/pred-occ-planner_amd/csrc/sogm_planner.hpp
--- a/pred-occ-planner_amd/csrc/sogm_planner.hpp
+++ b/pred-occ-planner_amd/csrc/sogm_planner.hpp
@@ -218,9 +218,9 @@
                            const CorridorIO &io, hipStream_t st, int agent0 = 0, hipEvent_t ev_map_read = nullptr);
 
 hipError_t launch_flow_gate(const FlowCtl &fc, int expected, hipStream_t st);
-hipError_t launch_corridor_flow(const MapView &m, const SogmPlannerParams &pp, const CorridorWorkspace &ws,
-                                const FlowCtl &fc, int n_agents, int n_workgroups, const CorridorIO &io, hipStream_t st);
-hipError_t launch_finish_flow(const FlowCtl &fc, int n_agents, int n_workgroups, const FinishArgs &f, hipStream_t st);
+hipError_t launch_worker_flow(const MapView &m, const SogmPlannerParams &pp, const CorridorWorkspace &ws, const FlowCtl &fc,
+                              int n_agents, int n_finish, int n_corridor, const CorridorIO &io, const FinishArgs &f,
+                              hipStream_t st);
 
 struct QpWorkspace {
   char  *scratch;
@@ -281,13 +281,15 @@
   int           *d_flow;
   long long     *d_flow_ts;
   sogm::FlowCtl  fc;
-  hipStream_t    fstream[4];
+  hipStream_t    wstream, qstream;
   hipEvent_t     ev_pdone;
   sogm::PrestampDev ps;
   int            ps_on;
   int            ps_world_on;
   SogmWorld      ps_world;
-  hipEvent_t     ev_gate, ev_fdone[4];
+  hipEvent_t     ev_gate;
+  hipEvent_t     ev_records;
+  hipEvent_t     ev_wdone, ev_qdone;
   int           *d_epoch;
   int            reset_epoch;
   int           *h_flow_fail;
diff --git a/pred-occ-planner_amd/csrc/sogm_resources.hpp b/pred-occ-planner_amd/csrc/sogm_resources.hpp
--- a/pred-occ-planner_amd/csrc/sogm_resources.hpp
+++ b/pred-occ-planner_amd/csrc/sogm_resources.hpp
@@ -54,6 +54,12 @@
         break;
       }
     *field = nullptr;
+  }
+
+  int streams_held() const {
+    int n = 0;
+    for (const Held &h : held_) n += h.kind == STREAM ? 1 : 0;
+    return n;
   }
 
   size_t mark() const { return held_.size(); }
diff --git a/pred-occ-planner_amd/planner.py b/pred-occ-planner_amd/planner.py
--- a/pred-occ-planner_amd/planner.py
+++ b/pred-occ-planner_amd/planner.py
@@ -98,6 +98,12 @@
         out = (C.c_int64 * len(_abi.COUNTER_NAMES))()
         check(lib().sogm_planner_counters(self._p, out, 1 if reset else 0), "sogm_planner_counters")
         return dict(zip(_abi.COUNTER_NAMES, [int(v) for v in out]))
+
+    def streams_held(self):
+        n = int(lib().sogm_debug_streams_held(self._p))
+        if n < 0:
+            check(n, "sogm_debug_streams_held")
+        return n
 
     def corridor_pairs(self):
         out = (C.c_uint64 * 4)()
```

After: 13520 replans/s, median of 6. 4.5% higher.
